# zhvng/open-musiclm

Hardware: AMD Instinct MI355X
Metric: train steps/sec + AR tokens/sec, coarse-stage musiclm_small (higher is better)
Workload: dtype fp16ff

## Files before the change

### include/omlm.h

```cpp
#ifndef OMLM_H
#define OMLM_H
#include <stdint.h>
#ifdef __cplusplus
extern "C" {
#endif

int         omlm_version(void);
const char* omlm_last_error(void);
void        omlm_set_error(const char* msg);

int omlm_gemm(const void* A, const void* B, void* C, const float* Cin,
              const int* a_map, const int* b_map, const int* c_map, long long a_rows, long long b_rows,
              int M, int N, int K, int lda, int ldb, int ldc, int ldcin,
              int a_kmajor, int b_kmajor, int in_dtype, int out_dtype, float alpha,
              void* workspace, long long workspace_bytes, void* stream);
long long omlm_gemm_tail_workspace_bytes(int M, int N);

int omlm_layernorm_fwd(const float* x, const float* gamma, void* y, void* xcast, float* mean, float* rstd,
                       int M, int D, int ldy, float eps, int out_dtype, void* stream);
int omlm_layernorm_fwd_planes(const float* x, const float* gamma, void* y, void* y_lo, float* mean, float* rstd,
                              int M, int D, int ldy, float eps, int out_dtype, void* stream);
long long omlm_layernorm_bwd_workspace_bytes(int D);
int omlm_layernorm_bwd(const void* dy, const float* x, const float* gamma, const float* mean, const float* rstd,
                       const float* dres, float* dx, void* dxcast, float* dgamma, float* workspace, int M, int D,
                       float dx_scale, int cast_dtype, int dy_dtype, void* stream);
int omlm_layernorm_bwd2(const void* dy, const float* x, const float* gamma, const float* mean, const float* rstd,
                        const float* dres, const void* dres2, float* dx, void* dxcast, float* dgamma, float* workspace, int M, int D,
                        float dx_scale, int cast_dtype, int dy_dtype, void* stream);

int omlm_qk_norm_fwd(const float* q_raw, const float* kv_raw, const float* q_scale, const float* k_scale,
                     void* q, void* k, void* v, int M, int H, int out_dtype, void* stream);
int omlm_qk_norm_bwd(const float* dq, const float* dk, const float* dv, const float* q_raw, const float* kv_raw,
                     const float* q_scale, const float* k_scale, void* dq_raw, void* dkv_raw,
                     float* dq_scale, float* dk_scale, int M, int H, int out_dtype, void* stream);

int omlm_gemm_qknorm(const void* A, const void* B, void* C, void* C2, int c2_col0, int ldc2, const float* scale, float* norm_out,
                     int ldnorm, int groups, long long a_rows, long long b_rows, int M, int N, int K, int lda, int ldb, int ldc,
                     int dtype, void* stream);
int omlm_qk_norm_bwd2(const float* dq, const float* dk, const float* dv, const void* q, const void* k, const float* qn, const float* kn,
                      const float* q_scale, const float* k_scale, void* dq_raw, void* dkv_raw, float* dq_scale, float* dk_scale,
                      int M, int H, int dtype, void* stream);

int omlm_mqa_attn_fwd(const void* q, const void* k, const void* v, const float* bias, const float* biasT,
                      const unsigned char* keymask, void* out, float* lse, int B, int N, int H, float scale, int bias_ld,
                      int dtype, void* stream);
long long omlm_attn_bias_table_floats(int N, int H);
int omlm_attn_bias_prepare(const float* bias, float* biasT, int N, int H, int bias_ld, const float* q_scale,
                           const float* k_scale, float qk_bound, float scale, int p_max_log2, void* stream);
int omlm_attn_bias_prepare_group(const float* bias, float* const* biasT, int layers, int N, int H, int bias_ld,
                                 const float* const* q_scale, const float* const* k_scale, float qk_bound, float scale,
                                 int p_max_log2, void* stream);
long long omlm_mqa_attn_bwd_workspace_bytes(int B, int N, int H);
int omlm_mqa_attn_bwd(const void* q, const void* k, const void* v, const float* bias, const float* biasT,
                      const unsigned char* keymask, const void* out, const void* dout, const float* lse, float* delta,
                      float* dq, float* dk, float* dv, float* dbias, float* dbias_ws,
                      int B, int N, int H, float scale, int bias_ld, int dtype, void* stream);

int omlm_mqa_attn_fwd_dropout(const void* q, const void* k, const void* v, const float* bias, const float* biasT,
                              const unsigned char* keymask, void* out, float* lse, int B, int N, int H, float scale, int bias_ld,
                              int dtype, float p, unsigned long long seed, const unsigned long long* seed_dev, void* stream);
int omlm_mqa_attn_bwd_dropout(const void* q, const void* k, const void* v, const float* bias, const float* biasT,
                              const unsigned char* keymask, const void* out, const void* dout, const float* lse, float* delta,
                              float* dq, float* dk, float* dv, float* dbias, float* dbias_ws,
                              int B, int N, int H, float scale, int bias_ld, int dtype, float p, unsigned long long seed,
                              const unsigned long long* seed_dev, void* stream);
int omlm_mqa_attn_fwd_prefix(const void* q, const void* k, const void* v, const float* bias, const float* biasT, const unsigned char* keymask,
                             void* out, float* lse, int B, int N, int H, float scale, int bias_ld, int dtype, int P, float p,
                             unsigned long long seed, const unsigned long long* seed_dev, void* stream);
int omlm_mqa_attn_bwd_prefix(const void* q, const void* k, const void* v, const float* bias, const float* biasT, const unsigned char* keymask,
                             const void* out, const void* dout, const float* lse, float* delta, float* dq, float* dk, float* dv, float* dbias,
                             float* dbias_ws, int B, int N, int H, float scale, int bias_ld, int dtype, int P, float p, unsigned long long seed,
                             const unsigned long long* seed_dev, void* stream);
long long omlm_attn_bias_table_floats_prefix(int N, int H, int P);
int omlm_attn_bias_prepare_group_prefix(const float* bias, float* const* biasT, int layers, int N, int H, int bias_ld,
                                        const float* const* q_scale, const float* const* k_scale, float qk_bound, float scale,
                                        int p_max_log2, int P, void* stream);
int omlm_attn_dropout_keep(unsigned char* keep, int B, int N, int H, float p, unsigned long long seed,
                           const unsigned long long* seed_dev, void* stream);
int omlm_dropout_residual_fwd(const float* x, const float* y, float* x1, long long M, int D, float p, unsigned long long seed,
                              const unsigned long long* seed_dev, void* stream);
int omlm_dropout_residual_bwd(const float* dx1, void* dy, long long M, int D, float p, unsigned long long seed,
                              const unsigned long long* seed_dev, int out_dtype, void* stream);

int omlm_ffmid_fwd(const void* h1, const void* convw, const void* gamma, void* h2, float* mean, float* rstd,
                   int M, int nseq, int F, int Fp, float eps, float p, unsigned long long seed,
                   const unsigned long long* seed_dev, unsigned char* drop_bits, void* gh, int dtype, void* stream);
int omlm_ffmid_fwd_planes(const void* h1, const void* h1_lo, const void* convw, const void* convw_lo, const void* gamma, const void* gamma_lo,
                          void* h2, void* h2_lo, float* mean, float* rstd, int M, int nseq, int F, int Fp, float eps, float p,
                          unsigned long long seed, const unsigned long long* seed_dev, unsigned char* drop_bits, void* gh, int dtype, void* stream);
long long omlm_ffmid_bwd_workspace_bytes(int F, int Fp);
int omlm_ffmid_bwd(const void* dh2, const void* h1, const void* convw, const void* gamma, const float* mean,
                   const float* rstd, void* du_tmp, void* dh1, float* dgamma, float* dconv, float* workspace,
                   int M, int nseq, int F, int Fp, float p, unsigned long long seed,
                   const unsigned long long* seed_dev, const unsigned char* drop_bits, const void* gh, int dtype, void* stream);
int omlm_colsum_accumulate(const float* part, float* out, int P, int C, int ldp, void* stream);
typedef struct omlm_colsum_desc { const float* part; float* out; int P, C, ldp; } omlm_colsum_desc;
int omlm_colsum_group(const omlm_colsum_desc* problems, int count, void* stream);
int omlm_ffmid_set_impl(int impl);

int omlm_embed_gather_fwd(const int* ids, const int* seg, const int* posidx,
                          const float* const* tables, const float* const* starts, const float* const* pos,
                          int nseq, float* out, int B, int N, int D,
                          const long long* table_rows, const long long* pos_rows, int* err_flag, void* stream);
int omlm_embed_gather_bwd(const int* ids, const int* seg, const int* posidx,
                          float* const* dtables, float* const* dstarts, float* const* dpos,
                          int nseq, const float* dx, int B, int N, int D, float alpha,
                          const long long* table_rows, const long long* pos_rows, int* err_flag, void* stream);

int omlm_prepare_train_batch(const long long* const* ids, int* const* labels, const int* len, const int* eos, const int* Q,
                             const int* codebook, int nseq, int B, int pad_id, const float* scores, int n_drop,
                             int* ids32, unsigned char* keymask, int N, void* stream);

int omlm_cross_entropy_fwd(const float* logits, const int* labels, float* row_lse, float* nll_sum,
                           int R, int V, int ld, int* err_flag, void* stream);
int omlm_cross_entropy_bwd(const float* logits, const int* labels, const float* row_lse, const float* gscale,
                           float coef, void* dlogits, int R, int V, int ld, int ldd, int out_dtype, void* stream);

int omlm_sumsq_accumulate(const float* g, long long n, float* out, float* partials, void* stream);
int omlm_adamw_clip_step(float* p, float* g, float* m, float* v, void* p16, long long n,
                         float lr, float beta1, float beta2, float eps, float wd, int step,
                         float gscale, const float* gnorm_sq, float max_norm, int decoupled, int zero_grad, int p16_dtype,
                         const float* ls_state, void* stream);
int omlm_loss_scale_update(float* ls_state, const float* gnorm_sq, float growth, float backoff, int interval,
                           float scale_min, float scale_max, void* stream);

int omlm_cast_pad(const float* src, void* dst, long long R, int C, int ld_src, int ld_dst, int out_dtype, void* stream);
int omlm_transpose_cast(const float* src, void* dst, int R, int C, int ld_src, int ld_dst, int out_dtype, void* stream);
typedef struct omlm_cast_pad_desc { const float* src; void* dst; int R, C, ld_src, ld_dst, transpose, lo; } omlm_cast_pad_desc;
int omlm_cast_pad_group(const omlm_cast_pad_desc* problems, int count, int out_dtype, void* stream);

int omlm_gemm_planes(const void* A, long long a_plane_bytes, const void* B, long long b_plane_bytes, void* C, const float* Cin,
                     const int* a_map, const int* b_map, const int* c_map, long long a_rows, long long b_rows,
                     int M, int N, int K, int lda, int ldb, int ldc, int ldcin,
                     int a_kmajor, int b_kmajor, int out_dtype, float alpha, void* workspace, long long workspace_bytes, void* stream);
int omlm_split_planes(const float* x, void* planes, long long n, long long plane_elems, void* stream);
int omlm_gemm_planes16(const void* A, const void* A_lo, const void* B, const void* B_lo, void* C, void* C_lo, const float* Cin,
                       const int* a_map, const int* c_map, long long a_rows, long long b_rows, int M, int N, int K,
                       int lda, int ldb, int ldc, int ldcin, int dtype, void* workspace, long long workspace_bytes, void* stream);
int omlm_gemm_mx16(const void* A, const void* A8, long long a8_stride, const unsigned char* a_scale,
                   const void* B, const void* B8, long long b8_stride, const unsigned char* b_scale,
                   void* C, void* C_lo, int c_lo_bf8, const float* Cin, long long a_rows, long long b_rows,
                   int M, int N, int K, int lda, int ldb, int ldc, int ldcin,
                   void* workspace, long long workspace_bytes, void* stream);
long long omlm_gemm_mx16_workspace_bytes(int M, int N, int K);
int omlm_layernorm_fwd_mx(const float* x, const float* gamma, void* y, void* y8, long long y8_stride, unsigned char* scale8,
                          float* mean, float* rstd, int M, int D, int ldy, float eps, void* stream);
int omlm_ffmid_fwd_mx(const void* h1, const void* h1_lo, const void* convw, const void* convw_lo, const void* gamma, const void* gamma_lo,
                      void* h2, void* h2_8, long long h2_8_stride, unsigned char* scale8, float* mean, float* rstd, int M, int nseq, int F, int Fp,
                      float eps, float p, unsigned long long seed, const unsigned long long* seed_dev, unsigned char* drop_bits, void* gh, void* stream);
typedef struct omlm_quant_rows_desc { const float* src; unsigned char* dst8; long long lo_stride; unsigned char* scale8; int R, C, ld_src, ld8; } omlm_quant_rows_desc;
int omlm_quant_rows_mx(const omlm_quant_rows_desc* problems, int count, void* stream);
typedef struct omlm_gemm_wgrad_desc {
    const void* A; const void* B; float* C; const int* c_map;
    int M, N, K, lda, ldb, ldc;
} omlm_gemm_wgrad_desc;
int omlm_gemm_wgrad_group(const omlm_gemm_wgrad_desc* problems, int count, int splits, int dtype, void* stream);

int omlm_relpos_first_fwd(const float* w0, const float* b0, float* pre, float* z, int n, int Hd, void* stream);
int omlm_relpos_first_bwd(const float* ds, float* dw0, int n, int Hd, void* stream);
int omlm_relpos_first_fwd_from(const float* w0, const float* b0, float* pre, float* z, int n, int Hd, int x0, void* stream);
int omlm_relpos_first_bwd_from(const float* ds, float* dw0, int n, int Hd, int x0, void* stream);
int omlm_bias_silu_fwd(const float* a, const float* b, float* pre, float* z, long long R, int C, void* stream);
int omlm_silu_bwd(const float* dz, const float* pre, float* ds, long long total, void* stream);
int omlm_bias_add(const float* a, const float* b, float* out, int R, int C, int ld, void* stream);
int omlm_relpos_mlp_fwd(const float* w0, const float* b0, const float* W1, const float* b1, const float* W2, const float* b2,
                        const float* W3, const float* b3, float* pre0, float* z0, float* pre1, float* z1, float* pre2, float* z2,
                        float* table, int n, int Hd, int H, int ldb, void* stream);
int omlm_relpos_mlp_bwd(const float* dtable, const float* W1, const float* W2, const float* W3, const float* pre0, const float* z0,
                        const float* pre1, const float* z1, const float* pre2, const float* z2, float* scratch, float* gw0, float* gb0,
                        float* gW1, float* gb1, float* gW2, float* gb2, float* gW3, float* gb3, int n, int Hd, int H, int ldb, void* stream);
int omlm_relpos_mlp_fwd_from(const float* w0, const float* b0, const float* W1, const float* b1, const float* W2, const float* b2,
                             const float* W3, const float* b3, float* pre0, float* z0, float* pre1, float* z1, float* pre2, float* z2,
                             float* table, int n, int Hd, int H, int ldb, int x0, void* stream);
int omlm_relpos_mlp_bwd_from(const float* dtable, const float* W1, const float* W2, const float* W3, const float* pre0, const float* z0,
                             const float* pre1, const float* z1, const float* pre2, const float* z2, float* scratch, float* gw0, float* gb0,
                             float* gW1, float* gb1, float* gW2, float* gb2, float* gW3, float* gb3, int n, int Hd, int H, int ldb, int x0,
                             void* stream);

int omlm_rvq_encode(const float* x, const float* codebooks_T, int* indices, float* residual_out,
                    int n, int D, int C, int nstage, void* stream);
int omlm_nearest_centroid(const float* x, const float* centroids_T, int* indices, int n, int D, int C, void* stream);
int omlm_rvq_encode_strided(const float* x, const float* codebook_T, int* indices, int idx_stride, float* residual_out,
                            int n, int D, int C, void* stream);
int omlm_vq_accumulate(const float* x, const int* indices, int idx_stride, float* counts, float* sums, int n, int D, int K, void* stream);
int omlm_vq_kmeans_update(float* means, float* means_T, const float* counts, const float* sums, int K, int D, void* stream);
int omlm_vq_ema_update(float* cluster_size, float* embed_avg, float* embed, float* embed_T, const float* counts, const float* sums,
                       float* total_scratch, int K, int D, float decay, float eps, void* stream);

int omlm_sample_topk_gumbel(const float* logits, const float* uniform, long long* out, int B, int V, int ld,
                            int k, float temperature, int forbid_last, void* stream);

int omlm_sample_topk_gumbel_at(const float* logits, const float* uniform_base, const int* step_dev, long long* out,
                               long long* hist, int B, int V, int ld, int k, float temperature, int forbid_last, void* stream);

int omlm_sample_embed_at(const float* logits, const float* uniform_base, const int* step_dev, long long* out, long long* hist,
                         int B, int V, int ld, int k, float temperature, int forbid_last,
                         const float* emb_table, long long emb_row_offset, long long emb_rows, float* x, int D, void* stream);

typedef struct omlm_decode_args {
    int B, D, H, L, F, Fp, Nmax, w_dtype, round_bf16, nsplit;
    float eps, scale;
    const int* pos_dev;
    const void* const* Wq; const void* const* Wkv; const void* const* Wo; const void* const* W1p; const void* const* W2p;
    const float* const* attn_gamma; const float* const* q_scale; const float* const* k_scale;
    const float* const* ffin_gamma; const float* const* convw; const float* const* mid_gamma;
    float* const* Kc; float* const* Vc; float* const* hist;
    const float* bias_table; int bias_ld;
    const float* final_gamma; const void* head_W; int V1; int ldV;
    const float* emb_table; long long emb_row_offset; long long emb_rows;
    float* x; float* x1; float* q; float* parts; float* u; float* logits;
    int* advance_pos; int* advance_step;
    float* ln_parts;
    const void* const* W1p_lo; const void* const* W2p_lo; const void* head_W_lo;
    float* splitk_ws; int* splitk_cnt;
} omlm_decode_args;
#define OMLM_DECODE_SPLITK_FLOATS(D) (4 * (((D) + 15) / 16) * 256)
#define OMLM_DECODE_LN_PARTS(D, Fp) ((((D) + 15) / 16 > ((Fp) + 7) / 8 ? ((D) + 15) / 16 : ((Fp) + 7) / 8) * 32)
int omlm_decode_step(const omlm_decode_args* args, const long long* ids, void* stream);
int omlm_decode_advance(int* pos_dev, int* step_dev, void* stream);

int omlm_probe_tr16(short* out, void* stream);

#ifdef __cplusplus
}
#endif
#endif
```

### open_musiclm_amd/csrc/gemm.hip

```cpp
#include "common.h"
#include "gemm_common.h"

namespace OMLM_NS {

template <int BM_, int BN_, int WM_, int WN_, bool A_KMAJ, bool B_KMAJ, typename TOUT, bool KMAP, bool SPLIT3 = false, bool FASTK = false, int EPI = 0>
__device__ __forceinline__ void gemm_tile_body(const GemmArgs& g, const int lg, const bool split, char* smem) {
    constexpr int NWN = BN_ / WN_, NWAVES = (BM_ / WM_) * NWN;
    constexpr int MI = WM_ / 32, NJ = WN_ / 32;
    constexpr int A_BYTES = BM_ * BK * 2, B_BYTES = BN_ * BK * 2, STAGE = A_BYTES + B_BYTES;
    constexpr int UA = (BM_ / 8) / NWAVES, UB = (BN_ / 8) / NWAVES;

    const int tiles_m = (g.M + BM_ - 1) / BM_, tiles_n = (g.N + BN_ - 1) / BN_;
    const int nwg = tiles_m * tiles_n;
    const int nk1 = (g.K + BK - 1) / BK;
    const int nk_all = SPLIT3 ? 3 * nk1 : nk1;
    constexpr int GROUP = OMLM_SUPER_ROWS / BM_;
    const int lane = threadIdx.x & 63;
    const int wave = __builtin_amdgcn_readfirstlane(threadIdx.x >> 6);
    const int wm = (wave / NWN) * WM_, wn = (wave % NWN) * WN_;
    const dma_rsrc rsA = make_dma_rsrc(g.A, (unsigned long long)g.a_rows * g.lda * 2);
    const dma_rsrc rsB = make_dma_rsrc(g.B, (unsigned long long)g.b_rows * g.ldb * 2);
    const dma_rsrc rsAl = make_dma_rsrc(SPLIT3 ? g.A_lo : g.A, (unsigned long long)g.a_rows * g.lda * 2);
    const dma_rsrc rsBl = make_dma_rsrc(SPLIT3 ? g.B_lo : g.B, (unsigned long long)g.b_rows * g.ldb * 2);

    {
        const int ksplit_id = lg / nwg;
        const int bid = lg - ksplit_id * nwg;
        const int kt0 = ksplit_id * g.kt_per_split;
        const int kt1 = min(nk_all, kt0 + g.kt_per_split);
        const int gsz = GROUP * tiles_n;
        const int grp = bid / gsz, first_m = grp * GROUP;
        const int rows_in = min(GROUP, tiles_m - first_m);
        const int tm = first_m + (bid - grp * gsz) % rows_in, tn = (bid - grp * gsz) / rows_in;
        const int m0 = tm * BM_, n0 = tn * BN_;

        DmaStagerT<A_KMAJ, BM_, NWAVES> sa;
        DmaStagerT<B_KMAJ, BN_, NWAVES> sb;
        sa.init(g.a_map, g.lda, g.M, m0, wave, lane);
        sb.init(g.b_map, g.ldb, g.N, n0, wave, lane);

        f32x16 acc[MI][NJ];
#pragma unroll
        for (int i = 0; i < MI; ++i)
#pragma unroll
            for (int j = 0; j < NJ; ++j)
#pragma unroll
                for (int e = 0; e < 16; ++e) acc[i][j][e] = 0.f;

        auto tile_at = [&](int t, bool& pa, bool& pb) -> int {
            if constexpr (SPLIT3) {
                const int which = t >= 2 * nk1 ? 2 : (t >= nk1 ? 1 : 0);
                pa = which == 2;
                pb = which == 1;
                return (t - which * nk1) * BK;
            } else {
                pa = false; pb = false;
                return t * BK;
            }
        };
        if (kt0 < kt1) {
            bool pa, pb;
            const int k00 = tile_at(kt0, pa, pb);
            sa.template issue<KMAP, FASTK>(SPLIT3 && pa ? rsAl : rsA, g.a_map, g.lda, k00, g.K, smem, wave);
            sb.template issue<KMAP, FASTK>(SPLIT3 && pb ? rsBl : rsB, g.b_map, g.ldb, k00, g.K, smem + A_BYTES, wave);
        }
        {
            h16x8 a[2][MI], b[2][NJ];
            bool pending = false;
            constexpr int MPS = MI * NJ, NLOAD = UA + UB;
            constexpr int SPREAD = 2;
            constexpr int STRIDE = (SPREAD * MPS) / NLOAD > 0 ? (SPREAD * MPS) / NLOAD : 1;
            for (int kt = kt0; kt < kt1; ++kt) {
                const int cur = (kt - kt0) & 1;
                asm volatile("s_waitcnt vmcnt(0)" ::: "memory");
                __syncthreads();
                const bool live = kt + 1 < kt1;
                char* nxt = smem + (cur ^ 1) * STAGE;
                bool pan, pbn;
                const int knext = tile_at(kt + 1, pan, pbn);
                const dma_rsrc rsAn = SPLIT3 && pan ? rsAl : rsA, rsBn = SPLIT3 && pbn ? rsBl : rsB;
                const char* As = smem + cur * STAGE;
                const char* Bs = As + A_BYTES;
                auto phase = [&](const int ph, const int fi, const bool mul) {
#pragma unroll
                    for (int i = 0; i < MI; ++i)
#pragma unroll
                        for (int j = 0; j < NJ; ++j) {
                            if (mul) acc[i][j] = OMLM_MFMA_32x32x16(a[fi][i], b[fi][j], acc[i][j]);
                            else if (mul) asm volatile("" :: "v"(a[fi][i]), "v"(b[fi][j]));
                            const int midx = ph * MPS + i * NJ + j;
                            if (midx % STRIDE == 0 && midx / STRIDE < NLOAD) {
                                const int l = midx / STRIDE;
                                __builtin_amdgcn_sched_barrier(0);
                                if (l < UA) sa.template issue_one<KMAP, FASTK>(l, rsAn, g.a_map, g.lda, knext, g.K, nxt, wave, live);
                                else        sb.template issue_one<KMAP, FASTK>(l - UA, rsBn, g.b_map, g.ldb, knext, g.K, nxt + A_BYTES, wave, live);
                                __builtin_amdgcn_sched_barrier(0);
                            }
                        }
                };
#pragma unroll
                for (int i = 0; i < MI; ++i) a[0][i] = read_frag<A_KMAJ>(As, wm + 32 * i, 0, lane);
#pragma unroll
                for (int j = 0; j < NJ; ++j) b[0][j] = read_frag<B_KMAJ>(Bs, wn + 32 * j, 0, lane);
                __builtin_amdgcn_sched_barrier(0);
                phase(0, 1, pending);
                __builtin_amdgcn_sched_barrier(0);
#pragma unroll
                for (int st = 0; st < 3; ++st) {
#pragma unroll
                    for (int i = 0; i < MI; ++i) a[(st + 1) & 1][i] = read_frag<A_KMAJ>(As, wm + 32 * i, st + 1, lane);
#pragma unroll
                    for (int j = 0; j < NJ; ++j) b[(st + 1) & 1][j] = read_frag<B_KMAJ>(Bs, wn + 32 * j, st + 1, lane);
                    __builtin_amdgcn_sched_barrier(0);
                    phase(st + 1, st & 1, true);
                    __builtin_amdgcn_sched_barrier(0);
                }
                pending = true;
            }
            if (pending) {
#pragma unroll
                for (int i = 0; i < MI; ++i)
#pragma unroll
                    for (int j = 0; j < NJ; ++j) acc[i][j] = OMLM_MFMA_32x32x16(a[1][i], b[1][j], acc[i][j]);
            }
        }
        asm volatile("s_waitcnt vmcnt(0)" ::: "memory");
        __syncthreads();
        constexpr bool SLICE = BM_ == 128 && BN_ == 128 && std::is_same<TOUT, float>::value && EPI == 0;
        tile_epilogue<MI, NJ, WN_, TOUT, EPI, (MI * NJ <= 4), SLICE>(g, acc, smem, m0, n0, wm, wn, wave, lane, split, nullptr,
                                                                     SLICE ? ksplit_id : 0);
    }
}

template <int BM_, int BN_, int WM_, int WN_, bool A_KMAJ, bool B_KMAJ, typename TOUT, bool KMAP, bool SPLIT3 = false, bool FASTK = false, int EPI = 0>
__global__ __launch_bounds__((BM_ / WM_) * (BN_ / WN_) * 64) void gemm_bf16_tile_kernel(GemmArgs g) {
    extern __shared__ __attribute__((aligned(16))) char smem[];
    const int nwg = gridDim.x;
    const int total = nwg * (int)gridDim.y;
    const int lg = xcd_logical_id(blockIdx.y * nwg + blockIdx.x, total);
    gemm_tile_body<BM_, BN_, WM_, WN_, A_KMAJ, B_KMAJ, TOUT, KMAP, SPLIT3, FASTK, EPI>(g, lg, gridDim.y > 1, smem);
}


template <int BM_, int BN_, int WM_, int WN_, bool A_KMAJ, bool B_KMAJ, typename TOUT, bool CIN, int EPI = 0>
__global__ __launch_bounds__((BM_ / WM_) * (BN_ / WN_) * 64) void gemm_bf16_tile_persist_kernel(GemmArgs g) {
    extern __shared__ __attribute__((aligned(16))) char smem[];
    constexpr int NWN = BN_ / WN_, NWAVES = (BM_ / WM_) * NWN;
    constexpr int MI = WM_ / 32, NJ = WN_ / 32;
    constexpr int A_BYTES = BM_ * BK * 2, B_BYTES = BN_ * BK * 2, STAGE = A_BYTES + B_BYTES;
    constexpr int UA = (BM_ / 8) / NWAVES, UB = (BN_ / 8) / NWAVES;
    constexpr int PATCH = 32 * (WN_ + 4) * 4;
    static_assert((NWAVES - 1) * PATCH <= STAGE, "all but the last wave's patch must fit inside one stage");
    constexpr int GROUP = OMLM_SUPER_ROWS / BM_;
    constexpr int VEC = sizeof(TOUT) == 2 ? 8 : 4, NSTORE = MI * (32 / (64 / (WN_ / VEC)));

    const int tiles_m = (g.M + BM_ - 1) / BM_, tiles_n = (g.N + BN_ - 1) / BN_;
    const int total = tiles_m * tiles_n;
    const int nk = g.K / BK;
    const int lane = threadIdx.x & 63;
    const int wave = __builtin_amdgcn_readfirstlane(threadIdx.x >> 6);
    const int wm = (wave / NWN) * WM_, wn = (wave % NWN) * WN_;
    const dma_rsrc rsA = make_dma_rsrc(g.A, (unsigned long long)g.a_rows * g.lda * 2);
    const dma_rsrc rsB = make_dma_rsrc(g.B, (unsigned long long)g.b_rows * g.ldb * 2);
    const unsigned smem_lds = (unsigned)(size_t)LDS_PTR(char, smem);

    auto origin = [&](int lin, int& m0, int& n0) {
        const int bid = xcd_logical_id(lin, total);
        const int gsz = GROUP * tiles_n;
        const int grp = bid / gsz, first_m = grp * GROUP;
        const int rows_in = min(GROUP, tiles_m - first_m);
        m0 = (first_m + (bid - grp * gsz) % rows_in) * BM_;
        n0 = ((bid - grp * gsz) / rows_in) * BN_;
    };
    auto piece = [&](int l, const unsigned (&va)[UA], const unsigned (&vb)[UB], int k0, unsigned stage_lds, bool live) {
        if (l < UA) {
            const int b = wave + NWAVES * l;
            dma_issue_s(rsA, stage_lds + (unsigned)(b * 1024), live ? va[l] : OOB_OFF,
                        A_KMAJ ? (unsigned)k0 * (unsigned)(g.lda * 2) : (unsigned)(k0 * 2));
        } else {
            const int b = wave + NWAVES * (l - UA);
            dma_issue_s(rsB, stage_lds + (unsigned)A_BYTES + (unsigned)(b * 1024), live ? vb[l - UA] : OOB_OFF,
                        B_KMAJ ? (unsigned)k0 * (unsigned)(g.ldb * 2) : (unsigned)(k0 * 2));
        }
    };

    int lin = blockIdx.x;
    const int G = gridDim.x;
    if (lin >= total) return;
    int m0, n0;
    origin(lin, m0, n0);
    unsigned va[UA], vb[UB];
    {
        DmaStagerT<A_KMAJ, BM_, NWAVES> sa;
        DmaStagerT<B_KMAJ, BN_, NWAVES> sb;
        sa.init(nullptr, g.lda, g.M, m0, wave, lane);
        sb.init(nullptr, g.ldb, g.N, n0, wave, lane);
#pragma unroll
        for (int i = 0; i < UA; ++i) va[i] = sa.vfast[i];
#pragma unroll
        for (int i = 0; i < UB; ++i) vb[i] = sb.vfast[i];
    }
    int par = 0;
#pragma unroll
    for (int l = 0; l < UA + UB; ++l) piece(l, va, vb, 0, smem_lds, true);
    bool counted = false;

    for (;;) {
        const int lin_n = lin + G;
        const bool has_next = lin_n < total;
        int m0n = m0, n0n = n0;
        if (has_next) origin(lin_n, m0n, n0n);
        unsigned van[UA], vbn[UB];
        {
            DmaStagerT<A_KMAJ, BM_, NWAVES> sa;
            DmaStagerT<B_KMAJ, BN_, NWAVES> sb;
            sa.init(nullptr, g.lda, g.M, m0n, wave, lane);
            sb.init(nullptr, g.ldb, g.N, n0n, wave, lane);
#pragma unroll
            for (int i = 0; i < UA; ++i) van[i] = sa.vfast[i];
#pragma unroll
            for (int i = 0; i < UB; ++i) vbn[i] = sb.vfast[i];
        }
        f32x16 acc[MI][NJ];
#pragma unroll
        for (int i = 0; i < MI; ++i)
#pragma unroll
            for (int j = 0; j < NJ; ++j)
#pragma unroll
                for (int e = 0; e < 16; ++e) acc[i][j][e] = 0.f;
        {
            h16x8 a[2][MI], b[2][NJ];
            bool pending = false;
            constexpr int MPS = MI * NJ, NLOAD = UA + UB;
            constexpr int SPREAD = 2;
            constexpr int STRIDE = (SPREAD * MPS) / NLOAD > 0 ? (SPREAD * MPS) / NLOAD : 1;
            for (int kt = 0; kt < nk; ++kt) {
                const int cur = (par + kt) & 1;
                if (kt == 0 && counted) asm volatile("s_waitcnt vmcnt(%0)" :: "n"(NSTORE) : "memory");
                else asm volatile("s_waitcnt vmcnt(0)" ::: "memory");
                __syncthreads();
                const bool last = kt + 1 == nk;
                const bool live = !last || has_next;
                const unsigned nxt = smem_lds + (unsigned)((cur ^ 1) * STAGE);
                const int knext = last ? 0 : (kt + 1) * BK;
                const char* As = smem + cur * STAGE;
                const char* Bs = As + A_BYTES;
                auto phase = [&](const int ph, const int fi, const bool mul) {
#pragma unroll
                    for (int i = 0; i < MI; ++i)
#pragma unroll
                        for (int j = 0; j < NJ; ++j) {
                            if (mul) acc[i][j] = OMLM_MFMA_32x32x16(a[fi][i], b[fi][j], acc[i][j]);
                            const int midx = ph * MPS + i * NJ + j;
                            if (midx % STRIDE == 0 && midx / STRIDE < NLOAD) {
                                const int l = midx / STRIDE;
                                __builtin_amdgcn_sched_barrier(0);
                                unsigned v;
                                if (l < UA) v = last ? van[l] : va[l]; else v = last ? vbn[l - UA] : vb[l - UA];
                                {
                                    unsigned one_a[UA], one_b[UB];
#pragma unroll
                                    for (int x = 0; x < UA; ++x) one_a[x] = v;
#pragma unroll
                                    for (int x = 0; x < UB; ++x) one_b[x] = v;
                                    piece(l, one_a, one_b, knext, nxt, live);
                                }
                                __builtin_amdgcn_sched_barrier(0);
                            }
                        }
                };
#pragma unroll
                for (int i = 0; i < MI; ++i) a[0][i] = read_frag<A_KMAJ>(As, wm + 32 * i, 0, lane);
#pragma unroll
                for (int j = 0; j < NJ; ++j) b[0][j] = read_frag<B_KMAJ>(Bs, wn + 32 * j, 0, lane);
                __builtin_amdgcn_sched_barrier(0);
                phase(0, 1, pending);
                __builtin_amdgcn_sched_barrier(0);
#pragma unroll
                for (int st = 0; st < 3; ++st) {
#pragma unroll
                    for (int i = 0; i < MI; ++i) a[(st + 1) & 1][i] = read_frag<A_KMAJ>(As, wm + 32 * i, st + 1, lane);
#pragma unroll
                    for (int j = 0; j < NJ; ++j) b[(st + 1) & 1][j] = read_frag<B_KMAJ>(Bs, wn + 32 * j, st + 1, lane);
                    __builtin_amdgcn_sched_barrier(0);
                    phase(st + 1, st & 1, true);
                    __builtin_amdgcn_sched_barrier(0);
                }
                pending = true;
            }
            if (pending) {
#pragma unroll
                for (int i = 0; i < MI; ++i)
#pragma unroll
                    for (int j = 0; j < NJ; ++j) acc[i][j] = OMLM_MFMA_32x32x16(a[1][i], b[1][j], acc[i][j]);
            }
        }
        const int cur_last = (par + nk - 1) & 1;
        if (!has_next) asm volatile("s_waitcnt vmcnt(0)" ::: "memory");
        __syncthreads();
        float* patch = wave < NWAVES - 1 ? (float*)(smem + cur_last * STAGE + wave * PATCH) : (float*)(smem + 2 * STAGE);
        GemmArgs ge = g;
        ge.c_map = nullptr;
        if constexpr (!CIN) ge.Cin = nullptr;
        tile_epilogue<MI, NJ, WN_, TOUT, EPI, false>(ge, acc, smem, m0, n0, wm, wn, wave, lane, false, patch);
        if (!has_next) break;
        counted = m0 + BM_ <= g.M && n0 + BN_ <= g.N;
        par = (par + nk) & 1;
        lin = lin_n; m0 = m0n; n0 = n0n;
#pragma unroll
        for (int i = 0; i < UA; ++i) va[i] = van[i];
#pragma unroll
        for (int i = 0; i < UB; ++i) vb[i] = vbn[i];
    }
}


template <bool A_KMAJ, bool B_KMAJ, typename TOUT, bool SPLIT3 = false>
__device__ __forceinline__ void gemm_tile8_body(const GemmArgs& g, const int m0, const int n0, const int kt0, const int kt1, const bool split, char* smem) {
    constexpr int A_BYTES = 256 * BK * 2, STAGE = 2 * A_BYTES;
    const int lane = threadIdx.x & 63;
    const int wave = __builtin_amdgcn_readfirstlane(threadIdx.x >> 6);
    const int wr = wave >> 2, wc = wave & 3;
    const dma_rsrc rsA = make_dma_rsrc(g.A, (unsigned long long)g.a_rows * g.lda * 2);
    const dma_rsrc rsB = make_dma_rsrc(g.B, (unsigned long long)g.b_rows * g.ldb * 2);
    const dma_rsrc rsAl = make_dma_rsrc(SPLIT3 ? g.A_lo : g.A, (unsigned long long)g.a_rows * g.lda * 2);
    const dma_rsrc rsBl = make_dma_rsrc(SPLIT3 ? g.B_lo : g.B, (unsigned long long)g.b_rows * g.ldb * 2);
    DmaStagerT<A_KMAJ, 256, 8> sa;
    DmaStagerT<B_KMAJ, 256, 8> sb;
    sa.init(nullptr, g.lda, g.M, m0, wave, lane);
    sb.init(nullptr, g.ldb, g.N, n0, wave, lane);
    const int nk = kt1 - kt0;
    const unsigned smem_lds = (unsigned)(size_t)LDS_PTR(char, smem);

    f32x16 acc[2][2][2];
#pragma unroll
    for (int x = 0; x < 8; ++x)
#pragma unroll
        for (int e = 0; e < 16; ++e) acc[x >> 2][(x >> 1) & 1][x & 1][e] = 0.f;

    auto stage = [&](auto JC, const int T) {
        constexpr int J = decltype(JC)::value;
        constexpr bool isA = (J & 1) != 0;
        constexpr int h = J >> 1;
        const bool live = T < nk;
        unsigned k0 = (unsigned)(kt0 + T) * BK;
        bool lo = false;
        if constexpr (SPLIT3) {
            const int t = kt0 + T, nk1 = g.K / BK;
            const int which = t >= 2 * nk1 ? 2 : (t >= nk1 ? 1 : 0);
            k0 = (unsigned)(t - which * nk1) * BK;
            lo = isA ? which == 2 : which == 1;
        }
        const dma_rsrc rs = isA ? (SPLIT3 && lo ? rsAl : rsA) : (SPLIT3 && lo ? rsBl : rsB);
        if constexpr (SPLIT3) k0 = (unsigned)__builtin_amdgcn_readfirstlane((int)k0);
        const unsigned base = smem_lds + (unsigned)((T & 1) * STAGE) + (isA ? 0u : (unsigned)A_BYTES);
#pragma unroll
        for (int u = 0; u < 2; ++u) {
            const int i = 2 * h + u;
            const int b = wave + 8 * i;
            if constexpr (isA) dma_issue_s(rs, base + (unsigned)(b * 1024), live ? sa.vfast[i] : OOB_OFF, A_KMAJ ? k0 * (unsigned)(g.lda * 2) : k0 * 2u);
            else               dma_issue_s(rs, base + (unsigned)(b * 1024), live ? sb.vfast[i] : OOB_OFF, B_KMAJ ? k0 * (unsigned)(g.ldb * 2) : k0 * 2u);
        }
    };
    using J0 = std::integral_constant<int, 0>; using J1 = std::integral_constant<int, 1>;
    using J2 = std::integral_constant<int, 2>; using J3 = std::integral_constant<int, 3>;

    h16x8 a[2][4], bX[4], bY[4], bZ[4];
    auto read_a = [&](const int T, const int ha) {
        const char* As = smem + (T & 1) * STAGE;
#pragma unroll
        for (int i = 0; i < 2; ++i)
#pragma unroll
            for (int st = 0; st < 4; ++st) a[i][st] = read_frag<A_KMAJ>(As, ha * 128 + wr * 64 + 32 * i, st, lane);
    };
    auto read_b = [&](h16x8 (&b)[4], const int T, const int hb) {
        const char* Bs = smem + (T & 1) * STAGE + A_BYTES;
#pragma unroll
        for (int st = 0; st < 4; ++st) b[st] = read_frag<B_KMAJ>(Bs, hb * 128 + wc * 32, st, lane);
    };
    auto mma = [&](f32x16 (&c)[2], const h16x8 (&b)[4]) {
        __builtin_amdgcn_s_setprio(1);
#pragma unroll
        for (int st = 0; st < 4; ++st)
#pragma unroll
            for (int i = 0; i < 2; ++i) c[i] = OMLM_MFMA_32x32x16(a[i][st], b[st], c[i]);
        __builtin_amdgcn_s_setprio(0);
    };
#define T8_SYNC_IN()                                                           \
    do {                                                                       \
        __builtin_amdgcn_sched_barrier(0);                                     \
        asm volatile("s_waitcnt vmcnt(10)" ::: "memory");                      \
        __builtin_amdgcn_s_barrier();                                          \
        asm volatile("s_waitcnt lgkmcnt(0)" ::: "memory");                     \
        __builtin_amdgcn_sched_barrier(0);                                     \
    } while (0)
#define T8_SYNC_OUT()                                                          \
    do {                                                                       \
        __builtin_amdgcn_sched_barrier(0);                                     \
        __builtin_amdgcn_s_barrier();                                          \
        __builtin_amdgcn_sched_barrier(0);                                     \
    } while (0)

    stage(J0{}, 0); stage(J1{}, 0); stage(J2{}, 0); stage(J3{}, 0);
    stage(J0{}, 1); stage(J1{}, 1); stage(J2{}, 1);
    asm volatile("s_waitcnt vmcnt(10)" ::: "memory");
    __builtin_amdgcn_s_barrier();
    read_b(bX, 0, 0);
    asm volatile("s_waitcnt lgkmcnt(0)" ::: "memory");
    __builtin_amdgcn_sched_barrier(0);
    if (wr == 1) __builtin_amdgcn_s_barrier();

    auto ktile = [&](h16x8 (&b0)[4], h16x8 (&bn)[4], const int T) {
        read_a(T, 0);             stage(J3{}, T + 1);  T8_SYNC_IN();  mma(acc[0][0], b0);  T8_SYNC_OUT();
        read_b(bY, T, 1);         stage(J0{}, T + 2);  T8_SYNC_IN();  mma(acc[0][1], bY);  T8_SYNC_OUT();
        read_a(T, 1);             stage(J1{}, T + 2);  T8_SYNC_IN();  mma(acc[1][1], bY);  T8_SYNC_OUT();
        read_b(bn, T + 1, 0);     stage(J2{}, T + 2);  T8_SYNC_IN();  mma(acc[1][0], b0);  T8_SYNC_OUT();
    };
    for (int T = 0; T < nk; T += 2) {
        ktile(bX, bZ, T);
        if (T + 1 < nk) ktile(bZ, bX, T + 1);
    }
    if (wr == 0) __builtin_amdgcn_s_barrier();
#undef T8_SYNC_IN
#undef T8_SYNC_OUT
    asm volatile("s_waitcnt vmcnt(0)" ::: "memory");
    __syncthreads();
#pragma unroll
    for (int ha = 0; ha < 2; ++ha)
#pragma unroll
        for (int hb = 0; hb < 2; ++hb)
            tile_epilogue<2, 1, 32, TOUT>(g, reinterpret_cast<f32x16 (&)[2][1]>(acc[ha][hb]), smem, m0, n0, ha * 128 + wr * 64, hb * 128 + wc * 32,
                                          wave, lane, split);
}

template <bool A_KMAJ, bool B_KMAJ, typename TOUT, bool SPLIT3 = false>
__global__ __launch_bounds__(512) void gemm_tile8_kernel(GemmArgs g) {
    extern __shared__ __attribute__((aligned(16))) char smem[];
    const int nwg = gridDim.x;
    const int lg = xcd_logical_id(blockIdx.y * nwg + blockIdx.x, nwg * (int)gridDim.y);
    const int tiles_m = (g.M + 255) / 256, tiles_n = (g.N + 255) / 256;
    const int ksplit = lg / nwg, bid = lg - ksplit * nwg;
    const int nk_all = (SPLIT3 ? 3 : 1) * (g.K / BK);
    const int kt0 = ksplit * g.kt_per_split, kt1 = min(nk_all, kt0 + g.kt_per_split);
    constexpr int GROUP = OMLM_SUPER_ROWS / 256;
    const int gsz = GROUP * tiles_n;
    const int grp = bid / gsz, first_m = grp * GROUP;
    const int rows_in = min(GROUP, tiles_m - first_m);
    const int tm = first_m + (bid - grp * gsz) % rows_in, tn = (bid - grp * gsz) / rows_in;
    if (kt0 >= kt1) return;
    gemm_tile8_body<A_KMAJ, B_KMAJ, TOUT, SPLIT3>(g, tm * 256, tn * 256, kt0, kt1, gridDim.y > 1, smem);
}


#define OMLM_GROUP_MAX 48
struct omlm_gemm_wgrad_desc { const void* A; const void* B; float* C; const int* c_map; int M, N, K, lda, ldb, ldc; };
struct GroupProb { const void* A; const void* B; float* C; const int* c_map; int M, N, K, lda, ldb, ldc, kt_per_split, start; };
struct GroupArgs { int n, total; GroupProb p[OMLM_GROUP_MAX]; };

template <bool FASTK, bool T8 = false>
__global__ __launch_bounds__(512) void gemm_wgrad_group_kernel(GroupArgs ga) {
    extern __shared__ __attribute__((aligned(16))) char smem[];
    const int lg = xcd_logical_id(blockIdx.x, ga.total);
    int pi = 0;
    for (int i = 1; i < ga.n; ++i) if (lg >= ga.p[i].start) pi = i;
    const GroupProb& q = ga.p[pi];
    GemmArgs g;
    g.A = q.A; g.B = q.B; g.C = q.C; g.Cin = q.C; g.a_map = nullptr; g.b_map = nullptr; g.c_map = q.c_map;
    g.a_rows = q.K; g.b_rows = q.K; g.M = q.M; g.N = q.N; g.K = q.K; g.lda = q.lda; g.ldb = q.ldb; g.ldc = q.ldc; g.ldcin = q.ldc;
    g.alpha = 1.f; g.kt_per_split = q.kt_per_split; g.bal_ck = 0; g.bal_chunks = 0; g.debug = 0; g.split3 = 0; g.A_lo = nullptr; g.B_lo = nullptr; g.C_lo = nullptr; g.c_lo8 = 0; g.c_split_stride = 0;
    g.epi_scale = nullptr; g.epi_norm = nullptr; g.epi_groups = 0; g.epi_ldnorm = 0; g.C2 = nullptr; g.c2_col0 = 0; g.ldc2 = 0;
    const int nk = (q.K + BK - 1) / BK;
    if constexpr (T8) {
        const int lq = lg - q.start;
        const int tiles_m = (q.M + 255) / 256, tiles_n = (q.N + 255) / 256, nwg = tiles_m * tiles_n;
        const int ksplit = lq / nwg, bid = lq - ksplit * nwg;
        const int kt0 = ksplit * q.kt_per_split, kt1 = min(nk, kt0 + q.kt_per_split);
        constexpr int GROUP = OMLM_SUPER_ROWS / 256;
        const int gsz = GROUP * tiles_n;
        const int grp = bid / gsz, first_m = grp * GROUP;
        const int rows_in = min(GROUP, tiles_m - first_m);
        const int tm = first_m + (bid - grp * gsz) % rows_in, tn = (bid - grp * gsz) / rows_in;
        if (kt0 < kt1) gemm_tile8_body<true, true, float>(g, tm * 256, tn * 256, kt0, kt1, q.kt_per_split < nk, smem);
    } else {
        gemm_tile_body<256, 256, 128, 64, true, true, float, false, false, FASTK>(g, lg - q.start, q.kt_per_split < nk, smem);
    }
}


#ifdef OMLM_ISA_ONLY
template __global__ void gemm_bf16_tile_persist_kernel<256, 256, 128, 64, false, false, h16_t, false>(GemmArgs);
template __global__ void gemm_bf16_tile_persist_kernel<256, 256, 128, 64, false, true, h16_t, false>(GemmArgs);
template __global__ void gemm_bf16_tile_persist_kernel<256, 256, 128, 64, false, false, float, true>(GemmArgs);
template __global__ void gemm_bf16_tile_persist_kernel<256, 256, 128, 64, false, true, float, true>(GemmArgs);
template __global__ void gemm_bf16_tile_persist_kernel<128, 128, 64, 64, false, false, h16_t, false>(GemmArgs);
template __global__ void gemm_bf16_tile_persist_kernel<128, 128, 64, 64, false, false, float, true>(GemmArgs);
template __global__ void gemm_bf16_tile_persist_kernel<128, 128, 64, 64, false, false, h16_t, false, 1>(GemmArgs);
template __global__ void gemm_tile8_kernel<false, false, h16_t>(GemmArgs);
template __global__ void gemm_tile8_kernel<false, true, h16_t>(GemmArgs);
template __global__ void gemm_tile8_kernel<false, false, float>(GemmArgs);
template __global__ void gemm_tile8_kernel<true, true, float>(GemmArgs);
template __global__ void gemm_tile8_kernel<false, false, h16pl_t, true>(GemmArgs);
template __global__ void gemm_tile8_kernel<false, false, float, true>(GemmArgs);
}
#else
static int gemm_persist_slots() {
    static int ncu8 = -1;
    if (ncu8 < 0) {
        int dev = 0, n = 0;
        ncu8 = (hipGetDevice(&dev) == hipSuccess && hipDeviceGetAttribute(&n, hipDeviceAttributeMultiprocessorCount, dev) == hipSuccess && n >= 8) ? n / 8 * 8 : 0;
    }
    const char* e = getenv("OMLM_GEMM_PERSIST");
    return (e && e[0] == '0') ? 0 : ncu8;
}

static int gemm_t8_mode() {
    const char* e = getenv("OMLM_GEMM_T8");
    return e ? atoi(e) : OMLM_GEMM_T8_DEFAULT;
}
static bool gemm_t8_wanted(int K, int tiles, int splits) {
    const int mode = gemm_t8_mode();
    if (mode <= 0) return false;
    if (mode == 1) return true;
    static int ncu = 0;
    if (ncu == 0) {
        int dev = 0, n = 0;
        ncu = (hipGetDevice(&dev) == hipSuccess && hipDeviceGetAttribute(&n, hipDeviceAttributeMultiprocessorCount, dev) == hipSuccess && n > 0) ? n : 256;
    }
    return splits == 1 && K >= 2048 && tiles > ncu;
}

template <int BM_, int BN_, int WM_, int WN_, typename TOUT>
static int launch_tile(const GemmArgs& g, int a_kmaj, int b_kmaj, int splits, hipStream_t st) {
    constexpr int NTH = (BM_ / WM_) * (BN_ / WN_) * 64;
    constexpr size_t LDS = 2 * (size_t)(BM_ + BN_) * BK * 2;
    const int tiles = ((g.M + BM_ - 1) / BM_) * ((g.N + BN_ - 1) / BN_);
    dim3 grid(tiles, splits), block(NTH);
    if constexpr (BM_ == 256 && BN_ == 256) {
        if (gemm_t8_wanted(g.split3 ? 3 * g.K : g.K, tiles, splits) && g.K % BK == 0 && !g.a_map && !g.b_map &&
            (!g.split3 || !OMLM_FP16)) {
#define OMLM_T8_LAUNCH(AK, BKM)                                                                                       \
            do {                                                                                                       \
                auto k8 = gemm_tile8_kernel<AK, BKM, TOUT>;                                                            \
                static bool attr8 = false;                                                                             \
                if (!attr8) { (void)hipFuncSetAttribute((const void*)k8, hipFuncAttributeMaxDynamicSharedMemorySize, (int)LDS); attr8 = true; } \
                if constexpr (!OMLM_FP16) {                                                                            \
                    auto k83 = gemm_tile8_kernel<AK, BKM, TOUT, true>;                                                 \
                    static bool attr83 = false;                                                                        \
                    if (!attr83) { (void)hipFuncSetAttribute((const void*)k83, hipFuncAttributeMaxDynamicSharedMemorySize, (int)LDS); attr83 = true; } \
                    if (g.split3) { hipLaunchKernelGGL(k83, grid, block, LDS, st, g); break; }                         \
                }                                                                                                      \
                hipLaunchKernelGGL(k8, grid, block, LDS, st, g);                                                       \
            } while (0)
            if (!a_kmaj && !b_kmaj)      OMLM_T8_LAUNCH(false, false);
            else if (!a_kmaj && b_kmaj)  OMLM_T8_LAUNCH(false, true);
            else if (a_kmaj && b_kmaj)   OMLM_T8_LAUNCH(true, true);
            else                         OMLM_T8_LAUNCH(true, false);
#undef OMLM_T8_LAUNCH
            return omlm_post_launch("omlm_gemm");
        }
    }
    const bool need_kmap = (a_kmaj && g.a_map) || (b_kmaj && g.b_map);
    if (need_kmap && BM_ != 128) { omlm_set_error("omlm_gemm: k-row maps are only built for the 128x128 tile"); return OMLM_ERR_UNSUPPORTED; }
#define OMLM_TILE_LAUNCH(AK, BKM)                                                                                          \
    do {                                                                                                                    \
        auto kfn = gemm_bf16_tile_kernel<BM_, BN_, WM_, WN_, AK, BKM, TOUT, false>;                                        \
        auto kmap = gemm_bf16_tile_kernel<BM_, BN_, WM_, WN_, AK, BKM, TOUT, (AK || BKM) && BM_ == 128>;                   \
        auto kfast = gemm_bf16_tile_kernel<BM_, BN_, WM_, WN_, AK, BKM, TOUT, false, false, true>;                         \
        static bool attr = false;                                                                                           \
        if (!attr) {                                                                                                        \
            (void)hipFuncSetAttribute((const void*)kfn, hipFuncAttributeMaxDynamicSharedMemorySize, (int)LDS);             \
            (void)hipFuncSetAttribute((const void*)kfast, hipFuncAttributeMaxDynamicSharedMemorySize, (int)LDS);           \
            (void)hipFuncSetAttribute((const void*)kmap, hipFuncAttributeMaxDynamicSharedMemorySize, (int)LDS);            \
        }                                                                                                                   \
        if constexpr (!OMLM_FP16) {                                                                                         \
            auto ks3 = gemm_bf16_tile_kernel<BM_, BN_, WM_, WN_, AK, BKM, TOUT, false, true>;                               \
            if (!attr) (void)hipFuncSetAttribute((const void*)ks3, hipFuncAttributeMaxDynamicSharedMemorySize, (int)LDS);  \
            attr = true;                                                                                                    \
            if (g.split3) { hipLaunchKernelGGL(ks3, grid, block, LDS, st, g); break; }                                     \
        }                                                                                                                   \
        attr = true;                                                                                                        \
        if (need_kmap) hipLaunchKernelGGL(kmap, grid, block, LDS, st, g);                                                  \
        else if (g.K % BK == 0) hipLaunchKernelGGL(kfast, grid, block, LDS, st, g);                                        \
        else           hipLaunchKernelGGL(kfn, grid, block, LDS, st, g);                                                   \
    } while (0)
    if constexpr ((BM_ == 256 && BN_ == 256) || (BM_ == 128 && BN_ == 128)) {
        const int slots = gemm_persist_slots() * (BM_ == 128 ? 2 : 1);
        if (slots > 0 && !a_kmaj && splits == 1 && !g.split3 && !g.a_map && !g.b_map && !g.c_map && g.K % BK == 0 && tiles > slots) {
            constexpr size_t LDSP = LDS + 32 * (WN_ + 4) * 4;
            static bool pattr = false;
            auto k0 = gemm_bf16_tile_persist_kernel<BM_, BN_, WM_, WN_, false, false, TOUT, false>;
            auto k1 = gemm_bf16_tile_persist_kernel<BM_, BN_, WM_, WN_, false, true, TOUT, false>;
            auto k0c = gemm_bf16_tile_persist_kernel<BM_, BN_, WM_, WN_, false, false, TOUT, true>;
            auto k1c = gemm_bf16_tile_persist_kernel<BM_, BN_, WM_, WN_, false, true, TOUT, true>;
            if (!pattr) {
                (void)hipFuncSetAttribute((const void*)k0, hipFuncAttributeMaxDynamicSharedMemorySize, (int)LDSP);
                (void)hipFuncSetAttribute((const void*)k1, hipFuncAttributeMaxDynamicSharedMemorySize, (int)LDSP);
                (void)hipFuncSetAttribute((const void*)k0c, hipFuncAttributeMaxDynamicSharedMemorySize, (int)LDSP);
                (void)hipFuncSetAttribute((const void*)k1c, hipFuncAttributeMaxDynamicSharedMemorySize, (int)LDSP);
                pattr = true;
            }
            hipLaunchKernelGGL(g.Cin ? (b_kmaj ? k1c : k0c) : (b_kmaj ? k1 : k0), dim3(slots), block, LDSP, st, g);
            return omlm_post_launch("omlm_gemm");
        }
    }
    if (!a_kmaj && !b_kmaj)      OMLM_TILE_LAUNCH(false, false);
    else if (!a_kmaj && b_kmaj)  OMLM_TILE_LAUNCH(false, true);
    else if (a_kmaj && b_kmaj)   OMLM_TILE_LAUNCH(true, true);
    else                         OMLM_TILE_LAUNCH(true, false);
#undef OMLM_TILE_LAUNCH
    return omlm_post_launch("omlm_gemm");
}

template <int BM_, int BN_, int WM_, int WN_, typename TOUT>
static int launch_tile_s3(const GemmArgs& g, hipStream_t st, int splits = 1) {
    constexpr int NTH = (BM_ / WM_) * (BN_ / WN_) * 64;
    constexpr size_t LDS = 2 * (size_t)(BM_ + BN_) * BK * 2;
    const int tiles = ((g.M + BM_ - 1) / BM_) * ((g.N + BN_ - 1) / BN_);
    dim3 grid(tiles, splits), block(NTH);
    if constexpr (BM_ == 256 && BN_ == 256) {
        if (gemm_t8_mode() > 0 && g.K % BK == 0 && !g.a_map && splits == 1) {
            auto k8 = gemm_tile8_kernel<false, false, TOUT, true>;
            static bool attr8 = false;
            if (!attr8) { (void)hipFuncSetAttribute((const void*)k8, hipFuncAttributeMaxDynamicSharedMemorySize, (int)LDS); attr8 = true; }
            hipLaunchKernelGGL(k8, grid, block, LDS, st, g);
            return omlm_post_launch("omlm_gemm_planes16");
        }
    }
    auto ks3 = gemm_bf16_tile_kernel<BM_, BN_, WM_, WN_, false, false, TOUT, false, true>;
    static bool attr = false;
    if (!attr) { (void)hipFuncSetAttribute((const void*)ks3, hipFuncAttributeMaxDynamicSharedMemorySize, (int)LDS); attr = true; }
    hipLaunchKernelGGL(ks3, grid, block, LDS, st, g);
    return omlm_post_launch("omlm_gemm_planes16");
}

template <typename T, typename TOUT>
static int launch_layout(const GemmArgs& g, int a_kmaj, int b_kmaj, int splits, hipStream_t st) {
    const int tiles = ((g.M + BM - 1) / BM) * ((g.N + BN - 1) / BN);
    const size_t lds = 4 * (size_t)(BM * BK * 2);
    dim3 grid(tiles, splits), block(NTHREADS);
    if constexpr (elt_traits<T>::precise) {
        if (!a_kmaj && !b_kmaj)      hipLaunchKernelGGL((gemm_kernel<T, false, false, TOUT>), grid, block, lds, st, g);
        else if (!a_kmaj && b_kmaj)  hipLaunchKernelGGL((gemm_kernel<T, false, true, TOUT>), grid, block, lds, st, g);
        else if (a_kmaj && b_kmaj)   hipLaunchKernelGGL((gemm_kernel<T, true, true, TOUT>), grid, block, lds, st, g);
        else                         hipLaunchKernelGGL((gemm_kernel<T, true, false, TOUT>), grid, block, lds, st, g);
    }
    return omlm_post_launch("omlm_gemm");
}


static bool gemm_tail_split_on() {
    const char* e = getenv("OMLM_GEMM_TAIL_SPLIT");
    return !(e && e[0] == '0');
}

static int gemm_impl(const void* A, const void* B, void* C, const float* Cin,
                     const int* a_map, const int* b_map, const int* c_map,
                     long long a_rows, long long b_rows,
                     int M, int N, int K, int lda, int ldb, int ldc, int ldcin,
                     int a_kmajor, int b_kmajor, int in_dtype, int out_dtype, float alpha, void* stream,
                     int split3, const void* A_lo, const void* B_lo, void* C_lo = nullptr, bool s3_route = false,
                     float* tail_ws = nullptr, long long tail_ws_bytes = 0) {
    if (M <= 0 || N <= 0) return OMLM_OK;
    OMLM_CHECK_ARG(A && B && C, "null operand");
    OMLM_CHECK_ARG(K > 0, "K must be positive");
    OMLM_CHECK_ARG((lda % 8) == 0 && (ldb % 8) == 0, "operand leading dimensions must be multiples of 8 elements");
    OMLM_CHECK_ARG(((uintptr_t)A % 16) == 0 && ((uintptr_t)B % 16) == 0, "operands must be 16-byte aligned");
    OMLM_CHECK_ARG(in_dtype == 0 || in_dtype == 1, "in_dtype: 0=fp32 (bf16x3) or 1=bf16");
    OMLM_CHECK_ARG(out_dtype == 0 || out_dtype == 1, "out_dtype: 0=fp32 or 1=bf16");
    const size_t esz = in_dtype == 0 ? 4 : 2;
    OMLM_CHECK_ARG((unsigned long long)a_rows * lda * esz < 0xFFFFFFF0ull, "A exceeds the 4 GiB buffer-descriptor window");
    OMLM_CHECK_ARG((unsigned long long)b_rows * ldb * esz < 0xFFFFFFF0ull, "B exceeds the 4 GiB buffer-descriptor window");
    if (a_kmajor) OMLM_CHECK_ARG(lda >= ((M + 7) / 8) * 8, "k-major A: row pitch shorter than M padded to 8");
    if (b_kmajor) OMLM_CHECK_ARG(ldb >= ((N + 7) / 8) * 8, "k-major B: row pitch shorter than N padded to 8");
    if (!a_kmajor || !b_kmajor) OMLM_CHECK_ARG(K % 8 == 0, "k-contiguous operands need K % 8 == 0 (zero-pad the contraction)");
    GemmArgs g;
    g.A = A; g.B = B; g.C = C; g.Cin = Cin; g.a_map = a_map; g.b_map = b_map; g.c_map = c_map;
    g.a_rows = a_rows; g.b_rows = b_rows; g.M = M; g.N = N; g.K = K;
    g.lda = lda; g.ldb = ldb; g.ldc = ldc; g.ldcin = ldcin; g.alpha = alpha;
    g.bal_ck = 0; g.bal_chunks = 0; g.debug = 0;
    g.split3 = split3; g.A_lo = A_lo; g.B_lo = B_lo; g.C_lo = C_lo; g.c_lo8 = 0; g.c_split_stride = 0;
    g.epi_scale = nullptr; g.epi_norm = nullptr; g.epi_groups = 0; g.epi_ldnorm = 0; g.C2 = nullptr; g.c2_col0 = 0; g.ldc2 = 0;
    hipStream_t st = as_stream(stream);
    int bm = BM, bn = BN;
    const char* force = getenv("OMLM_GEMM_TILE");
    const bool need_kmap = (a_kmajor && a_map) || (b_kmajor && b_map);
    if (in_dtype == 1 && !need_kmap) {
        if (force && force[0]) { if (!strcmp(force, "256x256")) { bm = 256; bn = 256; } else if (!strcmp(force, "256x128")) { bm = 256; bn = 128; } }
        else if (K <= 512 && N <= 1024 && K % BK == 0 && !a_kmajor && !a_map && !b_map && !c_map && !split3 && Cin != (const float*)C &&
                 ((M + 127) / 128) * ((N + 127) / 128) > 2 * gemm_persist_slots() && gemm_persist_slots() > 0) { bm = 128; bn = 128; }
        else if (M >= 1024 && N >= 1024) { bm = 256; bn = 256; }
        else if (M >= 2048 && N > 512) { bm = 256; bn = 128; }
        else if (N >= 2048 && M >= 256) { bm = 256; bn = 256; }
    }
    static int ncu = 0;
    if (ncu == 0) {
        int dev = 0, n = 0;
        if (hipGetDevice(&dev) == hipSuccess && hipDeviceGetAttribute(&n, hipDeviceAttributeMultiprocessorCount, dev) == hipSuccess && n > 0) ncu = n;
        else ncu = 256;
    }
    const int nk = ((K + BK - 1) / BK) * (split3 ? 3 : 1);
    const int tiles = ((M + bm - 1) / bm) * ((N + bn - 1) / bn);
    int splits = 1;
    const bool fine = in_dtype == 0 && !split3;
    if (Cin == (const float*)C && out_dtype == 0 && tiles < 512 && nk >= (fine ? 4 : 16)) {
        const int slots = (bm == 256 ? 1 : 2) * ncu;
        int smax = fine ? nk / 2 : nk / 8; if (smax > 32) smax = 32; if (smax < 1) smax = 1;
        int smin = (slots + tiles - 1) / tiles; if (smin > smax) smin = smax; if (smin < 1) smin = 1;
        float best = -1.f;
        for (int sp = smin; sp <= smax; ++sp) {
            const int total = tiles * sp, rounds = (total + slots - 1) / slots;
            const float util = (float)total / (float)(rounds * slots) - (bm == 256 ? 0.02f : 0.012f) * (float)sp;
            if (util > best) { best = util; splits = sp; }
        }
    }
    g.kt_per_split = (nk + splits - 1) / splits;
    splits = (nk + g.kt_per_split - 1) / g.kt_per_split;
    if (in_dtype == 0) {
#if OMLM_FP16
        omlm_set_error("omlm_gemm: fp32 operands are served by the bf16 copy of the library");
        return OMLM_ERR_UNSUPPORTED;
#else
        static bool attr_done = false;
        if (!attr_done) {
            (void)hipFuncSetAttribute((const void*)gemm_kernel<float, false, false, float>, hipFuncAttributeMaxDynamicSharedMemorySize, 65536);
            (void)hipFuncSetAttribute((const void*)gemm_kernel<float, false, true, float>, hipFuncAttributeMaxDynamicSharedMemorySize, 65536);
            (void)hipFuncSetAttribute((const void*)gemm_kernel<float, true, true, float>, hipFuncAttributeMaxDynamicSharedMemorySize, 65536);
            (void)hipFuncSetAttribute((const void*)gemm_kernel<float, true, false, float>, hipFuncAttributeMaxDynamicSharedMemorySize, 65536);
            attr_done = true;
        }
        OMLM_CHECK_ARG(out_dtype == 0, "fp32 operands produce fp32 output");
        return launch_layout<float, float>(g, a_kmajor, b_kmajor, splits, st);
#endif
    }
    auto launch = [&](const GemmArgs& ga, int tm_, int tn_, int sp) -> int {
        if (s3_route) {
            if (tm_ == 256 && tn_ == 256)
                return ga.C_lo ? launch_tile_s3<256, 256, 128, 64, h16pl_t>(ga, st) : launch_tile_s3<256, 256, 128, 64, float>(ga, st);
            if (tm_ == 256 && tn_ == 128)
                return ga.C_lo ? launch_tile_s3<256, 128, 64, 64, h16pl_t>(ga, st) : launch_tile_s3<256, 128, 64, 64, float>(ga, st);
            return ga.C_lo ? launch_tile_s3<128, 128, 64, 64, h16pl_t>(ga, st) : launch_tile_s3<128, 128, 64, 64, float>(ga, st);
        }
        if (tm_ == 256 && tn_ == 256)
            return out_dtype == 0 ? launch_tile<256, 256, 128, 64, float>(ga, a_kmajor, b_kmajor, sp, st)
                                  : launch_tile<256, 256, 128, 64, h16_t>(ga, a_kmajor, b_kmajor, sp, st);
        if (tm_ == 256 && tn_ == 128)
            return out_dtype == 0 ? launch_tile<256, 128, 64, 64, float>(ga, a_kmajor, b_kmajor, sp, st)
                                  : launch_tile<256, 128, 64, 64, h16_t>(ga, a_kmajor, b_kmajor, sp, st);
        return out_dtype == 0 ? launch_tile<128, 128, 64, 64, float>(ga, a_kmajor, b_kmajor, sp, st)
                              : launch_tile<128, 128, 64, 64, h16_t>(ga, a_kmajor, b_kmajor, sp, st);
    };
    if (bm == 256 && bn == 256 && splits == 1 && !a_kmajor && !a_map && !c_map && !(force && force[0]) && tiles > ncu) {
        const int tiles_n = (N + 255) / 256, tiles_m = (M + 255) / 256;
        const int rem = tiles % ncu;
        const int m_full = ((tiles / ncu) * ncu) / tiles_n;
        if (rem > 0 && rem < ncu / 2 && m_full >= 1 && m_full < tiles_m) {
            const size_t osz = out_dtype == 0 ? 4 : 2;
            const long long M1 = (long long)m_full * 256;
            GemmArgs g1 = g, g2 = g;
            g1.M = (int)M1;
            g2.M = M - (int)M1;
            g2.A = (const char*)A + (size_t)M1 * lda * 2;
            g2.a_rows = a_rows - M1;
            g2.C = (char*)C + (size_t)M1 * ldc * osz;
            if (g.A_lo && !a_kmajor) g2.A_lo = (const char*)g.A_lo + (size_t)M1 * lda * 2;
            if (g.C_lo) g2.C_lo = (char*)g.C_lo + (size_t)M1 * ldc * osz;
            if (Cin) g2.Cin = Cin + (size_t)M1 * ldcin;
            const int rc = launch(g1, 256, 256, 1);
            if (rc != OMLM_OK) return rc;
            if (tail_ws && gemm_tail_split_on() && alpha == 1.0f) {
                const int Mt = g2.M, Nw = (N + 3) / 4 * 4;
                const int tiles_t = ((Mt + 127) / 128) * ((N + 127) / 128);
                int S = (2 * ncu) / tiles_t;
                if (S > nk / 8) S = nk / 8;
                if (S > 8) S = 8;
                if (S >= 2) {
                    const int ktps = (nk + S - 1) / S;
                    S = (nk + ktps - 1) / ktps;
                    const long long slice = (long long)Mt * Nw;
                    if (S >= 2 && (long long)S * slice * 4 <= tail_ws_bytes) {
                        GemmArgs gw = g2;
                        gw.C = tail_ws; gw.C_lo = nullptr; gw.Cin = nullptr; gw.ldc = Nw; gw.ldcin = 0;
                        gw.c_split_stride = slice; gw.kt_per_split = ktps;
                        const int rc2 = s3_route ? launch_tile_s3<128, 128, 64, 64, float>(gw, st, S)
                                                 : launch_tile<128, 128, 64, 64, float>(gw, a_kmajor, b_kmajor, S, st);
                        if (rc2 != OMLM_OK) return rc2;
                        const long long quads = (long long)Mt * (Nw / 4);
                        const int blocks = (int)((quads + 255) / 256 > 4096 ? 4096 : (quads + 255) / 256);
                        if (out_dtype == 0)
                            hipLaunchKernelGGL(gemm_tail_reduce_kernel<0>, dim3(blocks), dim3(256), 0, st, tail_ws, S, slice, Mt, N, Nw, g2.C, nullptr, ldc, g2.Cin, ldcin);
                        else if (g2.C_lo)
                            hipLaunchKernelGGL(gemm_tail_reduce_kernel<2>, dim3(blocks), dim3(256), 0, st, tail_ws, S, slice, Mt, N, Nw, g2.C, g2.C_lo, ldc, g2.Cin, ldcin);
                        else
                            hipLaunchKernelGGL(gemm_tail_reduce_kernel<1>, dim3(blocks), dim3(256), 0, st, tail_ws, S, slice, Mt, N, Nw, g2.C, nullptr, ldc, g2.Cin, ldcin);
                        return omlm_post_launch("omlm_gemm (tail reduce)");
                    }
                }
            }
            return launch(g2, 128, 128, 1);
        }
    }
    return launch(g, bm, bn, splits);
}

#if !OMLM_FP16
extern "C" long long omlm_gemm_tail_workspace_bytes(int M, int N) {
    if (M <= 0 || N <= 0) return 0;
    int dev = 0, ncu = 256;
    if (hipGetDevice(&dev) == hipSuccess) (void)hipDeviceGetAttribute(&ncu, hipDeviceAttributeMultiprocessorCount, dev);
    const long long tiles_n = (N + 255) / 256, tiles_m = (M + 255) / 256;
    if (tiles_m * tiles_n <= ncu) return 0;
    long long tail_rows = ((long long)(ncu / 2) / tiles_n + 1) * 256;
    if (tail_rows > M) tail_rows = M;
    return 8ll * tail_rows * ((N + 3) / 4 * 4) * 4;
}
#endif

#if !OMLM_FP16
extern "C" int omlm_gemm_h(const void* A, const void* B, void* C, const float* Cin, const int* a_map, const int* b_map, const int* c_map,
                           long long a_rows, long long b_rows, int M, int N, int K, int lda, int ldb, int ldc, int ldcin,
                           int a_kmajor, int b_kmajor, int in_dtype, int out_dtype, float alpha, void* workspace, long long workspace_bytes, void* stream);
#endif
extern "C" int OMLM_API(omlm_gemm)(const void* A, const void* B, void* C, const float* Cin,
                         const int* a_map, const int* b_map, const int* c_map,
                         long long a_rows, long long b_rows,
                         int M, int N, int K, int lda, int ldb, int ldc, int ldcin,
                         int a_kmajor, int b_kmajor, int in_dtype, int out_dtype, float alpha, void* workspace, long long workspace_bytes, void* stream) {
#if !OMLM_FP16
    if (in_dtype == OMLM_DT_F16) {
        OMLM_CHECK_ARG(out_dtype == OMLM_DT_F32 || out_dtype == OMLM_DT_F16, "fp16 operands produce fp32 or fp16 output");
        return omlm_gemm_h(A, B, C, Cin, a_map, b_map, c_map, a_rows, b_rows, M, N, K, lda, ldb, ldc, ldcin, a_kmajor, b_kmajor,
                           1, OMLM_H_CODE(out_dtype), alpha, workspace, workspace_bytes, stream);
    }
#endif
    OMLM_CHECK_ARG((workspace == nullptr) == (workspace_bytes == 0) && workspace_bytes >= 0 && ((uintptr_t)workspace % 16) == 0,
                   "tail workspace: 16-byte aligned buffer and its size, or NULL / 0");
    return gemm_impl(A, B, C, Cin, a_map, b_map, c_map, a_rows, b_rows, M, N, K, lda, ldb, ldc, ldcin, a_kmajor, b_kmajor,
                     in_dtype, out_dtype, alpha, stream, 0, nullptr, nullptr, nullptr, false, (float*)workspace, workspace_bytes);
}

#if !OMLM_FP16
extern "C" int omlm_gemm_qknorm_h(const void* A, const void* B, void* C, void* C2, int c2_col0, int ldc2, const float* scale, float* norm_out,
                                  int ldnorm, int groups, long long a_rows, long long b_rows, int M, int N, int K, int lda, int ldb, int ldc,
                                  int dtype, void* stream);
#endif
extern "C" int OMLM_API(omlm_gemm_qknorm)(const void* A, const void* B, void* C, void* C2, int c2_col0, int ldc2, const float* scale,
                                          float* norm_out, int ldnorm, int groups, long long a_rows, long long b_rows, int M, int N, int K,
                                          int lda, int ldb, int ldc, int dtype, void* stream) {
#if !OMLM_FP16
    if (dtype == OMLM_DT_F16) return omlm_gemm_qknorm_h(A, B, C, C2, c2_col0, ldc2, scale, norm_out, ldnorm, groups, a_rows, b_rows, M, N, K, lda, ldb, ldc, 1, stream);
#endif
    if (M <= 0 || N <= 0) return OMLM_OK;
    OMLM_CHECK_ARG(dtype == 1, "gemm_qknorm: operand dtype 1 (bf16) or 2 (fp16)");
    OMLM_CHECK_ARG(A && B && C && scale && norm_out && K > 0 && (K % 8) == 0, "gemm_qknorm: null operand / K");
    OMLM_CHECK_ARG((N % 64) == 0 && groups >= 0 && groups * 64 <= N && ldnorm >= groups, "gemm_qknorm: N must be whole 64-wide heads");
    OMLM_CHECK_ARG((lda % 8) == 0 && (ldb % 8) == 0 && (ldc % 8) == 0 && ((uintptr_t)A % 16) == 0 && ((uintptr_t)B % 16) == 0 && ((uintptr_t)C % 16) == 0,
                   "gemm_qknorm: 16-byte aligned operands, pitches multiples of 8");
    OMLM_CHECK_ARG(!C2 || ((c2_col0 % 64) == 0 && (ldc2 % 8) == 0 && ((uintptr_t)C2 % 16) == 0), "gemm_qknorm: second output");
    OMLM_CHECK_ARG((unsigned long long)a_rows * lda * 2 < 0xFFFFFFF0ull && (unsigned long long)b_rows * ldb * 2 < 0xFFFFFFF0ull, "operand exceeds the 4 GiB window");
    GemmArgs g;
    memset(&g, 0, sizeof(g));
    g.A = A; g.B = B; g.C = C; g.a_rows = a_rows; g.b_rows = b_rows; g.M = M; g.N = N; g.K = K; g.lda = lda; g.ldb = ldb; g.ldc = ldc;
    g.alpha = 1.f; g.epi_scale = scale; g.epi_norm = norm_out; g.epi_groups = groups; g.epi_ldnorm = ldnorm; g.C2 = C2; g.c2_col0 = c2_col0; g.ldc2 = ldc2;
    const int nk = (K + BK - 1) / BK;
    g.kt_per_split = nk;
    constexpr size_t LDS = 2 * (size_t)(128 + 128) * BK * 2;
    const int tiles = ((M + 127) / 128) * ((N + 127) / 128);
    auto kfast = gemm_bf16_tile_kernel<128, 128, 64, 64, false, false, h16_t, false, false, true, 1>;
    auto kgen = gemm_bf16_tile_kernel<128, 128, 64, 64, false, false, h16_t, false, false, false, 1>;
    static bool attr = false;
    if (!attr) {
        (void)hipFuncSetAttribute((const void*)kfast, hipFuncAttributeMaxDynamicSharedMemorySize, (int)LDS);
        (void)hipFuncSetAttribute((const void*)kgen, hipFuncAttributeMaxDynamicSharedMemorySize, (int)LDS);
        attr = true;
    }
    const int slots = 2 * gemm_persist_slots();
    if (slots > 0 && tiles > slots && K % BK == 0) {
        constexpr size_t LDSP = LDS + 32 * (64 + 4) * 4;
        auto kp = gemm_bf16_tile_persist_kernel<128, 128, 64, 64, false, false, h16_t, false, 1>;
        static bool pattr = false;
        if (!pattr) { (void)hipFuncSetAttribute((const void*)kp, hipFuncAttributeMaxDynamicSharedMemorySize, (int)LDSP); pattr = true; }
        hipLaunchKernelGGL(kp, dim3(slots), dim3(256), LDSP, as_stream(stream), g);
    }
    else if (K % BK == 0) hipLaunchKernelGGL(kfast, dim3(tiles, 1), dim3(256), LDS, as_stream(stream), g);
    else                                        hipLaunchKernelGGL(kgen, dim3(tiles, 1), dim3(256), LDS, as_stream(stream), g);
    return omlm_post_launch("omlm_gemm_qknorm");
}

#if !OMLM_FP16
extern "C" int omlm_gemm_planes16_h(const void* A, const void* A_lo, const void* B, const void* B_lo, void* C, void* C_lo, const float* Cin,
                                    const int* a_map, const int* c_map, long long a_rows, long long b_rows, int M, int N, int K,
                                    int lda, int ldb, int ldc, int ldcin, int dtype, void* workspace, long long workspace_bytes, void* stream);
#endif
extern "C" int OMLM_API(omlm_gemm_planes16)(const void* A, const void* A_lo, const void* B, const void* B_lo, void* C, void* C_lo, const float* Cin,
                                            const int* a_map, const int* c_map, long long a_rows, long long b_rows, int M, int N, int K,
                                            int lda, int ldb, int ldc, int ldcin, int dtype, void* workspace, long long workspace_bytes, void* stream) {
#if !OMLM_FP16
    if (dtype == OMLM_DT_F16) return omlm_gemm_planes16_h(A, A_lo, B, B_lo, C, C_lo, Cin, a_map, c_map, a_rows, b_rows, M, N, K, lda, ldb, ldc, ldcin, 1,
                                                          workspace, workspace_bytes, stream);
#endif
    OMLM_CHECK_ARG((workspace == nullptr) == (workspace_bytes == 0) && workspace_bytes >= 0 && ((uintptr_t)workspace % 16) == 0,
                   "tail workspace: 16-byte aligned buffer and its size, or NULL / 0");
    OMLM_CHECK_ARG(dtype == 1, "gemm_planes16: operand dtype 1 (bf16) or 2 (fp16)");
    OMLM_CHECK_ARG(A_lo && B_lo, "gemm_planes16: null lo plane");
    OMLM_CHECK_ARG(((uintptr_t)A_lo % 16) == 0 && ((uintptr_t)B_lo % 16) == 0 && ((uintptr_t)C_lo % 16) == 0, "gemm_planes16: 16-byte aligned planes");
    OMLM_CHECK_ARG(!(C_lo && Cin), "gemm_planes16: plane output takes no residual");
    return gemm_impl(A, B, C, Cin, a_map, nullptr, c_map, a_rows, b_rows, M, N, K, lda, ldb, ldc, ldcin, 0, 0,
                     1, C_lo ? 1 : 0, 1.0f, stream, 1, A_lo, B_lo, C_lo, true, (float*)workspace, workspace_bytes);
}

#if !OMLM_FP16
extern "C" int omlm_gemm_planes(const void* A, long long a_plane_bytes, const void* B, long long b_plane_bytes, void* C, const float* Cin,
                                const int* a_map, const int* b_map, const int* c_map, long long a_rows, long long b_rows,
                                int M, int N, int K, int lda, int ldb, int ldc, int ldcin,
                                int a_kmajor, int b_kmajor, int out_dtype, float alpha, void* workspace, long long workspace_bytes, void* stream) {
    OMLM_CHECK_ARG((workspace == nullptr) == (workspace_bytes == 0) && workspace_bytes >= 0 && ((uintptr_t)workspace % 16) == 0,
                   "tail workspace: 16-byte aligned buffer and its size, or NULL / 0");
    OMLM_CHECK_ARG(a_plane_bytes > 0 && b_plane_bytes > 0 && (a_plane_bytes % 16) == 0 && (b_plane_bytes % 16) == 0, "plane strides");
    OMLM_CHECK_ARG(!(a_kmajor && a_map) && !(b_kmajor && b_map), "k-row maps are not supported on operand planes");
    return gemm_impl(A, B, C, Cin, a_map, b_map, c_map, a_rows, b_rows, M, N, K, lda, ldb, ldc, ldcin, a_kmajor, b_kmajor,
                     1, out_dtype, alpha, stream, 1, (const char*)A + a_plane_bytes, (const char*)B + b_plane_bytes, nullptr, false,
                     (float*)workspace, workspace_bytes);
}

__global__ __launch_bounds__(256) void split_planes_kernel(const float* __restrict__ x, unsigned short* __restrict__ planes,
                                                           long long n, long long plane_elems) {
    const long long i0 = ((long long)blockIdx.x * 256 + threadIdx.x) * 8;
    const long long stride = (long long)gridDim.x * 256 * 8;
    for (long long i = i0; i < n; i += stride) {
        if (i + 8 <= n) {
            const float4 a = *(const float4*)(x + i), b = *(const float4*)(x + i + 4);
            unsigned h0, h1, h2, h3, l0, l1, l2, l3;
            split_pair(a.x, a.y, h0, l0); split_pair(a.z, a.w, h1, l1);
            split_pair(b.x, b.y, h2, l2); split_pair(b.z, b.w, h3, l3);
            u32x4 hi, lo;
            hi[0] = h0; hi[1] = h1; hi[2] = h2; hi[3] = h3; lo[0] = l0; lo[1] = l1; lo[2] = l2; lo[3] = l3;
            *(u32x4*)(planes + i) = hi;
            *(u32x4*)(planes + plane_elems + i) = lo;
        } else {
            for (long long j = i; j < n; ++j) {
                const unsigned u = f2u(x[j]) & 0xFFFF0000u;
                planes[j] = (unsigned short)(u >> 16);
                planes[plane_elems + j] = (unsigned short)bf16_bits_rne(x[j] - u2f(u));
            }
        }
    }
}
extern "C" int omlm_split_planes(const float* x, void* planes, long long n, long long plane_elems, void* stream) {
    if (n <= 0) return OMLM_OK;
    OMLM_CHECK_ARG(x && planes && plane_elems >= n && (plane_elems % 8) == 0, "split_planes arguments");
    OMLM_CHECK_ARG(((uintptr_t)x % 16) == 0 && ((uintptr_t)planes % 16) == 0, "split_planes: 16-byte aligned buffers");
    long long blocks = (n / 8 + 255) / 256;
    if (blocks > 16384) blocks = 16384;
    if (blocks < 1) blocks = 1;
    hipLaunchKernelGGL(split_planes_kernel, dim3((unsigned)blocks), dim3(256), 0, as_stream(stream), x, (unsigned short*)planes, n, plane_elems);
    return omlm_post_launch("omlm_split_planes");
}

#endif

#if !OMLM_FP16
extern "C" int omlm_gemm_wgrad_group_h(const omlm_gemm_wgrad_desc* d, int count, int splits, int dtype, void* stream);
#endif
extern "C" int OMLM_API(omlm_gemm_wgrad_group)(const omlm_gemm_wgrad_desc* d, int count, int splits, int dtype, void* stream) {
    if (count <= 0) return OMLM_OK;
    OMLM_CHECK_ARG(d, "null descriptor array");
#if !OMLM_FP16
    if (dtype == OMLM_DT_F16) return omlm_gemm_wgrad_group_h(d, count, splits, 1, stream);
#endif
    OMLM_CHECK_ARG(dtype == 1, "wgrad group: operand dtype must be 1 (bf16) or 2 (fp16)");
    static int ncu = 0;
    if (ncu == 0) {
        int dev = 0, n = 0;
        if (hipGetDevice(&dev) == hipSuccess && hipDeviceGetAttribute(&n, hipDeviceAttributeMultiprocessorCount, dev) == hipSuccess && n > 0) ncu = n;
        else ncu = 256;
    }
    static bool attr = false;
    if (!attr) {
        (void)hipFuncSetAttribute((const void*)gemm_wgrad_group_kernel<false>, hipFuncAttributeMaxDynamicSharedMemorySize, 131072);
        (void)hipFuncSetAttribute((const void*)gemm_wgrad_group_kernel<true>, hipFuncAttributeMaxDynamicSharedMemorySize, 131072);
        (void)hipFuncSetAttribute((const void*)gemm_wgrad_group_kernel<true, true>, hipFuncAttributeMaxDynamicSharedMemorySize, 131072);
        attr = true;
    }
    for (int base = 0; base < count; base += OMLM_GROUP_MAX) {
        const int n = count - base < OMLM_GROUP_MAX ? count - base : OMLM_GROUP_MAX;
        long long units = 0;
        int nk_min = 1 << 30;
        bool fastk = true;
        for (int i = 0; i < n; ++i) {
            const omlm_gemm_wgrad_desc& q = d[base + i];
            if (q.K % BK != 0) fastk = false;
            OMLM_CHECK_ARG(q.A && q.B && q.C && q.M > 0 && q.N > 0 && q.K > 0, "wgrad group: bad problem");
            OMLM_CHECK_ARG((q.lda % 8) == 0 && (q.ldb % 8) == 0 && q.lda >= ((q.M + 7) / 8) * 8 && q.ldb >= ((q.N + 7) / 8) * 8,
                           "wgrad group: k-major operand pitches must be multiples of 8 covering the padded extent");
            OMLM_CHECK_ARG(((uintptr_t)q.A % 16) == 0 && ((uintptr_t)q.B % 16) == 0, "wgrad group: operands must be 16-byte aligned");
            OMLM_CHECK_ARG((unsigned long long)q.K * q.lda * 2 < 0xFFFFFFF0ull && (unsigned long long)q.K * q.ldb * 2 < 0xFFFFFFF0ull,
                           "wgrad group: operand exceeds the 4 GiB buffer-descriptor window");
            units += (long long)((q.M + 255) / 256) * ((q.N + 255) / 256);
            const int nk = (q.K + BK - 1) / BK;
            if (nk < nk_min) nk_min = nk;
        }
        int sp = splits;
        if (sp <= 0) {
            float best = -1.f;
            sp = 1;
            for (int s = 1; s <= 4; ++s) {
                const long long wgs = units * s, rounds = (wgs + ncu - 1) / ncu;
                const float util = (float)wgs / (float)(rounds * ncu) - 0.02f * (float)(s - 1);
                if (util > best) { best = util; sp = s; }
            }
        }
        if (sp > nk_min / 8) sp = nk_min / 8 > 0 ? nk_min / 8 : 1;
        GroupArgs ga;
        memset(&ga, 0, sizeof(ga));
        ga.n = n;
        int start = 0;
        for (int i = 0; i < n; ++i) {
            const omlm_gemm_wgrad_desc& q = d[base + i];
            GroupProb& p = ga.p[i];
            p.A = q.A; p.B = q.B; p.C = q.C; p.c_map = q.c_map; p.M = q.M; p.N = q.N; p.K = q.K; p.lda = q.lda; p.ldb = q.ldb; p.ldc = q.ldc;
            const int nk = (q.K + BK - 1) / BK;
            p.kt_per_split = (nk + sp - 1) / sp;
            const int s_eff = (nk + p.kt_per_split - 1) / p.kt_per_split;
            p.start = start;
            start += ((q.M + 255) / 256) * ((q.N + 255) / 256) * s_eff;
        }
        ga.total = start;
        if (fastk && gemm_t8_mode() > 0) hipLaunchKernelGGL((gemm_wgrad_group_kernel<true, true>), dim3(start), dim3(512), 131072, as_stream(stream), ga);
        else if (fastk) hipLaunchKernelGGL(gemm_wgrad_group_kernel<true>, dim3(start), dim3(512), 131072, as_stream(stream), ga);
        else       hipLaunchKernelGGL(gemm_wgrad_group_kernel<false>, dim3(start), dim3(512), 131072, as_stream(stream), ga);
    }
    return omlm_post_launch("omlm_gemm_wgrad_group");
}

}
#endif
```

### open_musiclm_amd/engine.py

```python
from __future__ import annotations

import math
import os
from dataclasses import dataclass, field
from typing import Dict, List, Optional, Sequence, Tuple

import torch

from . import ops
from .hip import require_gpu

ATTN_SCALE = 8.0
DIM_HEAD = 64

_PRECISIONS = {"bf16": torch.bfloat16, "bf16x3": torch.float32, "fp16": torch.float16, "fp16ff": torch.float16}


def is_half(precision: str) -> bool:
    return precision in ("fp16", "fp16ff")
_H16 = (torch.bfloat16, torch.float16)



FF_PLANES_MAX_FP = 4096


def ff_planes_ok(Fp: int) -> bool:
    return Fp <= FF_PLANES_MAX_FP


def ff_mx_ok(D: int, Fp: int) -> bool:
    return D % 64 == 0 and D <= 4096 and Fp % 64 == 0 and ff_planes_ok(Fp)


def default_precision() -> str:
    p = os.environ.get("OMLM_PRECISION", "bf16")
    if p not in _PRECISIONS:
        raise ValueError(f"OMLM_PRECISION must be one of {list(_PRECISIONS)}, got {p}")
    return p


def loss_scale_initial() -> float:
    return float(os.environ.get("OMLM_FP16_LOSS_SCALE", "4096"))


def loss_scale_state(model) -> torch.Tensor:
    dev = model.start_tokens[0].device
    st = model.__dict__.get("_omlm_ls_state")
    if st is None or st.device != dev:
        st = torch.tensor([loss_scale_initial(), 0.0, 0.0, 0.0, loss_scale_initial()], device=dev, dtype=torch.float32)
        model.__dict__["_omlm_ls_state"] = st
    return st


def loss_scale(precision: str, model=None) -> float:
    if not is_half(precision):
        return 1.0
    if model is None or "_omlm_ls_state" not in model.__dict__:
        return loss_scale_initial()
    return float(model.__dict__["_omlm_ls_state"][0].item())


_MODEL_OF: Dict[int, tuple] = {}


def tag_parameters(model, precision: Optional[str]):
    import weakref
    ref = weakref.ref(model)
    for p in model.parameters():
        p._omlm_precision = precision
        key = id(p)
        _MODEL_OF[key] = (weakref.ref(p, lambda _r, k=key: _MODEL_OF.pop(k, None)), ref)


def model_of(p) -> Optional[torch.nn.Module]:
    ent = _MODEL_OF.get(id(p))
    if ent is None or ent[0]() is not p:
        return None
    return ent[1]()


@torch.no_grad()
def unscale_grads_(model, precision: Optional[str] = None):
    s = loss_scale(precision or getattr(model, "precision", None) or default_precision(), model)
    if s != 1.0:
        for p in model.parameters():
            if p.grad is not None:
                p.grad.mul_(1.0 / s)


def ceil_to(x: int, m: int) -> int:
    return (x + m - 1) // m * m


def grad_of(p: torch.Tensor) -> torch.Tensor:
    if p.grad is None:
        p.grad = torch.zeros_like(p, memory_format=torch.contiguous_format)
    return p.grad


@dataclass
class SeqLayout:
    B: int
    N: int
    lens: Tuple[int, ...]
    starts: Tuple[int, ...]
    n_out: Tuple[int, ...]
    seg: torch.Tensor
    posidx: torch.Tensor
    start_col: torch.Tensor
    final_only: bool = False
    head_maps: Dict[Tuple[int, int], Tuple[torch.Tensor, torch.Tensor, int]] = field(default_factory=dict)


def build_layout(B: int, lens: Sequence[int], quantizers: Sequence[int], device, final_rows_only: bool = False) -> SeqLayout:
    starts, pos = [], 0
    for l in lens:
        starts.append(pos)
        pos += l + 1
    N = pos
    seg = torch.empty(N, dtype=torch.int32)
    posidx = torch.zeros(N, dtype=torch.int32)
    start_col = torch.zeros(N, dtype=torch.bool)
    for s, (st, l) in enumerate(zip(starts, lens)):
        seg[st: st + l + 1] = s
        start_col[st] = True
        posidx[st + 1: st + l + 1] = torch.arange(l, dtype=torch.int32)
    n_out = [l for l in lens[:-1]] + [lens[-1] + 1]
    lay = SeqLayout(B, N, tuple(lens), tuple(starts), tuple(n_out), seg.to(device), posidx.to(device),
                    start_col.to(device), final_rows_only)
    if final_rows_only:
        s, st, n_s, Q = len(lens) - 1, starts[-1], n_out[-1], quantizers[-1]
        b = torch.arange(B)
        a_map = (b * N + st + n_s - 1).to(torch.int32)
        lay.head_maps[(s, (n_s - 1) % Q)] = (a_map.to(device), b.to(torch.int32).to(device), B)
        return lay
    for s, (st, n_s, Q) in enumerate(zip(starts, n_out, quantizers)):
        for qq in range(Q):
            js = torch.arange(qq, n_s, Q)
            if js.numel() == 0:
                continue
            b = torch.arange(B)[:, None]
            a_map = (b * N + st + js[None, :]).reshape(-1).to(torch.int32)
            c_map = (b * n_s + js[None, :]).reshape(-1).to(torch.int32)
            lay.head_maps[(s, qq)] = (a_map.to(device), c_map.to(device), int(a_map.numel()))
    return lay


def h16_operand(w: torch.Tensor, T: torch.dtype) -> torch.Tensor:
    sh = getattr(w, "_omlm_bf16", None)
    if (sh is not None and sh.dtype == T and getattr(w, "_omlm_bf16_version", -1) == w._version and sh.device == w.device):
        return sh
    c = torch.empty(w.shape, dtype=T, device=w.device)
    ops.cast_pad(w.detach(), c, w.numel() // w.shape[-1], w.shape[-1], w.shape[-1], w.shape[-1])
    return c


class PreparedWeights:
    def __init__(self, model, precision: str, persistent: bool = True):
        tr = model.transformer
        self.precision = precision
        self.T = _PRECISIONS[precision]
        self.ff3 = precision == "fp16ff"
        T = self.T
        dev = model.start_tokens[0].device
        D = tr.dim
        Fp_all = {ceil_to(ff.inner_dim, 64) for _, _, ff in tr.layers}
        self.ff_planes = self.ff3 and all(ff_planes_ok(f) for f in Fp_all)
        self.mx = self.ff_planes and all(ff_mx_ok(D, f) for f in Fp_all)
        quants = ops.QuantRowsGroup()
        self.layers = []
        wbuf = model.__dict__.setdefault("_omlm_wbuf", {})
        packs = ops.CastPadGroup()
        for li, (attn, _, ff) in enumerate(tr.layers):
            F = ff.inner_dim
            Fp = ceil_to(F, 64)
            w1 = ff.w_in.weight
            w2 = ff.w_out.weight
            ent = {}
            if T == torch.float32:
                ent["Wq"], ent["Wkv"], ent["Wo"] = attn.to_q.weight, attn.to_kv.weight, attn.to_out[0].weight
            else:
                for name, w in (("Wq", attn.to_q.weight), ("Wkv", attn.to_kv.weight), ("Wo", attn.to_out[0].weight)):
                    ent[name] = h16_operand(w, T)
            bkey = (li, T, str(dev), F, D)
            if not persistent:
                W1p, W2p, convp, gammap = (torch.zeros(2 * Fp, D, dtype=T, device=dev), torch.zeros(D, Fp, dtype=T, device=dev),
                                           torch.zeros(3, 2 * Fp, dtype=T, device=dev), torch.zeros(Fp, dtype=T, device=dev))
            else:
                if bkey not in wbuf:
                    wbuf[bkey] = (torch.zeros(2 * Fp, D, dtype=T, device=dev), torch.zeros(D, Fp, dtype=T, device=dev),
                                  torch.zeros(3, 2 * Fp, dtype=T, device=dev), torch.zeros(Fp, dtype=T, device=dev))
                W1p, W2p, convp, gammap = wbuf[bkey]
            packs.add(w1.detach(), W1p, F, D, D, D)
            packs.add(w1.detach()[F:], W1p[Fp:], F, D, D, D)
            packs.add(w2.detach(), W2p, D, F, F, Fp)
            ent["W1p"], ent["W2p"], ent["F"], ent["Fp"] = W1p, W2p, F, Fp
            if self.ff_planes:
                lkey = bkey + ("lo",)
                if not persistent or lkey not in wbuf:
                    lo = (torch.zeros(2 * Fp, D, dtype=T, device=dev), torch.zeros(D, Fp, dtype=T, device=dev),
                          torch.zeros(3, 2 * Fp, dtype=T, device=dev), torch.zeros(Fp, dtype=T, device=dev))
                    if persistent:
                        wbuf[lkey] = lo
                else:
                    lo = wbuf[lkey]
                W1l, W2l, convl, gammal = lo
                if not (self.mx and persistent):
                    packs.add(w1.detach(), W1l, F, D, D, D, lo=True)
                    packs.add(w1.detach()[F:], W1l[Fp:], F, D, D, D, lo=True)
                    packs.add(w2.detach(), W2l, D, F, F, Fp, lo=True)
                ent["W1p_lo"], ent["W2p_lo"], ent["convw_lo"], ent["gamma_mid_lo"] = W1l, W2l, convl, gammal
            if self.mx:
                mkey = bkey + ("mx",)
                if not persistent or mkey not in wbuf:
                    m8 = (ops.Fp8Planes(2 * Fp, D, dev), ops.Fp8Planes(D, Fp, dev))
                    if persistent:
                        wbuf[mkey] = m8
                else:
                    m8 = wbuf[mkey]
                quants.add(w1.detach(), m8[0], 0, F, D, D)
                quants.add(w1.detach()[F:], m8[0], Fp, F, D, D)
                quants.add(w2.detach(), m8[1], 0, D, F, F)
                ent["W1p8"], ent["W2p8"] = m8
            cw = ff.conv_weight().detach().reshape(2 * F, 3)
            packs.add(cw, convp, F, 3, 3, 2 * Fp, transpose=True)
            packs.add(cw[F:], convp[:, Fp:], F, 3, 3, 2 * Fp, transpose=True)
            packs.add(ff.norm_mid.gamma.detach(), gammap, 1, F, F, Fp)
            ent["convw"], ent["gamma_mid"] = convp, gammap
            if self.ff_planes:
                packs.add(cw, ent["convw_lo"], F, 3, 3, 2 * Fp, transpose=True, lo=True)
                packs.add(cw[F:], ent["convw_lo"][:, Fp:], F, 3, 3, 2 * Fp, transpose=True, lo=True)
                packs.add(ff.norm_mid.gamma.detach(), ent["gamma_mid_lo"], 1, F, F, Fp, lo=True)
            cache = ff.__dict__.setdefault("_omlm_cmap", {})
            if (F, Fp, str(dev)) not in cache:
                cm = torch.full((2 * Fp,), -1, dtype=torch.int32)
                cm[:F] = torch.arange(F, dtype=torch.int32)
                cm[Fp:Fp + F] = torch.arange(F, 2 * F, dtype=torch.int32)
                cache[(F, Fp, str(dev))] = cm.to(dev)
            ent["dW1_cmap"] = cache[(F, Fp, str(dev))]
            self.layers.append(ent)
        self.heads_lo = []
        if self.ff3:
            for w in model.logit_weights:
                lo = torch.empty(w.shape, dtype=T, device=dev)
                packs.add(w.detach().reshape(-1, D), lo.view(-1, D), w.numel() // D, D, D, D, lo=True)
                self.heads_lo.append(lo)
        packs.flush()
        quants.flush()
        self.heads = [w if T == torch.float32 else h16_operand(w, T) for w in model.logit_weights]


def prepared_weights(model, precision: str) -> PreparedWeights:
    key = (precision, sum(p._version for p in model.parameters()), tuple(p.data_ptr() for p in model.parameters()))
    cache = getattr(model, "_omlm_prepared", None)
    if cache is not None and cache[0] == key:
        return cache[1]
    pw = PreparedWeights(model, precision, persistent=False)
    object.__setattr__(model, "_omlm_prepared", (key, pw))
    return pw


class RelposStepCache:

    def __init__(self, tr):
        self.tr, self.enabled, self.valid = tr, False, False
        self.n, self.table, self.dtable, self.saved = None, None, None, None

    def __getstate__(self):
        return dict(tr=self.tr, enabled=False, valid=False, n=None, table=None, dtable=None, saved=None)

    def usable(self, n: int) -> bool:
        return self.enabled and self.valid and self.n == n

    def adopt(self, n: int, table: torch.Tensor, saved):
        self.n, self.table, self.saved = n, table, saved
        self.dtable = torch.zeros_like(table)
        self.valid = True

    def reset_accum(self):
        if self.dtable is not None:
            self.dtable.zero_()

    def refresh(self):
        if not self.enabled or self.n is None:
            return
        table, saved = relpos_forward(self.tr, self.n, True, prefix_rows(self.tr))
        self.table.copy_(table)
        self.saved = saved
        self.dtable.zero_()
        self.valid = True

    def flush(self):
        if self.enabled and self.valid and self.n is not None:
            relpos_backward(self.tr, self.n, self.saved, self.dtable)
        self.valid = False


def relpos_step_cache(tr) -> "RelposStepCache":
    c = tr.__dict__.get("_omlm_relpos_cache")
    if c is None:
        c = tr.__dict__["_omlm_relpos_cache"] = RelposStepCache(tr)
    return c


def prefix_rows(tr) -> int:
    return int(getattr(tr, "non_causal_prefix_size", 0) or 0)


def relpos_rows(n: int, P: int = 0) -> Tuple[int, int]:
    x0 = -(min(P, n) - 1) if P > 0 else 0
    return n - x0, x0


def relpos_forward(tr, n: int, save: bool, P: int = 0):
    rp = tr.rel_pos_bias
    if rp is None:
        return None, None
    H = tr.heads
    ldb = ceil_to(H, 8)
    dev = tr.norm.gamma.device
    rows, x0 = relpos_rows(n, P)
    if tr.relative_position_bias_type == "t5":
        from .transformer import t5_bucket_of_distance
        bucket = t5_bucket_of_distance(torch.arange(x0, n, device=dev), rp.num_buckets, rp.max_distance)
        table = torch.zeros(rows, ldb, device=dev, dtype=torch.float32)
        table[:, :H] = rp.relative_attention_bias.weight.detach()[bucket]
        return table, ("t5", bucket)
    lin = [rp.net[0][0], rp.net[1][0], rp.net[2][0], rp.net[3]]
    Hd = lin[0].weight.shape[0]
    if Hd in (256, 512) and H <= 16 and len(rp.net) == 4:
        saves = [torch.empty(rows, Hd, device=dev) for _ in range(6)] if save else None
        table = torch.empty(rows, ldb, device=dev)
        ops.relpos_mlp_fwd(lin[0].weight.detach().reshape(-1), lin[0].bias.detach(), lin[1].weight.detach(), lin[1].bias.detach(),
                           lin[2].weight.detach(), lin[2].bias.detach(), lin[3].weight.detach(), lin[3].bias.detach(), saves, table, rows, Hd, H, ldb,
                           x0=x0)
        return table, (("mlp_fused", saves) if save else None)
    n = rows
    pres, zs = [], []
    pre = torch.empty(n, Hd, device=dev)
    z = torch.empty(n, Hd, device=dev)
    ops.relpos_first_fwd(lin[0].weight.detach().reshape(-1), lin[0].bias.detach(), pre, z, n, Hd, x0=x0)
    pres.append(pre); zs.append(z)
    for k in (1, 2):
        a = torch.empty(n, Hd, device=dev)
        ops.gemm(zs[-1], lin[k].weight.detach(), a, M=n, N=Hd, K=Hd, planes=False)
        pre = torch.empty(n, Hd, device=dev)
        z = torch.empty(n, Hd, device=dev)
        ops.bias_silu_fwd(a, lin[k].bias.detach(), pre, z, n, Hd)
        pres.append(pre); zs.append(z)
    a = torch.zeros(n, ldb, device=dev)
    ops.gemm(zs[-1], lin[3].weight.detach(), a, M=n, N=H, K=Hd, ldc=ldb)
    table = torch.empty(n, ldb, device=dev)
    ops.bias_add(a, lin[3].bias.detach(), table, n, H, ldb)
    return table, (("mlp", pres, zs) if save else None)


def relpos_backward(tr, n: int, saved, dtable: torch.Tensor):
    rp = tr.rel_pos_bias
    H = tr.heads
    ldb = dtable.shape[-1]
    dev = dtable.device
    x0 = n - dtable.shape[0]
    n = dtable.shape[0]
    if saved[0] == "t5":
        g = grad_of(rp.relative_attention_bias.weight)
        g.index_add_(0, saved[1], dtable[:, :H])
        return
    lin = [rp.net[0][0], rp.net[1][0], rp.net[2][0], rp.net[3]]
    Hd = lin[0].weight.shape[0]
    if saved[0] == "mlp_fused":
        scratch = torch.empty(3 * n * Hd, device=dev)
        grads = [grad_of(lin[0].weight).view(-1), grad_of(lin[0].bias), grad_of(lin[1].weight), grad_of(lin[1].bias),
                 grad_of(lin[2].weight), grad_of(lin[2].bias), grad_of(lin[3].weight), grad_of(lin[3].bias)]
        ops.relpos_mlp_bwd(dtable, lin[1].weight.detach(), lin[2].weight.detach(), lin[3].weight.detach(), saved[1], scratch, grads, n, Hd, H, ldb,
                           x0=x0)
        return
    _, pres, zs = saved
    ops.colsum_accumulate(dtable, grad_of(lin[3].bias), n, H, ldb)
    gw = grad_of(lin[3].weight)
    ops.gemm(dtable, zs[2], gw, M=H, N=Hd, K=n, a_kmajor=True, b_kmajor=True, Cin=gw, lda=ldb)
    dz = torch.empty(n, Hd, device=dev)
    ops.gemm(dtable, lin[3].weight.detach(), dz, M=n, N=Hd, K=ldb, b_kmajor=True, lda=ldb, b_rows=H)
    for k in (2, 1):
        ds = torch.empty(n, Hd, device=dev)
        ops.silu_bwd(dz, pres[k], ds, n * Hd)
        ops.colsum_accumulate(ds, grad_of(lin[k].bias), n, Hd, Hd)
        gw = grad_of(lin[k].weight)
        ops.gemm(ds, zs[k - 1], gw, M=Hd, N=Hd, K=n, a_kmajor=True, b_kmajor=True, Cin=gw, planes=False)
        dz = torch.zeros(n, Hd, device=dev)
        ops.gemm(ds, lin[k].weight.detach(), dz, M=n, N=Hd, K=Hd, b_kmajor=True, Cin=dz, planes=False)
    ds = torch.empty(n, Hd, device=dev)
    ops.silu_bwd(dz, pres[0], ds, n * Hd)
    ops.colsum_accumulate(ds, grad_of(lin[0].bias), n, Hd, Hd)
    ops.relpos_first_bwd(ds, grad_of(lin[0].weight).view(-1), n, Hd, x0=x0)


class LayerSaved:
    __slots__ = ("x", "m1", "r1", "xn", "xc", "q_raw", "kv_raw", "q", "k", "v", "o", "lse", "abias",
                 "x1", "m2", "r2", "xn2", "h1", "h2", "m3", "r3", "seed", "p", "drop_bits", "gh", "h1_lo_tail",
                 "pa", "sa", "po", "so")


def _dropout_state(tr, dev):
    st = tr.__dict__.get("_omlm_dropout")
    if st is None or st["counter"].device != dev:
        rank = int(os.environ.get("RANK", "0"))
        g = torch.Generator().manual_seed((int(torch.initial_seed()) + 0x9E3779B1 * rank) & 0x7FFFFFFF)
        L = len(tr.layers)
        st = dict(counter=torch.zeros(1, dtype=torch.int64, device=dev),
                  seeds=[int(v) for v in torch.randint(1, 2 ** 62, (L,), generator=g)])
        a = [int(v) for v in torch.randint(1, 2 ** 62, (2 * L,), generator=g)]
        st["attn_seeds"], st["out_seeds"] = a[:L], a[L:]
        st["last"] = None
        tr.__dict__["_omlm_dropout"] = st
    return st


def dropout_salt(tr, dev) -> torch.Tensor:
    st = _dropout_state(tr, dev)
    st["counter"].add_(1)
    st["last"] = st["counter"].clone()
    return st["last"], st["seeds"]


def dropout_state(tr, dev=None) -> dict:
    st = tr.__dict__.get("_omlm_dropout")
    if st is None:
        st = _dropout_state(tr, dev if dev is not None else torch.device("cpu"))
    last = st["last"]
    return dict(ff=list(st["seeds"]), attn=list(st["attn_seeds"]), out=list(st["out_seeds"]),
                salt=int(last.item()) if last is not None else None)


def trunk_forward(tr, pw: PreparedWeights, x: torch.Tensor, keymask: Optional[torch.Tensor], B: int, N: int,
                  save: bool, training: bool, keep_h1_lo_tail: bool = False):
    T = pw.T
    dev = x.device
    M, D = x.shape
    H = tr.heads
    P = prefix_rows(tr)
    rc = tr.__dict__.get("_omlm_relpos_cache")
    if rc is not None and save and training and rc.usable(N):
        table, rp_saved = rc.table, ("cached", rc)
    else:
        table, rp_saved = relpos_forward(tr, N, save, P)
        if (rc is not None and rc.enabled and rc.n is None and save and training and rp_saved is not None and rp_saved[0] != "t5"
                and not torch.cuda.is_current_stream_capturing()):
            rc.adopt(N, table, rp_saved)
            rp_saved = ("cached", rc)
    saved_layers: List[LayerSaved] = []
    abiases = None
    salt, seeds, aseeds, oseeds = (None, None, None, None)
    aps = [(float(a_.attn_dropout.p), float(a_.to_out[1].p)) if training else (0.0, 0.0) for a_, _, _ in tr.layers]
    if training and (any(float(ff.dropout_p) > 0 for _, _, ff in tr.layers) or any(pa > 0 or po > 0 for pa, po in aps)):
        salt, seeds = dropout_salt(tr, dev)
        st_ = tr.__dict__["_omlm_dropout"]
        aseeds, oseeds = st_["attn_seeds"], st_["out_seeds"]
    for li, ((attn, _, ff), w) in enumerate(zip(tr.layers, pw.layers)):
        sv = LayerSaved()
        F, Fp = w["F"], w["Fp"]
        m1 = torch.empty(M, device=dev); r1 = torch.empty(M, device=dev)
        xn = torch.empty(M, D, dtype=T, device=dev)
        xc = x if T == torch.float32 else torch.empty(M, D, dtype=T, device=dev)
        ops.layernorm_fwd(x, attn.norm.gamma.detach(), xn, None if T == torch.float32 else xc, m1, r1)
        q = torch.empty(M, H * DIM_HEAD, dtype=T, device=dev)
        k = torch.empty(M, DIM_HEAD, dtype=T, device=dev)
        v = torch.empty(M, DIM_HEAD, dtype=T, device=dev)
        fused_qk = T in _H16
        if fused_qk:
            qn = torch.empty(M, H, device=dev)
            kn = torch.empty(M, device=dev)
            q_raw, kv_raw = qn, kn
            ops.gemm_qknorm(xn, w["Wq"], q, attn.q_scale.detach(), qn, H, M=M, N=H * DIM_HEAD, K=D)
            ops.gemm_qknorm(xc, w["Wkv"], k, attn.k_scale.detach(), kn, 1, M=M, N=2 * DIM_HEAD, K=D, C2=v, c2_col0=DIM_HEAD)
        else:
            q_raw = torch.empty(M, H * DIM_HEAD, device=dev)
            kv_raw = torch.empty(M, 2 * DIM_HEAD, device=dev)
            ops.gemm(xn, w["Wq"], q_raw, M=M, N=H * DIM_HEAD, K=D)
            ops.gemm(xc, w["Wkv"], kv_raw, M=M, N=2 * DIM_HEAD, K=D)
            ops.qk_norm_fwd(q_raw, kv_raw, attn.q_scale.detach(), attn.k_scale.detach(), q, k, v, H)
        o = torch.empty(M, H * DIM_HEAD, dtype=T, device=dev)
        lse = torch.empty(B, H, N, device=dev)
        if abiases is None:
            abiases = ops.AttnBias.group(table, N, H, dev, [a_.q_scale.detach() for a_, _, _ in tr.layers],
                                         [a_.k_scale.detach() for a_, _, _ in tr.layers], scale=ATTN_SCALE, half=T == torch.float16, P=P)
        abias = abiases[li]
        pa, po = aps[li]
        sa = aseeds[li] if pa > 0 else 0
        so = oseeds[li] if po > 0 else 0
        if P > 0:
            ops.attn_fwd_prefix(q, k, v, abias, keymask, o, lse, B, N, H, ATTN_SCALE, P, p=pa, seed=sa, seed_dev=salt if pa > 0 else None)
        else:
            ops.attn_fwd(q, k, v, abias, keymask, o, lse, B, N, H, ATTN_SCALE, p=pa, seed=sa, seed_dev=salt if pa > 0 else None)
        x1 = torch.empty(M, D, device=dev)
        if po > 0:
            yo = torch.empty(M, D, device=dev)
            ops.gemm(o, w["Wo"], yo, M=M, N=D, K=H * DIM_HEAD)
            ops.dropout_residual_fwd(x, yo, x1, po, so, seed_dev=salt)
            del yo
        else:
            ops.gemm(o, w["Wo"], x1, M=M, N=D, K=H * DIM_HEAD, Cin=x)
        m2 = torch.empty(M, device=dev); r2 = torch.empty(M, device=dev)
        xn2 = torch.empty(M, D, dtype=T, device=dev)
        h1 = torch.empty(M, 2 * Fp, dtype=T, device=dev)
        if pw.mx:
            P1 = ops.Fp8Planes(M, D, dev, zero=False)
            ops.layernorm_fwd_mx(x1, ff.norm_in.gamma.detach(), xn2, P1, m2, r2)
            h1_lo = torch.empty(M, 2 * Fp, dtype=torch.uint8, device=dev)
            ops.gemm_mx16(xn2, P1, w["W1p"], w["W1p8"], h1, h1_lo, M=M, N=2 * Fp, K=D)
        elif pw.ff_planes:
            xn2_lo = torch.empty(M, D, dtype=T, device=dev)
            ops.layernorm_fwd_planes(x1, ff.norm_in.gamma.detach(), xn2, xn2_lo, m2, r2)
            h1_lo = torch.empty(M, 2 * Fp, dtype=T, device=dev)
            ops.gemm_planes16(xn2, xn2_lo, w["W1p"], w["W1p_lo"], h1, h1_lo, M=M, N=2 * Fp, K=D)
        else:
            ops.layernorm_fwd(x1, ff.norm_in.gamma.detach(), xn2, None, m2, r2)
            ops.gemm(xn2, w["W1p"], h1, M=M, N=2 * Fp, K=D)
        h2 = torch.empty(M, Fp, dtype=T, device=dev)
        m3 = torch.empty(M, device=dev); r3 = torch.empty(M, device=dev)
        p = float(ff.dropout_p) if training else 0.0
        seed = seeds[li] if (p > 0 and seeds is not None) else 0
        drop_bits = torch.empty(M, Fp // 8, dtype=torch.uint8, device=dev) if (p > 0 and (save or pw.ff_planes)) else None
        gh = torch.empty(M, Fp, dtype=T, device=dev) if save else None
        x2 = torch.empty(M, D, device=dev)
        if pw.ff_planes:
            if pw.mx:
                P2 = ops.Fp8Planes(M, Fp, dev, zero=False)
                ops.ffmid_fwd_mx(h1, h1_lo, w["convw"], w["convw_lo"], w["gamma_mid"], w["gamma_mid_lo"], h2, P2, m3, r3, N, F, Fp, p, seed,
                                 seed_dev=salt if p > 0 else None, drop_bits=drop_bits, gh=gh)
                ops.gemm_mx16(h2, P2, w["W2p"], w["W2p8"], x2, M=M, N=D, K=Fp, Cin=x1)
            else:
                h2_lo = torch.empty(M, Fp, dtype=T, device=dev)
                ops.ffmid_fwd_planes(h1, h1_lo, w["convw"], w["convw_lo"], w["gamma_mid"], w["gamma_mid_lo"], h2, h2_lo, m3, r3, N, F, Fp, p, seed,
                                     seed_dev=salt if p > 0 else None, drop_bits=drop_bits, gh=gh)
                ops.gemm_planes16(h2, h2_lo, w["W2p"], w["W2p_lo"], x2, M=M, N=D, K=Fp, Cin=x1)
                del xn2_lo, h2_lo
            if keep_h1_lo_tail and save:
                take = min(2, N)
                sv.h1_lo_tail = torch.zeros(B, 2, 2 * Fp, device=dev)
                tail = h1_lo.view(B, N, -1)[:, N - take:]
                if tail.dtype == torch.uint8:
                    tail = (tail.contiguous().to(torch.int16) << 8).view(torch.float16)
                sv.h1_lo_tail[:, 2 - take:].copy_(tail)
            del h1_lo
        else:
            ops.ffmid_fwd(h1, w["convw"], w["gamma_mid"], h2, m3, r3, N, F, Fp, p, seed, seed_dev=salt if p > 0 else None,
                          drop_bits=drop_bits, gh=gh)
            ops.gemm(h2, w["W2p"], x2, M=M, N=D, K=Fp, Cin=x1)
        if save:
            sv.x, sv.m1, sv.r1, sv.xn, sv.xc = x, m1, r1, xn, xc
            sv.q_raw, sv.kv_raw, sv.q, sv.k, sv.v, sv.o, sv.lse, sv.abias = q_raw, kv_raw, q, k, v, o, lse, abias
            sv.x1, sv.m2, sv.r2, sv.xn2, sv.h1, sv.h2, sv.m3, sv.r3, sv.seed, sv.p = x1, m2, r2, xn2, h1, h2, m3, r3, seed, p
            sv.drop_bits = drop_bits
            sv.gh = gh
            sv.pa, sv.sa, sv.po, sv.so = pa, sa, po, so
            saved_layers.append(sv)
        x = x2
    mf = torch.empty(M, device=dev); rf = torch.empty(M, device=dev)
    y = torch.empty(M, D, dtype=T, device=dev)
    if pw.ff3:
        y_lo = torch.empty(M, D, dtype=T, device=dev)
        ops.layernorm_fwd_planes(x, tr.norm.gamma.detach(), y, y_lo, mf, rf)
        y._omlm_lo = y_lo
    else:
        ops.layernorm_fwd(x, tr.norm.gamma.detach(), y, None, mf, rf)
    saved = dict(layers=saved_layers, xL=x, mf=mf, rf=rf, table=table, rp=rp_saved, keymask=keymask, salt=salt) if save else None
    return y, saved


def trunk_backward(tr, pw: PreparedWeights, saved, dy: torch.Tensor, B: int, N: int, out_scale: float, head_wgrads=None):
    T = pw.T
    dev = dy.device
    M, D = dy.shape
    H = tr.heads
    table, keymask = saved["table"], saved["keymask"]
    rp_cached = saved["rp"] is not None and saved["rp"][0] == "cached"
    dtable = (saved["rp"][1].dtable if rp_cached else torch.zeros_like(table)) if table is not None else None
    nl = len(saved["layers"])
    dres = torch.empty(M, D, device=dev)
    dres_c = dres if T == torch.float32 else torch.empty(M, D, dtype=T, device=dev)
    cg = ops.ColsumGroup()
    ops.layernorm_bwd(dy, saved["xL"], tr.norm.gamma.detach(), saved["mf"], saved["rf"], None, dres,
                      None if T == torch.float32 else dres_c, grad_of(tr.norm.gamma),
                      dx_scale=out_scale if nl == 0 else 1.0, defer=cg)
    ws = None
    wg = ops.WgradGroup() if T in _H16 else None
    for dYh, Xh, dWh, Mo, No in (head_wgrads or []):
        if wg is not None:
            wg.add(dYh, Xh, dWh, M=Mo, N=No, K=dYh.shape[0])
        else:
            ops.gemm(dYh, Xh, dWh, M=Mo, N=No, K=dYh.shape[0], a_kmajor=True, b_kmajor=True, Cin=dWh)

    def wgrad(dY, X, dW, Mo, No, c_map=None):
        if wg is not None:
            wg.add(dY, X, dW, M=Mo, N=No, K=M, c_map=c_map)
            if len(wg.items) >= 40:
                wg.flush()
        else:
            ops.gemm(dY, X, dW, M=Mo, N=No, K=M, a_kmajor=True, b_kmajor=True, Cin=dW, c_map=c_map)

    for li in range(nl - 1, -1, -1):
        attn, _, ff = tr.layers[li]
        w, sv = pw.layers[li], saved["layers"][li]
        F, Fp = w["F"], w["Fp"]
        dh2 = torch.empty(M, Fp, dtype=T, device=dev)
        ops.gemm(dres_c, w["W2p"], dh2, M=M, N=Fp, K=D, b_kmajor=True)
        gW2 = grad_of(ff.w_out.weight)
        wgrad(dres_c, sv.h2, gW2, D, F)
        if ws is None or ws.numel() < ops.ffmid_bwd_workspace_floats(F, Fp):
            ws = torch.empty(ops.ffmid_bwd_workspace_floats(F, Fp), device=dev)
        du = torch.empty(M, 2 * Fp, dtype=T, device=dev)
        dh1 = torch.empty(M, 2 * Fp, dtype=T, device=dev)
        gconv = grad_of(ff.conv_param()).view(-1) if ff.conv_param() is not None else None
        ops.ffmid_bwd(dh2, sv.h1, w["convw"], w["gamma_mid"], sv.m3, sv.r3, du, dh1,
                      grad_of(ff.norm_mid.gamma), gconv, ws, N, F, Fp, sv.p, sv.seed,
                      seed_dev=saved["salt"] if sv.p > 0 else None, drop_bits=sv.drop_bits, gh=sv.gh)
        del du, dh2
        dxn2 = torch.empty(M, D, dtype=T, device=dev)
        ops.gemm(dh1, w["W1p"], dxn2, M=M, N=D, K=2 * Fp, b_kmajor=True)
        gW1 = grad_of(ff.w_in.weight)
        wgrad(dh1, sv.xn2, gW1, 2 * Fp, D, c_map=w["dW1_cmap"])
        del dh1
        dx1 = torch.empty(M, D, device=dev)
        dx1_c = dx1 if T == torch.float32 else torch.empty(M, D, dtype=T, device=dev)
        ops.layernorm_bwd(dxn2, sv.x1, ff.norm_in.gamma.detach(), sv.m2, sv.r2, dres, dx1,
                          None if T == torch.float32 else dx1_c, grad_of(ff.norm_in.gamma), defer=cg)
        dyo = dx1_c
        if sv.po > 0:
            dyo = torch.empty(M, D, dtype=T, device=dev)
            ops.dropout_residual_bwd(dx1, dyo, sv.po, sv.so, seed_dev=saved["salt"])
        do = torch.empty(M, H * DIM_HEAD, dtype=T, device=dev)
        ops.gemm(dyo, w["Wo"], do, M=M, N=H * DIM_HEAD, K=D, b_kmajor=True)
        gWo = grad_of(attn.to_out[0].weight)
        wgrad(dyo, sv.o, gWo, D, H * DIM_HEAD)
        dq = torch.empty(M, H * DIM_HEAD, device=dev)
        dkv = torch.empty(2, M, DIM_HEAD, device=dev)
        dk, dv = dkv[0], dkv[1]
        delta = torch.empty(B, H, N, device=dev)
        P = prefix_rows(tr)
        if P > 0:
            ops.attn_bwd_prefix(sv.q, sv.k, sv.v, sv.abias, keymask, sv.o, do, sv.lse, delta, dq, dk, dv, dtable, B, N, H, ATTN_SCALE, P,
                                p=sv.pa, seed=sv.sa, seed_dev=saved["salt"] if sv.pa > 0 else None)
        else:
            ops.attn_bwd(sv.q, sv.k, sv.v, sv.abias, keymask, sv.o, do, sv.lse, delta, dq, dk, dv, dtable, B, N, H, ATTN_SCALE,
                         p=sv.pa, seed=sv.sa, seed_dev=saved["salt"] if sv.pa > 0 else None)
        dq_raw = torch.empty(M, H * DIM_HEAD, dtype=T, device=dev)
        dkv_raw = torch.empty(M, 2 * DIM_HEAD, dtype=T, device=dev)
        if T in _H16:
            ops.qk_norm_bwd2(dq, dk, dv, sv.q, sv.k, sv.q_raw, sv.kv_raw, attn.q_scale.detach(), attn.k_scale.detach(),
                             dq_raw, dkv_raw, grad_of(attn.q_scale), grad_of(attn.k_scale), H)
        else:
            ops.qk_norm_bwd(dq, dk, dv, sv.q_raw, sv.kv_raw, attn.q_scale.detach(), attn.k_scale.detach(),
                            dq_raw, dkv_raw, grad_of(attn.q_scale), grad_of(attn.k_scale), H)
        dxn = torch.empty(M, D, dtype=T, device=dev)
        kv16 = T in _H16
        tmp = torch.empty(M, D, dtype=T if kv16 else torch.float32, device=dev)
        ops.gemm(dq_raw, w["Wq"], dxn, M=M, N=D, K=H * DIM_HEAD, b_kmajor=True)
        ops.gemm(dkv_raw, w["Wkv"], tmp, M=M, N=D, K=2 * DIM_HEAD, b_kmajor=True, Cin=None if kv16 else dx1)
        gWq = grad_of(attn.to_q.weight)
        wgrad(dq_raw, sv.xn, gWq, H * DIM_HEAD, D)
        gWkv = grad_of(attn.to_kv.weight)
        wgrad(dkv_raw, sv.xc, gWkv, 2 * DIM_HEAD, D)
        dres = torch.empty(M, D, device=dev)
        dres_c = dres if T == torch.float32 else torch.empty(M, D, dtype=T, device=dev)
        last = li == 0
        ops.layernorm_bwd(dxn, sv.x, attn.norm.gamma.detach(), sv.m1, sv.r1, dx1 if kv16 else tmp, dres,
                          None if (T == torch.float32 or last) else dres_c, grad_of(attn.norm.gamma),
                          dx_scale=out_scale if last else 1.0, dres2=tmp if kv16 else None, defer=cg)
    cg.flush()
    if wg is not None:
        wg.flush()
    if dtable is not None and saved["rp"] is not None and not rp_cached:
        relpos_backward(tr, N, saved["rp"], dtable)
    return dres


def build_ids(model, all_token_ids: Sequence[torch.Tensor]) -> Tuple[torch.Tensor, List[int]]:
    parts, lens = [], []
    for seq, ids in zip(model.token_sequences, all_token_ids):
        ids = ids.reshape(ids.shape[0], -1)
        if seq.num_quantizers > 1:
            off = seq.codebook_size * (torch.arange(ids.shape[-1], device=ids.device) % seq.num_quantizers)
            ids = ids + off
        lens.append(ids.shape[-1])
        parts += [torch.full((ids.shape[0], 1), -2, device=ids.device, dtype=torch.int32), ids.to(torch.int32)]
    return torch.cat(parts, dim=1).contiguous(), lens


class PreparedIds:
    __slots__ = ("ids32", "lens")

    def __init__(self, ids32: torch.Tensor, lens: Sequence[int]):
        self.ids32, self.lens = ids32, list(lens)


def get_layout(model, B: int, lens: Sequence[int], device, final_rows_only: bool) -> SeqLayout:
    cache = model.__dict__.setdefault("_omlm_layouts", {})
    key = (B, tuple(lens), str(device), final_rows_only)
    if key not in cache:
        if len(cache) > 64:
            cache.clear()
        cache[key] = build_layout(B, lens, [s.num_quantizers for s in model.token_sequences], device, final_rows_only)
    return cache[key]


def embed_forward(model, ids32: torch.Tensor, lay: SeqLayout) -> torch.Tensor:
    B, N = ids32.shape
    D = model.dim
    x = torch.empty(B * N, D, device=ids32.device)
    pos = [e.weight.detach() for e in model.absolute_position_embeddings] if model.use_absolute_position_embeddings else None
    ops.embed_fwd(ids32, lay.seg, lay.posidx, [e.weight.detach() for e in model.embeddings],
                  [s.detach() for s in model.start_tokens], pos, x.view(B, N, D))
    return x


def embed_backward(model, ids32: torch.Tensor, lay: SeqLayout, dx: torch.Tensor, alpha: float):
    B, N = ids32.shape
    dpos = [grad_of(e.weight) for e in model.absolute_position_embeddings] if model.use_absolute_position_embeddings else None
    ops.embed_bwd(ids32, lay.seg, lay.posidx, [grad_of(e.weight) for e in model.embeddings],
                  [grad_of(s) for s in model.start_tokens], dpos, dx.view(B, N, -1), alpha)


def heads_forward(model, pw: PreparedWeights, y: torch.Tensor, lay: SeqLayout, want: Sequence[bool]):
    D = model.dim
    out = []
    y_lo = y.__dict__.pop("_omlm_lo", None) if pw.ff3 else None
    for s, seq in enumerate(model.token_sequences):
        if not want[s]:
            out.append(None)
            continue
        V1 = seq.codebook_size + 1
        ldV = ceil_to(V1, 8)
        n_s = lay.n_out[s]
        buf = torch.empty(lay.B if lay.final_only else lay.B * n_s, ldV, device=y.device)
        for qq in range(seq.num_quantizers):
            ent = lay.head_maps.get((s, qq))
            if ent is None:
                continue
            a_map, c_map, rows = ent
            if y_lo is not None:
                ops.gemm_planes16(y, y_lo, pw.heads[s][qq], pw.heads_lo[s][qq], buf, M=rows, N=V1, K=D, a_map=a_map, c_map=c_map, ldc=ldV,
                                  a_rows=y.shape[0], b_rows=V1)
                continue
            ops.gemm(y, pw.heads[s][qq], buf, M=rows, N=V1, K=D, a_map=a_map, c_map=c_map, ldc=ldV,
                     a_rows=y.shape[0], b_rows=V1)
        out.append(buf)
    return out


def heads_backward(model, pw: PreparedWeights, y: torch.Tensor, lay: SeqLayout, dlogits: Sequence[Optional[torch.Tensor]],
                   deferred: Optional[list] = None):
    D = model.dim
    dy = torch.zeros(y.shape[0], D, device=y.device)
    for s, seq in enumerate(model.token_sequences):
        dl = dlogits[s]
        if dl is None:
            continue
        V1 = seq.codebook_size + 1
        ldV = dl.shape[-1]
        gW = grad_of(model.logit_weights[s])
        for qq in range(seq.num_quantizers):
            ent = lay.head_maps.get((s, qq))
            if ent is None:
                continue
            a_map, c_map, rows = ent
            ops.gemm(dl, pw.heads[s][qq], dy, M=rows, N=D, K=ldV, b_kmajor=True, a_map=c_map, c_map=a_map,
                     a_rows=dl.shape[0], b_rows=V1)
            if deferred is not None and rows >= 1024:
                rp = ceil_to(rows, 64)
                gd = torch.empty(rp, dl.shape[-1], dtype=dl.dtype, device=dl.device)
                gy = torch.empty(rp, y.shape[-1], dtype=y.dtype, device=y.device)
                torch.index_select(dl, 0, c_map, out=gd[:rows])
                torch.index_select(y, 0, a_map, out=gy[:rows])
                if rp > rows:
                    gd[rows:].zero_(); gy[rows:].zero_()
                deferred.append((gd, gy, gW[qq], V1, D))
                continue
            ops.gemm(dl, y, gW[qq], M=V1, N=D, K=rows, a_kmajor=True, b_kmajor=True, a_map=c_map, b_map=a_map,
                     Cin=gW[qq], lda=ldV, a_rows=dl.shape[0], b_rows=y.shape[0])
    return dy


class ForwardState:
    __slots__ = ("model", "pw", "ids32", "lay", "trunk", "y", "B", "N", "logits", "labels", "lse_rows", "coefs")


def run_forward(model, all_token_ids, self_attn_mask, only_final: bool, save: bool, precision: str,
                want: Optional[Sequence[bool]] = None, final_rows_only: bool = False):
    tr = model.transformer
    require_gpu(model.start_tokens[0], "model parameters")
    ops.planes_begin()
    if isinstance(all_token_ids, PreparedIds):
        ids32, lens = all_token_ids.ids32, all_token_ids.lens
    else:
        ids32, lens = build_ids(model, all_token_ids)
    require_gpu(ids32, "token ids")
    B, N = ids32.shape
    lay = get_layout(model, B, lens, ids32.device, final_rows_only)
    pw = prepared_weights(model, precision) if not save else PreparedWeights(model, precision)
    keymask = None
    if self_attn_mask is not None:
        assert self_attn_mask.shape == (B, N), f"self_attn_mask must be [{B}, {N}]"
        keymask = self_attn_mask.to(torch.uint8).contiguous()
    x = embed_forward(model, ids32, lay)
    y, tsaved = trunk_forward(tr, pw, x, keymask, B, N, save, model.training)
    nseq = len(model.token_sequences)
    if want is None:
        want = [(not only_final) or s == nseq - 1 for s in range(nseq)]
    logits = heads_forward(model, pw, y, lay, want)
    st = None
    if save:
        st = ForwardState()
        st.model, st.pw, st.ids32, st.lay, st.trunk, st.y, st.B, st.N, st.logits = model, pw, ids32, lay, tsaved, y, B, N, logits
    else:
        ops.planes_end()
    return logits, lay, st


def run_backward(st: ForwardState, dlogits: Sequence[Optional[torch.Tensor]]):
    model = st.model
    deferred = [] if st.pw.T in _H16 else None
    dy = heads_backward(model, st.pw, st.y, st.lay, dlogits, deferred)
    alpha = float(model.transformer.grad_shrink_alpha)
    dx = trunk_backward(model.transformer, st.pw, st.trunk, dy, st.B, st.N, out_scale=alpha, head_wgrads=deferred)
    embed_backward(model, st.ids32, st.lay, dx, 1.0)
    ops.planes_end()


def logits_views(model, lay: SeqLayout, bufs):
    out = []
    for s, (seq, buf) in enumerate(zip(model.token_sequences, bufs)):
        if buf is None:
            out.append(None)
        else:
            out.append(buf.view(lay.B, -1, buf.shape[-1])[:, :, : seq.codebook_size + 1])
    return out


class LogitsFunction(torch.autograd.Function):

    @staticmethod
    def forward(ctx, model, all_token_ids, self_attn_mask, only_final, precision, *params):
        bufs, lay, st = run_forward(model, all_token_ids, self_attn_mask, only_final, True, precision)
        ctx.set_materialize_grads(False)
        ctx.st = st
        ctx.nparams = len(params)
        ctx.ls = loss_scale_state(model) if is_half(precision) else None
        views = logits_views(model, lay, bufs)
        ctx.present = [v is not None for v in views]
        return tuple(v for v in views if v is not None)

    @staticmethod
    def backward(ctx, *grads):
        st = ctx.st
        T = st.pw.T
        gi = iter(grads)
        dl = []
        for s, (seq, present) in enumerate(zip(st.model.token_sequences, ctx.present)):
            g = next(gi) if present else None
            if g is None:
                dl.append(None)
                continue
            V1 = seq.codebook_size + 1
            ldV = ceil_to(V1, 8)
            g2 = g.reshape(-1, V1).to(torch.float32).contiguous()
            if ctx.ls is not None:
                g2 = g2 * ctx.ls[0:1]
            d = torch.empty(g2.shape[0], ldV, dtype=T, device=g2.device)
            ops.cast_pad(g2, d, g2.shape[0], V1, V1, ldV)
            dl.append(d)
        run_backward(st, dl)
        ctx.st = None
        return (None,) * (5 + ctx.nparams)


class LossFunction(torch.autograd.Function):

    @staticmethod
    def forward(ctx, model, all_token_ids, labels, self_attn_mask, loss_weights, ignore_negative, precision, all_logits, *params):
        nseq = len(model.token_sequences)
        bufs, lay, st = run_forward(model, all_token_ids, self_attn_mask, False, True, precision,
                                    want=[bool(all_logits) or w > 0 for w in loss_weights])
        dev = next(b for b in bufs if b is not None).device
        total = 0
        total_dev = None
        nll = torch.zeros(nseq, device=dev)
        st.labels, st.lse_rows, st.coefs = [], [], []
        for s, (seq, buf, lb, w) in enumerate(zip(model.token_sequences, bufs, labels, loss_weights)):
            if w > 0:
                lb32 = lb.reshape(-1).to(torch.int32).contiguous()
                assert lb32.numel() == buf.shape[0], (lb32.numel(), buf.shape)
                lse_rows = torch.empty(buf.shape[0], device=dev)
                ops.ce_fwd(buf, lb32, lse_rows, nll[s:s + 1], seq.codebook_size + 1)
                if ignore_negative[s]:
                    cnt = (lb32 >= 0).sum().to(torch.float32)
                    total_dev = cnt if total_dev is None else total_dev + cnt
                else:
                    total += lb32.numel()
                st.labels.append(lb32); st.lse_rows.append(lse_rows)
            else:
                st.labels.append(None); st.lse_rows.append(None)
        loss = None
        if total_dev is None:
            for s, w in enumerate(loss_weights):
                if w > 0:
                    term = nll[s] * (float(w) / float(total))
                    loss = term if loss is None else loss + term
            st.coefs = [float(w) / float(total) if w > 0 else 0.0 for w in loss_weights]
            ctx.inv_total = None
        else:
            inv_total = 1.0 / (total_dev + float(total))
            for s, w in enumerate(loss_weights):
                if w > 0:
                    term = nll[s] * float(w)
                    loss = term if loss is None else loss + term
            loss = loss * inv_total
            st.coefs = [float(w) if w > 0 else 0.0 for w in loss_weights]
            ctx.inv_total = inv_total
        ctx.st = st
        ctx.nparams = len(params)
        ctx.ls = loss_scale_state(model) if is_half(precision) else None
        views = logits_views(model, lay, bufs)
        ctx.mark_non_differentiable(*[v for v in views if v is not None])
        return (loss, *views)

    @staticmethod
    def backward(ctx, gloss, *unused):
        st = ctx.st
        T = st.pw.T
        g = gloss.reshape(1).to(torch.float32).contiguous()
        if ctx.inv_total is not None:
            g = (g * ctx.inv_total).reshape(1).contiguous()
        if ctx.ls is not None:
            g = (g * ctx.ls[0:1]).contiguous()
        dl = []
        for s, seq in enumerate(st.model.token_sequences):
            if st.labels[s] is None:
                dl.append(None)
                continue
            buf = st.logits[s]
            d = torch.empty(buf.shape[0], buf.shape[1], dtype=T, device=buf.device)
            ops.ce_bwd(buf, st.labels[s], st.lse_rows[s], g, st.coefs[s], d, seq.codebook_size + 1)
            dl.append(d)
        run_backward(st, dl)
        ctx.st = None
        return (None,) * (8 + ctx.nparams)
```

### open_musiclm_amd/hip.py

```python
from __future__ import annotations

import ctypes as C
import os
from typing import Optional

import torch

_HERE = os.path.dirname(os.path.abspath(__file__))
LIB_PATH = os.environ.get("OMLM_LIB_PATH") or os.path.join(_HERE, "libomlm_hip.so")

_lib: Optional[C.CDLL] = None

vp, i32, i64, f32, u64 = C.c_void_p, C.c_int, C.c_longlong, C.c_float, C.c_ulonglong

SIGNATURES = {
    "omlm_version": [],
    "omlm_last_error": [],
    "omlm_set_error": [C.c_char_p],
    "omlm_gemm": [vp, vp, vp, vp, vp, vp, vp, i64, i64, i32, i32, i32, i32, i32, i32, i32, i32, i32, i32, i32, f32, vp, i64, vp],
    "omlm_gemm_tail_workspace_bytes": [i32, i32],
    "omlm_gemm_wgrad_group": [vp, i32, i32, i32, vp],
    "omlm_gemm_planes": [vp, i64, vp, i64, vp, vp, vp, vp, vp, i64, i64, i32, i32, i32, i32, i32, i32, i32, i32, i32, i32, f32, vp, i64, vp],
    "omlm_split_planes": [vp, vp, i64, i64, vp],
    "omlm_gemm_planes16": [vp, vp, vp, vp, vp, vp, vp, vp, vp, i64, i64, i32, i32, i32, i32, i32, i32, i32, i32, vp, i64, vp],
    "omlm_gemm_mx16": [vp, vp, i64, vp, vp, vp, i64, vp, vp, vp, i32, vp, i64, i64, i32, i32, i32, i32, i32, i32, i32, vp, i64, vp],
    "omlm_gemm_mx16_workspace_bytes": [i32, i32, i32],
    "omlm_layernorm_fwd_mx": [vp, vp, vp, vp, i64, vp, vp, vp, i32, i32, i32, f32, vp],
    "omlm_ffmid_fwd_mx": [vp, vp, vp, vp, vp, vp, vp, vp, i64, vp, vp, vp, i32, i32, i32, i32, f32, f32, u64, vp, vp, vp, vp],
    "omlm_quant_rows_mx": [vp, i32, vp],
    "omlm_layernorm_fwd_planes": [vp, vp, vp, vp, vp, vp, i32, i32, i32, f32, i32, vp],
    "omlm_ffmid_fwd_planes": [vp, vp, vp, vp, vp, vp, vp, vp, vp, vp, i32, i32, i32, i32, f32, f32, u64, vp, vp, vp, i32, vp],
    "omlm_layernorm_fwd": [vp, vp, vp, vp, vp, vp, i32, i32, i32, f32, i32, vp],
    "omlm_layernorm_bwd_workspace_bytes": [i32],
    "omlm_layernorm_bwd": [vp, vp, vp, vp, vp, vp, vp, vp, vp, vp, i32, i32, f32, i32, i32, vp],
    "omlm_layernorm_bwd2": [vp, vp, vp, vp, vp, vp, vp, vp, vp, vp, vp, i32, i32, f32, i32, i32, vp],
    "omlm_qk_norm_fwd": [vp, vp, vp, vp, vp, vp, vp, i32, i32, i32, vp],
    "omlm_qk_norm_bwd": [vp, vp, vp, vp, vp, vp, vp, vp, vp, vp, vp, i32, i32, i32, vp],
    "omlm_gemm_qknorm": [vp, vp, vp, vp, i32, i32, vp, vp, i32, i32, i64, i64, i32, i32, i32, i32, i32, i32, i32, vp],
    "omlm_qk_norm_bwd2": [vp, vp, vp, vp, vp, vp, vp, vp, vp, vp, vp, vp, vp, i32, i32, i32, vp],
    "omlm_attn_bias_table_floats": [i32, i32],
    "omlm_attn_bias_prepare": [vp, vp, i32, i32, i32, vp, vp, f32, f32, i32, vp],
    "omlm_attn_bias_prepare_group": [vp, vp, i32, i32, i32, i32, vp, vp, f32, f32, i32, vp],
    "omlm_mqa_attn_fwd": [vp, vp, vp, vp, vp, vp, vp, vp, i32, i32, i32, f32, i32, i32, vp],
    "omlm_mqa_attn_bwd": [vp, vp, vp, vp, vp, vp, vp, vp, vp, vp, vp, vp, vp, vp, vp, i32, i32, i32, f32, i32, i32, vp],
    "omlm_mqa_attn_bwd_workspace_bytes": [i32, i32, i32],
    "omlm_mqa_attn_fwd_dropout": [vp, vp, vp, vp, vp, vp, vp, vp, i32, i32, i32, f32, i32, i32, f32, u64, vp, vp],
    "omlm_mqa_attn_bwd_dropout": [vp, vp, vp, vp, vp, vp, vp, vp, vp, vp, vp, vp, vp, vp, vp, i32, i32, i32, f32, i32, i32, f32, u64, vp, vp],
    "omlm_mqa_attn_fwd_prefix": [vp] * 8 + [i32, i32, i32, f32, i32, i32, i32, f32, u64, vp, vp],
    "omlm_mqa_attn_bwd_prefix": [vp] * 15 + [i32, i32, i32, f32, i32, i32, i32, f32, u64, vp, vp],
    "omlm_attn_bias_table_floats_prefix": [i32, i32, i32],
    "omlm_attn_bias_prepare_group_prefix": [vp, vp, i32, i32, i32, i32, vp, vp, f32, f32, i32, i32, vp],
    "omlm_attn_dropout_keep": [vp, i32, i32, i32, f32, u64, vp, vp],
    "omlm_dropout_residual_fwd": [vp, vp, vp, i64, i32, f32, u64, vp, vp],
    "omlm_dropout_residual_bwd": [vp, vp, i64, i32, f32, u64, vp, i32, vp],
    "omlm_ffmid_fwd": [vp, vp, vp, vp, vp, vp, i32, i32, i32, i32, f32, f32, u64, vp, vp, vp, i32, vp],
    "omlm_ffmid_bwd_workspace_bytes": [i32, i32],
    "omlm_ffmid_bwd": [vp, vp, vp, vp, vp, vp, vp, vp, vp, vp, vp, i32, i32, i32, i32, f32, u64, vp, vp, vp, i32, vp],
    "omlm_colsum_accumulate": [vp, vp, i32, i32, i32, vp],
    "omlm_colsum_group": [vp, i32, vp],
    "omlm_ffmid_set_impl": [i32],
    "omlm_embed_gather_fwd": [vp, vp, vp, vp, vp, vp, i32, vp, i32, i32, i32, vp, vp, vp, vp],
    "omlm_embed_gather_bwd": [vp, vp, vp, vp, vp, vp, i32, vp, i32, i32, i32, f32, vp, vp, vp, vp],
    "omlm_prepare_train_batch": [vp, vp, vp, vp, vp, vp, i32, i32, i32, vp, i32, vp, vp, i32, vp],
    "omlm_cross_entropy_fwd": [vp, vp, vp, vp, i32, i32, i32, vp, vp],
    "omlm_cross_entropy_bwd": [vp, vp, vp, vp, f32, vp, i32, i32, i32, i32, i32, vp],
    "omlm_sumsq_accumulate": [vp, i64, vp, vp, vp],
    "omlm_adamw_clip_step": [vp, vp, vp, vp, vp, i64, f32, f32, f32, f32, f32, i32, f32, vp, f32, i32, i32, i32, vp, vp],
    "omlm_loss_scale_update": [vp, vp, f32, f32, i32, f32, f32, vp],
    "omlm_cast_pad": [vp, vp, i64, i32, i32, i32, i32, vp],
    "omlm_transpose_cast": [vp, vp, i32, i32, i32, i32, i32, vp],
    "omlm_cast_pad_group": [vp, i32, i32, vp],
    "omlm_sample_topk_gumbel_at": [vp, vp, vp, vp, vp, i32, i32, i32, i32, f32, i32, vp],
    "omlm_sample_embed_at": [vp, vp, vp, vp, vp, i32, i32, i32, i32, f32, i32, vp, i64, i64, vp, i32, vp],
    "omlm_decode_step": [vp, vp, vp],
    "omlm_decode_advance": [vp, vp, vp],
    "omlm_relpos_first_fwd": [vp, vp, vp, vp, i32, i32, vp],
    "omlm_relpos_first_bwd": [vp, vp, i32, i32, vp],
    "omlm_bias_silu_fwd": [vp, vp, vp, vp, i64, i32, vp],
    "omlm_silu_bwd": [vp, vp, vp, i64, vp],
    "omlm_bias_add": [vp, vp, vp, i32, i32, i32, vp],
    "omlm_relpos_mlp_fwd": [vp] * 15 + [i32, i32, i32, i32, vp],
    "omlm_relpos_mlp_bwd": [vp] * 19 + [i32, i32, i32, i32, vp],
    "omlm_relpos_first_fwd_from": [vp, vp, vp, vp, i32, i32, i32, vp],
    "omlm_relpos_first_bwd_from": [vp, vp, i32, i32, i32, vp],
    "omlm_relpos_mlp_fwd_from": [vp] * 15 + [i32, i32, i32, i32, i32, vp],
    "omlm_relpos_mlp_bwd_from": [vp] * 19 + [i32, i32, i32, i32, i32, vp],
    "omlm_rvq_encode": [vp, vp, vp, vp, i32, i32, i32, i32, vp],
    "omlm_nearest_centroid": [vp, vp, vp, i32, i32, i32, vp],
    "omlm_rvq_encode_strided": [vp, vp, vp, i32, vp, i32, i32, i32, vp],
    "omlm_vq_accumulate": [vp, vp, i32, vp, vp, i32, i32, i32, vp],
    "omlm_vq_kmeans_update": [vp, vp, vp, vp, i32, i32, vp],
    "omlm_vq_ema_update": [vp, vp, vp, vp, vp, vp, vp, i32, i32, f32, f32, vp],
    "omlm_sample_topk_gumbel": [vp, vp, vp, i32, i32, i32, i32, f32, i32, vp],
    "omlm_probe_tr16": [vp, vp],
}
_RESTYPES = {"omlm_last_error": C.c_char_p, "omlm_gemm_tail_workspace_bytes": C.c_longlong, "omlm_gemm_mx16_workspace_bytes": C.c_longlong, "omlm_ffmid_bwd_workspace_bytes": C.c_longlong,
             "omlm_attn_bias_table_floats": C.c_longlong, "omlm_attn_bias_table_floats_prefix": C.c_longlong, "omlm_mqa_attn_bwd_workspace_bytes": C.c_longlong,
             "omlm_layernorm_bwd_workspace_bytes": C.c_longlong, "omlm_set_error": None}


class HipLibraryMissing(RuntimeError):
    pass


def lib() -> C.CDLL:
    global _lib
    if _lib is None:
        if not os.path.exists(LIB_PATH):
            raise HipLibraryMissing(
                f"{LIB_PATH} not found: build it with `python -c 'import __graft_entry__ as g; g.build()'` "
                "(or `make -C open_musiclm_amd/csrc`). There is no CPU fallback for the MI355X hot path.")
        l = C.CDLL(LIB_PATH)
        for name, args in SIGNATURES.items():
            fn = getattr(l, name)
            fn.argtypes = args
            fn.restype = _RESTYPES.get(name, C.c_int)
        _lib = l
    return _lib


def stream_ptr() -> int:
    return torch.cuda.current_stream().cuda_stream


def ptr(t: Optional[torch.Tensor]):
    if t is None:
        return None
    return t.data_ptr()


def call(name: str, *args):
    rc = getattr(lib(), name)(*args)
    if rc != 0:
        msg = lib().omlm_last_error()
        raise RuntimeError(f"{name} failed (rc={rc}): {msg.decode() if msg else '?'}")


def require_gpu(t: torch.Tensor, what: str = "tensor"):
    if not t.is_cuda:
        raise RuntimeError(
            f"open_musiclm_amd: {what} is on {t.device}; the TokenConditionedTransformer path only runs on an "
            "MI355X through libomlm_hip.so (no CPU fallback). Move the model and inputs to 'cuda'.")
    cur = torch.cuda.current_device()
    if t.device.index != cur:
        raise RuntimeError(f"open_musiclm_amd: {what} lives on cuda:{t.device.index} but the current device is cuda:{cur}; "
                           "call torch.cuda.set_device(LOCAL_RANK) and keep the model and its inputs on that device")
```

### open_musiclm_amd/ops.py

```python
from __future__ import annotations

import ctypes as C
import os
import weakref
from typing import Optional, Sequence

import torch

from . import hip
from .hip import call, ptr, stream_ptr

F32, BF16, F16 = 0, 1, 2
_CODES = {torch.float32: F32, torch.bfloat16: BF16, torch.float16: F16}
H16 = (torch.bfloat16, torch.float16)


def dcode(dtype: torch.dtype) -> int:
    try:
        return _CODES[dtype]
    except KeyError:
        raise TypeError(f"unsupported operand dtype {dtype}") from None


def tdtype(code: int) -> torch.dtype:
    return {F32: torch.float32, BF16: torch.bfloat16, F16: torch.float16}[code]


def _chk(t: torch.Tensor, name: str):
    hip.require_gpu(t, name)
    if not t.is_contiguous():
        raise ValueError(f"{name} must be contiguous")


_X3_PLANES = os.environ.get("OMLM_X3_PLANES", "1") == "1"
_X3_MIN_MACS = 1 << 26
_PLANES = {}
_PLANE_SCOPE = [0]


def planes_begin():
    _PLANES.clear()
    _PLANE_SCOPE[0] = 1


def planes_end():
    _PLANES.clear()
    _PLANE_SCOPE[0] = 0


def operand_planes(t: torch.Tensor, rows: int, ld: int):
    n = int(rows) * int(ld)
    key = id(t)
    scoped = _PLANE_SCOPE[0] > 0
    if scoped:
        ent = _PLANES.get(key)
        if ent is not None and ent[0]() is t and ent[1] == t._version and ent[2] == (t.data_ptr(), n):
            return ent[3], ent[4]
    pe = (n + 7) // 8 * 8
    buf = torch.empty(2 * pe, dtype=torch.bfloat16, device=t.device)
    call("omlm_split_planes", ptr(t), ptr(buf), n, pe, stream_ptr())
    if scoped:
        try:
            ref = weakref.ref(t, lambda _r, k=key: _PLANES.pop(k, None))
            _PLANES[key] = (ref, t._version, (t.data_ptr(), n), buf, pe * 2)
        except TypeError:
            pass
    return buf, pe * 2


_TAIL_WS = {}
_TAIL_WS_BYTES = int(os.environ.get("OMLM_GEMM_TAIL_WS_MB", "64")) << 20


def tail_workspace(device: torch.device):
    if _TAIL_WS_BYTES <= 0:
        return None, 0
    idx = device.index if device.index is not None else torch.cuda.current_device()
    key = (idx, torch.cuda.current_stream(device).cuda_stream)
    buf = _TAIL_WS.get(key)
    if buf is None:
        buf = _TAIL_WS[key] = torch.empty(_TAIL_WS_BYTES // 4, device=device)
    return ptr(buf), _TAIL_WS_BYTES


def gemm(A: torch.Tensor, B: torch.Tensor, C_: torch.Tensor, *, M: int, N: int, K: int,
         lda: Optional[int] = None, ldb: Optional[int] = None, ldc: Optional[int] = None,
         a_kmajor: bool = False, b_kmajor: bool = False, Cin: Optional[torch.Tensor] = None,
         ldcin: Optional[int] = None, a_map=None, b_map=None, c_map=None, alpha: float = 1.0,
         a_rows: Optional[int] = None, b_rows: Optional[int] = None, planes: bool = True):
    hip.require_gpu(A, "A")
    assert A.dtype == B.dtype, (A.dtype, B.dtype)
    lda = lda if lda is not None else A.shape[-1]
    ldb = ldb if ldb is not None else B.shape[-1]
    ldc = ldc if ldc is not None else C_.shape[-1]
    if Cin is not None:
        assert Cin.dtype == torch.float32
        ldcin = ldcin if ldcin is not None else Cin.shape[-1]
    a_rows = a_rows if a_rows is not None else A.numel() // lda
    b_rows = b_rows if b_rows is not None else B.numel() // ldb
    ws, wsb = tail_workspace(A.device) if (A.dtype in H16 or A.dtype == torch.float32) else (None, 0)
    if (A.dtype == torch.float32 and planes and _X3_PLANES and M * N * K >= _X3_MIN_MACS and not (a_kmajor and a_map is not None)
            and not (b_kmajor and b_map is not None) and (a_kmajor and b_kmajor or K % 8 == 0)):
        pa, sa = operand_planes(A, a_rows, lda)
        pb, sb = operand_planes(B, b_rows, ldb)
        call("omlm_gemm_planes", ptr(pa), sa, ptr(pb), sb, ptr(C_), ptr(Cin), ptr(a_map), ptr(b_map), ptr(c_map),
             a_rows, b_rows, M, N, K, lda, ldb, ldc, ldcin or 0, int(a_kmajor), int(b_kmajor), dcode(C_.dtype), float(alpha),
             ws, wsb, stream_ptr())
        return
    call("omlm_gemm", ptr(A), ptr(B), ptr(C_), ptr(Cin), ptr(a_map), ptr(b_map), ptr(c_map),
         a_rows, b_rows, M, N, K, lda, ldb, ldc, ldcin or 0, int(a_kmajor), int(b_kmajor),
         dcode(A.dtype), dcode(C_.dtype), float(alpha), ws, wsb, stream_ptr())


def gemm_planes16(A, A_lo, B, B_lo, C_, C_lo=None, *, M: int, N: int, K: int, Cin: Optional[torch.Tensor] = None, a_map=None, c_map=None,
                  ldc: Optional[int] = None, a_rows: Optional[int] = None, b_rows: Optional[int] = None):
    hip.require_gpu(A, "A")
    assert A.dtype in H16 and A_lo.dtype == A.dtype and B.dtype == A.dtype and B_lo.dtype == A.dtype
    assert A_lo.shape == A.shape and B_lo.shape == B.shape
    if C_lo is None:
        assert C_.dtype == torch.float32 and (Cin is None or Cin.dtype == torch.float32)
    else:
        assert C_.dtype == A.dtype and C_lo.dtype == A.dtype and C_lo.shape == C_.shape and Cin is None
    lda, ldb = A.shape[-1], B.shape[-1]
    ldc = ldc if ldc is not None else C_.shape[-1]
    ws, wsb = tail_workspace(A.device)
    call("omlm_gemm_planes16", ptr(A), ptr(A_lo), ptr(B), ptr(B_lo), ptr(C_), ptr(C_lo), ptr(Cin), ptr(a_map), ptr(c_map),
         a_rows if a_rows is not None else A.numel() // lda, b_rows if b_rows is not None else B.numel() // ldb,
         M, N, K, lda, ldb, ldc, Cin.shape[-1] if Cin is not None else 0, dcode(A.dtype), ws, wsb, stream_ptr())


class Fp8Planes:
    __slots__ = ("planes", "scale", "rows", "ld")

    def __init__(self, rows: int, ld: int, device, zero: bool = True):
        self.rows, self.ld = int(rows), int(ld)
        rp = (self.rows + 255) // 256 * 256
        self.planes = (torch.zeros if zero else torch.empty)(2, rp, 2 * self.ld, dtype=torch.uint8, device=device)
        self.scale = (torch.full((rp,), 127, dtype=torch.uint8, device=device) if zero else torch.empty(rp, dtype=torch.uint8, device=device))

    @property
    def stride(self) -> int:
        return self.planes.shape[1] * self.planes.shape[2]


def gemm_mx16(A, A8: Fp8Planes, B, B8: Fp8Planes, C_, C_lo=None, *, M: int, N: int, K: int, Cin: Optional[torch.Tensor] = None):
    hip.require_gpu(A, "A")
    assert A.dtype == torch.float16 and B.dtype == torch.float16
    lda, ldb = A.shape[-1], B.shape[-1]
    assert A8.ld == lda and B8.ld == ldb and A8.rows >= M and B8.rows >= N
    if C_lo is None:
        assert C_.dtype == torch.float32 and (Cin is None or Cin.dtype == torch.float32)
    else:
        assert C_.dtype == A.dtype and C_lo.dtype in (A.dtype, torch.uint8) and C_lo.shape == C_.shape and Cin is None
    ws, wsb = tail_workspace(A.device)
    call("omlm_gemm_mx16", ptr(A), ptr(A8.planes), A8.stride, ptr(A8.scale), ptr(B), ptr(B8.planes), B8.stride, ptr(B8.scale),
         ptr(C_), ptr(C_lo), int(C_lo is not None and C_lo.dtype == torch.uint8), ptr(Cin), A.numel() // lda, B.numel() // ldb, M, N, K, lda, ldb, C_.shape[-1],
         Cin.shape[-1] if Cin is not None else 0, ws, wsb, stream_ptr())


class _WgradDesc(C.Structure):
    _fields_ = [("A", C.c_void_p), ("B", C.c_void_p), ("C", C.c_void_p), ("c_map", C.c_void_p),
                ("M", C.c_int), ("N", C.c_int), ("K", C.c_int), ("lda", C.c_int), ("ldb", C.c_int), ("ldc", C.c_int)]


class WgradGroup:

    def __init__(self):
        self.items = []
        self.dtype = None

    def add(self, dY: torch.Tensor, X: torch.Tensor, dW: torch.Tensor, *, M: int, N: int, K: int, c_map=None):
        hip.require_gpu(dY, "dY")
        assert dY.dtype in H16 and X.dtype == dY.dtype and dW.dtype == torch.float32
        assert self.dtype in (None, dY.dtype), "one operand type per group"
        self.dtype = dY.dtype
        self.items.append((dY, X, dW, c_map, M, N, K, dY.shape[-1], X.shape[-1], dW.shape[-1]))

    def flush(self, splits: int = 0):
        n = len(self.items)
        if n == 0:
            return
        arr = (_WgradDesc * n)()
        for d, (dY, X, dW, c_map, M, N, K, lda, ldb, ldc) in zip(arr, self.items):
            d.A, d.B, d.C, d.c_map = ptr(dY), ptr(X), ptr(dW), ptr(c_map)
            d.M, d.N, d.K, d.lda, d.ldb, d.ldc = M, N, K, lda, ldb, ldc
        call("omlm_gemm_wgrad_group", C.cast(arr, C.c_void_p), n, int(splits), dcode(self.dtype), stream_ptr())
        self.items = []


class _CastDesc(C.Structure):
    _fields_ = [("src", C.c_void_p), ("dst", C.c_void_p), ("R", C.c_int), ("C", C.c_int), ("ld_src", C.c_int), ("ld_dst", C.c_int),
                ("transpose", C.c_int), ("lo", C.c_int)]


class CastPadGroup:

    def __init__(self):
        self.items, self.dtype = [], None

    def add(self, src, dst, R, C_, ld_src, ld_dst, transpose=False, lo=False):
        hip.require_gpu(src, "src")
        assert src.dtype == torch.float32 and self.dtype in (None, dst.dtype), "fp32 sources, one output type per group"
        self.dtype = dst.dtype
        self.items.append((src, dst, int(R), int(C_), int(ld_src), int(ld_dst), int(bool(transpose)), int(bool(lo))))

    def flush(self):
        n = len(self.items)
        if n == 0:
            return
        arr = (_CastDesc * n)()
        for d, (src, dst, R, C_, ld_src, ld_dst, tr, lo) in zip(arr, self.items):
            d.src, d.dst, d.R, d.C, d.ld_src, d.ld_dst, d.transpose, d.lo = ptr(src), ptr(dst), R, C_, ld_src, ld_dst, tr, lo
        call("omlm_cast_pad_group", C.cast(arr, C.c_void_p), n, dcode(self.dtype), stream_ptr())
        self.items = []


def layernorm_fwd(x, gamma, y, xcast, mean, rstd, eps=1e-5):
    M, D = x.shape
    call("omlm_layernorm_fwd", ptr(x), ptr(gamma), ptr(y), ptr(xcast), ptr(mean), ptr(rstd),
         M, D, y.shape[-1], float(eps), dcode(y.dtype), stream_ptr())


def layernorm_fwd_planes(x, gamma, y, y_lo, mean, rstd, eps=1e-5):
    M, D = x.shape
    assert y.dtype in H16 and y_lo.dtype == y.dtype and y_lo.shape == y.shape
    call("omlm_layernorm_fwd_planes", ptr(x), ptr(gamma), ptr(y), ptr(y_lo), ptr(mean), ptr(rstd),
         M, D, y.shape[-1], float(eps), dcode(y.dtype), stream_ptr())


def layernorm_fwd_mx(x, gamma, y, P: "Fp8Planes", mean, rstd, eps=1e-5):
    M, D = x.shape
    assert y.dtype == torch.float16 and P.ld == y.shape[-1] and P.rows >= M
    call("omlm_layernorm_fwd_mx", ptr(x), ptr(gamma), ptr(y), ptr(P.planes), P.stride, ptr(P.scale), ptr(mean), ptr(rstd),
         M, D, y.shape[-1], float(eps), stream_ptr())


class _QuantDesc(C.Structure):
    _fields_ = [("src", C.c_void_p), ("dst8", C.c_void_p), ("lo_stride", C.c_longlong), ("scale8", C.c_void_p),
                ("R", C.c_int), ("C", C.c_int), ("ld_src", C.c_int), ("ld8", C.c_int)]


class QuantRowsGroup:

    def __init__(self):
        self.items = []

    def add(self, src, P: "Fp8Planes", row0: int, R: int, C_: int, ld_src: int):
        hip.require_gpu(src, "src")
        assert src.dtype == torch.float32 and row0 + R <= P.rows and C_ <= 2 * P.ld
        self.items.append((src, P, int(row0), int(R), int(C_), int(ld_src)))

    def flush(self):
        n = len(self.items)
        if n == 0:
            return
        arr = (_QuantDesc * n)()
        for d, (src, P, row0, R, C_, ld_src) in zip(arr, self.items):
            pitch = 2 * P.ld
            d.src, d.dst8, d.lo_stride, d.scale8 = ptr(src), P.planes.data_ptr() + row0 * pitch, P.stride, P.scale.data_ptr() + row0
            d.R, d.C, d.ld_src, d.ld8 = R, C_, ld_src, pitch
        call("omlm_quant_rows_mx", C.cast(arr, C.c_void_p), n, stream_ptr())
        self.items = []


_LN_WS = {}


def _ln_workspace(D: int, device) -> torch.Tensor:
    key = (D, str(device))
    if key not in _LN_WS:
        _LN_WS[key] = torch.empty(int(hip.lib().omlm_layernorm_bwd_workspace_bytes(D)) // 4, device=device)
    return _LN_WS[key]


class _ColsumDesc(C.Structure):
    _fields_ = [("part", C.c_void_p), ("out", C.c_void_p), ("P", C.c_int), ("C", C.c_int), ("ldp", C.c_int)]


class ColsumGroup:

    def __init__(self):
        self.items = []

    def add(self, part: torch.Tensor, out: torch.Tensor, P: int, C_: int, ldp: int):
        self.items.append((part, out, int(P), int(C_), int(ldp)))

    def flush(self):
        n = len(self.items)
        if n == 0:
            return
        arr = (_ColsumDesc * n)()
        for d, (part, out, P, C_, ldp) in zip(arr, self.items):
            d.part, d.out, d.P, d.C, d.ldp = ptr(part), ptr(out), P, C_, ldp
        call("omlm_colsum_group", C.cast(arr, C.c_void_p), n, stream_ptr())
        self.items = []


def layernorm_bwd(dy, x, gamma, mean, rstd, dres, dx, dxcast, dgamma, dx_scale=1.0, dres2=None, defer: Optional["ColsumGroup"] = None):
    M, D = x.shape
    code = dcode(dxcast.dtype) if dxcast is not None else (dcode(dres2.dtype) if dres2 is not None else F32)
    assert dres2 is None or dcode(dres2.dtype) == code, "dres2 must have the cast type"
    if dgamma is not None and defer is not None:
        rows = min(M, 2048)
        ws = torch.empty(rows * D, device=x.device)
        call("omlm_layernorm_bwd2", ptr(dy), ptr(x), ptr(gamma), ptr(mean), ptr(rstd), ptr(dres), ptr(dres2), ptr(dx),
             ptr(dxcast), None, ptr(ws), M, D, float(dx_scale), code, dcode(dy.dtype), stream_ptr())
        defer.add(ws, dgamma, rows, D, D)
        return
    ws = _ln_workspace(D, x.device) if dgamma is not None else None
    call("omlm_layernorm_bwd2", ptr(dy), ptr(x), ptr(gamma), ptr(mean), ptr(rstd), ptr(dres), ptr(dres2), ptr(dx),
         ptr(dxcast), ptr(dgamma), ptr(ws), M, D, float(dx_scale), code, dcode(dy.dtype), stream_ptr())


def qk_norm_fwd(q_raw, kv_raw, q_scale, k_scale, q, k, v, H):
    call("omlm_qk_norm_fwd", ptr(q_raw), ptr(kv_raw), ptr(q_scale), ptr(k_scale), ptr(q), ptr(k), ptr(v),
         q_raw.shape[0], H, dcode(q.dtype), stream_ptr())


def qk_norm_bwd(dq, dk, dv, q_raw, kv_raw, q_scale, k_scale, dq_raw, dkv_raw, dq_scale, dk_scale, H):
    call("omlm_qk_norm_bwd", ptr(dq), ptr(dk), ptr(dv), ptr(q_raw), ptr(kv_raw), ptr(q_scale), ptr(k_scale),
         ptr(dq_raw), ptr(dkv_raw), ptr(dq_scale), ptr(dk_scale), q_raw.shape[0], H, dcode(dq_raw.dtype), stream_ptr())


_DBIAS_WS = {}
_DBIAS_RETIRED = []


def gemm_qknorm(A, B, C_, scale, norm_out, groups, *, M, N, K, C2=None, c2_col0=0):
    hip.require_gpu(A, "A")
    assert A.dtype in H16 and B.dtype == A.dtype and C_.dtype == A.dtype and norm_out.dtype == torch.float32 and scale.dtype == torch.float32
    assert C2 is None or C2.dtype == A.dtype
    call("omlm_gemm_qknorm", ptr(A), ptr(B), ptr(C_), ptr(C2), int(c2_col0), C2.shape[-1] if C2 is not None else 0, ptr(scale), ptr(norm_out),
         norm_out.shape[-1] if norm_out.dim() > 1 else 1, int(groups), A.numel() // A.shape[-1], B.numel() // B.shape[-1], M, N, K,
         A.shape[-1], B.shape[-1], C_.shape[-1], dcode(A.dtype), stream_ptr())


def qk_norm_bwd2(dq, dk, dv, q, k, qn, kn, q_scale, k_scale, dq_raw, dkv_raw, dq_scale, dk_scale, H):
    call("omlm_qk_norm_bwd2", ptr(dq), ptr(dk), ptr(dv), ptr(q), ptr(k), ptr(qn), ptr(kn), ptr(q_scale), ptr(k_scale),
         ptr(dq_raw), ptr(dkv_raw), ptr(dq_scale), ptr(dk_scale), q.shape[0], H, dcode(dq_raw.dtype), stream_ptr())


class AttnBias:

    def __init__(self, table: Optional[torch.Tensor], N: int, H: int, device=None, q_scale=None, k_scale=None,
                 qk_bound: float = 0.0, scale: float = 8.0, half: bool = False, _tableT: Optional[torch.Tensor] = None):
        self.table, self.N, self.H = table, N, H
        dev = table.device if table is not None else device
        if _tableT is not None:
            self.tableT = _tableT
            return
        self.tableT = torch.empty(int(hip.lib().omlm_attn_bias_table_floats(N, H)), device=dev)
        call("omlm_attn_bias_prepare", ptr(table), ptr(self.tableT), N, H, table.shape[-1] if table is not None else 0,
             ptr(q_scale), ptr(k_scale), float(qk_bound), float(scale), 15 if half else 0, stream_ptr())

    @staticmethod
    def group(table: Optional[torch.Tensor], N: int, H: int, device, q_scales, k_scales, scale: float = 8.0, half: bool = False, P: int = 0):
        L = len(q_scales)
        dev = table.device if table is not None else device
        nfl = int(hip.lib().omlm_attn_bias_table_floats_prefix(N, H, P) if P > 0 else hip.lib().omlm_attn_bias_table_floats(N, H))
        buf = torch.empty(L, nfl, device=dev)
        outs = (C.c_void_p * L)(*[buf[l].data_ptr() for l in range(L)])
        qs = (C.c_void_p * L)(*[t.data_ptr() for t in q_scales])
        ks = (C.c_void_p * L)(*[t.data_ptr() for t in k_scales])
        for t in list(q_scales) + list(k_scales):
            hip.require_gpu(t, "scale")
        if P > 0:
            call("omlm_attn_bias_prepare_group_prefix", ptr(table), C.cast(outs, C.c_void_p), L, N, H, table.shape[-1] if table is not None else 0,
                 C.cast(qs, C.c_void_p), C.cast(ks, C.c_void_p), 0.0, float(scale), 15 if half else 0, int(P), stream_ptr())
        else:
            call("omlm_attn_bias_prepare_group", ptr(table), C.cast(outs, C.c_void_p), L, N, H, table.shape[-1] if table is not None else 0,
                 C.cast(qs, C.c_void_p), C.cast(ks, C.c_void_p), 0.0, float(scale), 15 if half else 0, stream_ptr())
        return [AttnBias(table, N, H, dev, _tableT=buf[l]) for l in range(L)]

    def dbias_workspace(self, B: int, N: int, H: int) -> torch.Tensor:
        n = int(hip.lib().omlm_mqa_attn_bwd_workspace_bytes(B, N, H)) // 4
        key = str(self.tableT.device)
        ws = _DBIAS_WS.get(key)
        if ws is None or ws.numel() < n:
            if ws is not None:
                _DBIAS_RETIRED.append(ws)
            ws = _DBIAS_WS[key] = torch.empty(n, device=self.tableT.device, dtype=torch.float32)
        return ws


def _attn_bias(bias, N, H, device) -> "AttnBias":
    return bias if isinstance(bias, AttnBias) else AttnBias(bias, N, H, device)


def attn_fwd(q, k, v, bias, keymask, out, lse, B, N, H, scale, p=0.0, seed=0, seed_dev=None):
    ab = _attn_bias(bias, N, H, q.device)
    if p > 0:
        call("omlm_mqa_attn_fwd_dropout", ptr(q), ptr(k), ptr(v), ptr(ab.table), ptr(ab.tableT), ptr(keymask), ptr(out), ptr(lse),
             B, N, H, float(scale), ab.table.shape[-1] if ab.table is not None else 0, dcode(q.dtype), float(p), int(seed),
             ptr(seed_dev), stream_ptr())
        return
    call("omlm_mqa_attn_fwd", ptr(q), ptr(k), ptr(v), ptr(ab.table), ptr(ab.tableT), ptr(keymask), ptr(out), ptr(lse),
         B, N, H, float(scale), ab.table.shape[-1] if ab.table is not None else 0, dcode(q.dtype), stream_ptr())


def attn_bwd(q, k, v, bias, keymask, out, dout, lse, delta, dq, dk, dv, dbias, B, N, H, scale, workspace=True, p=0.0, seed=0,
             seed_dev=None):
    ab = _attn_bias(bias, N, H, q.device)
    bias = ab.table
    ws = ab.dbias_workspace(B, N, H) if dbias is not None and workspace else None
    if p > 0:
        call("omlm_mqa_attn_bwd_dropout", ptr(q), ptr(k), ptr(v), ptr(bias), ptr(ab.tableT), ptr(keymask), ptr(out), ptr(dout), ptr(lse),
             ptr(delta), ptr(dq), ptr(dk), ptr(dv), ptr(dbias), ptr(ws), B, N, H, float(scale),
             bias.shape[-1] if bias is not None else 0, dcode(q.dtype), float(p), int(seed), ptr(seed_dev), stream_ptr())
        return
    call("omlm_mqa_attn_bwd", ptr(q), ptr(k), ptr(v), ptr(bias), ptr(ab.tableT), ptr(keymask), ptr(out), ptr(dout), ptr(lse),
         ptr(delta), ptr(dq), ptr(dk), ptr(dv), ptr(dbias), ptr(ws), B, N, H, float(scale),
         bias.shape[-1] if bias is not None else 0, dcode(q.dtype), stream_ptr())


def attn_fwd_prefix(q, k, v, bias, keymask, out, lse, B, N, H, scale, P, p=0.0, seed=0, seed_dev=None):
    table, tableT = (bias.table, bias.tableT) if isinstance(bias, AttnBias) else (bias, None)
    call("omlm_mqa_attn_fwd_prefix", ptr(q), ptr(k), ptr(v), ptr(table), ptr(tableT), ptr(keymask), ptr(out), ptr(lse), B, N, H, float(scale),
         table.shape[-1] if table is not None else 0, dcode(q.dtype), int(P), float(p), int(seed), ptr(seed_dev), stream_ptr())


def attn_bwd_prefix(q, k, v, bias, keymask, out, dout, lse, delta, dq, dk, dv, dtable, B, N, H, scale, P, workspace=True, p=0.0, seed=0,
                    seed_dev=None):
    table, tableT = (bias.table, bias.tableT) if isinstance(bias, AttnBias) else (bias, None)
    ws = None
    if dtable is not None and workspace:
        n = int(hip.lib().omlm_mqa_attn_bwd_workspace_bytes(B, N, H)) // 4
        key = str(q.device)
        ws = _DBIAS_WS.get(key)
        if ws is None or ws.numel() < n:
            if ws is not None:
                _DBIAS_RETIRED.append(ws)
            ws = _DBIAS_WS[key] = torch.empty(n, device=q.device, dtype=torch.float32)
    ld = table.shape[-1] if table is not None else (dtable.shape[-1] if dtable is not None else 0)
    call("omlm_mqa_attn_bwd_prefix", ptr(q), ptr(k), ptr(v), ptr(table), ptr(tableT), ptr(keymask), ptr(out), ptr(dout), ptr(lse), ptr(delta), ptr(dq),
         ptr(dk), ptr(dv), ptr(dtable), ptr(ws), B, N, H, float(scale), ld, dcode(q.dtype), int(P), float(p), int(seed), ptr(seed_dev),
         stream_ptr())


def attn_dropout_keep(B, N, H, p, seed, seed_dev=None, device=None) -> torch.Tensor:
    keep = torch.empty(B, H, N, N, dtype=torch.uint8, device=device if device is not None else seed_dev.device)
    call("omlm_attn_dropout_keep", ptr(keep), B, N, H, float(p), int(seed), ptr(seed_dev), stream_ptr())
    return keep


def dropout_residual_fwd(x, y, x1, p, seed, seed_dev=None):
    call("omlm_dropout_residual_fwd", ptr(x), ptr(y), ptr(x1), x.shape[0], x.shape[1], float(p), int(seed), ptr(seed_dev), stream_ptr())


def dropout_residual_bwd(dx1, dy, p, seed, seed_dev=None):
    call("omlm_dropout_residual_bwd", ptr(dx1), ptr(dy), dx1.shape[0], dx1.shape[1], float(p), int(seed), ptr(seed_dev), dcode(dy.dtype),
         stream_ptr())


def pack_conv_taps(convw: torch.Tensor, F: int, Fp: int) -> torch.Tensor:
    out = torch.zeros(3, 2 * Fp, device=convw.device, dtype=torch.float32)
    out[:, :F] = convw[:F].t()
    out[:, Fp:Fp + F] = convw[F:].t()
    return out


def pad_vector(v: torch.Tensor, n: int) -> torch.Tensor:
    out = torch.zeros(n, device=v.device, dtype=torch.float32)
    out[: v.numel()] = v
    return out


def ffmid_fwd(h1, convw, gamma, h2, mean, rstd, nseq, F, Fp, p, seed, eps=1e-5, seed_dev=None, drop_bits=None, gh=None):
    assert convw.shape == (3, 2 * Fp) and gamma.numel() == Fp
    assert convw.dtype == h1.dtype and gamma.dtype == h1.dtype, "taps / gamma travel in the operand dtype of h1"
    call("omlm_ffmid_fwd", ptr(h1), ptr(convw), ptr(gamma), ptr(h2), ptr(mean), ptr(rstd),
         h1.shape[0], nseq, F, Fp, float(eps), float(p), int(seed), ptr(seed_dev), ptr(drop_bits), ptr(gh), dcode(h1.dtype),
         stream_ptr())


def ffmid_fwd_planes(h1, h1_lo, convw, convw_lo, gamma, gamma_lo, h2, h2_lo, mean, rstd, nseq, F, Fp, p, seed, eps=1e-5, seed_dev=None,
                     drop_bits=None, gh=None):
    assert convw.shape == (3, 2 * Fp) and gamma.numel() == Fp and h1.dtype in H16
    for t in (h1_lo, convw, convw_lo, gamma, gamma_lo, h2, h2_lo):
        assert t.dtype == h1.dtype, "every plane travels in the operand dtype of h1"
    assert h1_lo.shape == h1.shape and h2_lo.shape == h2.shape and convw_lo.shape == convw.shape
    call("omlm_ffmid_fwd_planes", ptr(h1), ptr(h1_lo), ptr(convw), ptr(convw_lo), ptr(gamma), ptr(gamma_lo), ptr(h2), ptr(h2_lo), ptr(mean),
         ptr(rstd), h1.shape[0], nseq, F, Fp, float(eps), float(p), int(seed), ptr(seed_dev), ptr(drop_bits), ptr(gh), dcode(h1.dtype),
         stream_ptr())


def ffmid_fwd_mx(h1, h1_lo, convw, convw_lo, gamma, gamma_lo, h2, P: "Fp8Planes", mean, rstd, nseq, F, Fp, p, seed, eps=1e-5, seed_dev=None,
                 drop_bits=None, gh=None):
    assert convw.shape == (3, 2 * Fp) and gamma.numel() == Fp and h1.dtype == torch.float16 and h1_lo.dtype == torch.uint8
    for t in (convw, convw_lo, gamma, gamma_lo, h2):
        assert t.dtype == h1.dtype, "every plane travels in the operand dtype of h1"
    assert h1_lo.shape == h1.shape and convw_lo.shape == convw.shape and P.ld == Fp and P.rows >= h1.shape[0]
    call("omlm_ffmid_fwd_mx", ptr(h1), ptr(h1_lo), ptr(convw), ptr(convw_lo), ptr(gamma), ptr(gamma_lo), ptr(h2), ptr(P.planes), P.stride,
         ptr(P.scale), ptr(mean), ptr(rstd), h1.shape[0], nseq, F, Fp, float(eps), float(p), int(seed), ptr(seed_dev), ptr(drop_bits), ptr(gh),
         stream_ptr())


def ffmid_set_impl(impl: int):
    call("omlm_ffmid_set_impl", int(impl))


def ffmid_bwd_workspace_floats(F, Fp) -> int:
    return int(hip.lib().omlm_ffmid_bwd_workspace_bytes(F, Fp)) // 4


def ffmid_bwd(dh2, h1, convw, gamma, mean, rstd, du_tmp, dh1, dgamma, dconv, workspace, nseq, F, Fp, p, seed, seed_dev=None,
              drop_bits=None, gh=None):
    assert convw.shape == (3, 2 * Fp) and gamma.numel() == Fp
    assert convw.dtype == h1.dtype and gamma.dtype == h1.dtype, "taps / gamma travel in the operand dtype of h1"
    call("omlm_ffmid_bwd", ptr(dh2), ptr(h1), ptr(convw), ptr(gamma), ptr(mean), ptr(rstd), ptr(du_tmp), ptr(dh1),
         ptr(dgamma), ptr(dconv), ptr(workspace), h1.shape[0], nseq, F, Fp, float(p), int(seed), ptr(seed_dev), ptr(drop_bits),
         ptr(gh), dcode(h1.dtype), stream_ptr())


def _ptr_array(tensors: Sequence[Optional[torch.Tensor]]):
    arr = (C.c_void_p * len(tensors))()
    for i, t in enumerate(tensors):
        arr[i] = ptr(t) if t is not None else None
    return arr


_INDEX_ERR = {}


def index_error_flag(device) -> torch.Tensor:
    key = str(device)
    if key not in _INDEX_ERR:
        _INDEX_ERR[key] = torch.zeros(1, dtype=torch.int32, device=device)
    return _INDEX_ERR[key]


def raise_on_index_error(device):
    flag = _INDEX_ERR.get(str(device))
    if flag is None:
        return
    v = int(flag.item())
    if v:
        flag.zero_()
        what = [n for b, n in ((1, "token id >= embedding rows"), (2, "position >= absolute position rows"), (4, "label >= vocabulary")) if v & b]
        raise IndexError("open_musiclm_amd: " + ", ".join(what) + " (rows were skipped; check codebook sizes / the token store)")


def _rows_array(tensors):
    if tensors is None:
        return None
    return (C.c_longlong * len(tensors))(*[int(t.shape[0]) if t is not None else 0 for t in tensors])


def embed_fwd(ids, seg, posidx, tables, starts, pos_tables, out):
    B, N = ids.shape
    D = out.shape[-1]
    pos_arr = _ptr_array(pos_tables) if pos_tables is not None else None
    call("omlm_embed_gather_fwd", ptr(ids), ptr(seg), ptr(posidx), _ptr_array(tables), _ptr_array(starts),
         pos_arr, len(tables), ptr(out), B, N, D, _rows_array(tables), _rows_array(pos_tables), ptr(index_error_flag(out.device)),
         stream_ptr())


def embed_bwd(ids, seg, posidx, dtables, dstarts, dpos_tables, dx, alpha):
    B, N = ids.shape
    D = dx.shape[-1]
    pos_arr = _ptr_array(dpos_tables) if dpos_tables is not None else None
    call("omlm_embed_gather_bwd", ptr(ids), ptr(seg), ptr(posidx), _ptr_array(dtables), _ptr_array(dstarts),
         pos_arr, len(dtables), ptr(dx), B, N, D, float(alpha), _rows_array(dtables), _rows_array(dpos_tables),
         ptr(index_error_flag(dx.device)), stream_ptr())


def prepare_train_batch(raw_ids, eos_ids, quantizers, codebooks, pad_id, scores, n_drop, want_labels):
    n = len(raw_ids)
    B, dev = raw_ids[0].shape[0], raw_ids[0].device
    for t in raw_ids:
        hip.require_gpu(t, "token ids")
        assert t.dtype == torch.int64 and t.dim() == 2 and t.is_contiguous() and t.shape[0] == B
    lens = [int(t.shape[1]) for t in raw_ids]
    N = sum(l + 1 for l in lens) + (n - 1)
    ids32 = torch.empty(B, N, dtype=torch.int32, device=dev)
    keymask = torch.empty(B, N, dtype=torch.uint8, device=dev)
    labels = [torch.empty(B, l + 1, dtype=torch.int32, device=dev) if w else None for l, w in zip(lens, want_labels)]
    arr_i = lambda v: (C.c_int * n)(*[int(x) for x in v])
    call("omlm_prepare_train_batch", _ptr_array(raw_ids), _ptr_array(labels), arr_i(lens), arr_i(eos_ids), arr_i(quantizers), arr_i(codebooks),
         n, B, int(pad_id), ptr(scores), int(n_drop), ptr(ids32), ptr(keymask), N, stream_ptr())
    return ids32, keymask, labels, [l + 1 for l in lens[:-1]] + [lens[-1]]


def ce_fwd(logits, labels, row_lse, nll_sum, V):
    R, ld = logits.shape
    call("omlm_cross_entropy_fwd", ptr(logits), ptr(labels), ptr(row_lse), ptr(nll_sum), R, V, ld,
         ptr(index_error_flag(logits.device)), stream_ptr())


def ce_bwd(logits, labels, row_lse, gscale, coef, dlogits, V):
    R, ld = logits.shape
    call("omlm_cross_entropy_bwd", ptr(logits), ptr(labels), ptr(row_lse), ptr(gscale), float(coef), ptr(dlogits),
         R, V, ld, dlogits.shape[-1], dcode(dlogits.dtype), stream_ptr())


def sumsq_accumulate(g, out, partials=None):
    call("omlm_sumsq_accumulate", ptr(g), g.numel(), ptr(out), ptr(partials), stream_ptr())


def adamw_clip_step(p, g, m, v, p16, *, lr, beta1, beta2, eps, wd, step, gscale, gnorm_sq, max_norm,
                    decoupled, zero_grad, ls_state=None):
    call("omlm_adamw_clip_step", ptr(p), ptr(g), ptr(m), ptr(v), ptr(p16), p.numel(), float(lr), float(beta1),
         float(beta2), float(eps), float(wd), int(step), float(gscale), ptr(gnorm_sq), float(max_norm or 0.0),
         int(decoupled), int(zero_grad), dcode(p16.dtype) if p16 is not None else BF16, ptr(ls_state), stream_ptr())


def loss_scale_update(ls_state, gnorm_sq, *, growth=2.0, backoff=0.5, interval=2000, scale_min=1.0, scale_max=65536.0):
    call("omlm_loss_scale_update", ptr(ls_state), ptr(gnorm_sq), float(growth), float(backoff), int(interval), float(scale_min),
         float(scale_max), stream_ptr())


def cast_pad(src, dst, R, C_, ld_src, ld_dst):
    call("omlm_cast_pad", ptr(src), ptr(dst), R, C_, ld_src, ld_dst, dcode(dst.dtype), stream_ptr())


def transpose_cast(src, dst, R, C_, ld_src, ld_dst):
    call("omlm_transpose_cast", ptr(src), ptr(dst), R, C_, ld_src, ld_dst, dcode(dst.dtype), stream_ptr())


def colsum_accumulate(part, out, P, C_, ldp):
    call("omlm_colsum_accumulate", ptr(part), ptr(out), P, C_, ldp, stream_ptr())


def relpos_first_fwd(w0, b0, pre, z, n, Hd, x0=0):
    if x0:
        call("omlm_relpos_first_fwd_from", ptr(w0), ptr(b0), ptr(pre), ptr(z), n, Hd, int(x0), stream_ptr())
        return
    call("omlm_relpos_first_fwd", ptr(w0), ptr(b0), ptr(pre), ptr(z), n, Hd, stream_ptr())


def relpos_first_bwd(ds, dw0, n, Hd, x0=0):
    if x0:
        call("omlm_relpos_first_bwd_from", ptr(ds), ptr(dw0), n, Hd, int(x0), stream_ptr())
        return
    call("omlm_relpos_first_bwd", ptr(ds), ptr(dw0), n, Hd, stream_ptr())


def bias_silu_fwd(a, b, pre, z, R, C_):
    call("omlm_bias_silu_fwd", ptr(a), ptr(b), ptr(pre), ptr(z), R, C_, stream_ptr())


def silu_bwd(dz, pre, ds, total):
    call("omlm_silu_bwd", ptr(dz), ptr(pre), ptr(ds), total, stream_ptr())


def bias_add(a, b, out, R, C_, ld):
    call("omlm_bias_add", ptr(a), ptr(b), ptr(out), R, C_, ld, stream_ptr())


def relpos_mlp_fwd(w0, b0, W1, b1, W2, b2, W3, b3, saves, table, n, Hd, H, ldb, x0=0):
    sv = saves if saves is not None else [None] * 6
    if x0:
        call("omlm_relpos_mlp_fwd_from", ptr(w0), ptr(b0), ptr(W1), ptr(b1), ptr(W2), ptr(b2), ptr(W3), ptr(b3), *[ptr(t) for t in sv],
             ptr(table), int(n), int(Hd), int(H), int(ldb), int(x0), stream_ptr())
        return
    call("omlm_relpos_mlp_fwd", ptr(w0), ptr(b0), ptr(W1), ptr(b1), ptr(W2), ptr(b2), ptr(W3), ptr(b3), *[ptr(t) for t in sv], ptr(table),
         int(n), int(Hd), int(H), int(ldb), stream_ptr())


def relpos_mlp_bwd(dtable, W1, W2, W3, saves, scratch, grads, n, Hd, H, ldb, x0=0):
    if x0:
        call("omlm_relpos_mlp_bwd_from", ptr(dtable), ptr(W1), ptr(W2), ptr(W3), *[ptr(t) for t in saves], ptr(scratch),
             *[ptr(g) for g in grads], int(n), int(Hd), int(H), int(ldb), int(x0), stream_ptr())
        return
    call("omlm_relpos_mlp_bwd", ptr(dtable), ptr(W1), ptr(W2), ptr(W3), *[ptr(t) for t in saves], ptr(scratch), *[ptr(g) for g in grads],
         int(n), int(Hd), int(H), int(ldb), stream_ptr())


def rvq_encode(x, codebooks_T, indices, residual_out, n, D, C_, nstage, idx_stride=None):
    if idx_stride is None or idx_stride == nstage:
        call("omlm_rvq_encode", ptr(x), ptr(codebooks_T), ptr(indices), ptr(residual_out), n, D, C_, nstage, stream_ptr())
    else:
        assert nstage == 1
        call("omlm_rvq_encode_strided", ptr(x), ptr(codebooks_T), ptr(indices), int(idx_stride), ptr(residual_out), n, D, C_,
             stream_ptr())


def nearest_centroid(x, centroids_T, indices, n, D, C_):
    call("omlm_nearest_centroid", ptr(x), ptr(centroids_T), ptr(indices), n, D, C_, stream_ptr())


def vq_accumulate(x, indices, idx_stride, counts, sums, n, D, K):
    call("omlm_vq_accumulate", ptr(x), ptr(indices), int(idx_stride), ptr(counts), ptr(sums), n, D, K, stream_ptr())


def vq_kmeans_update(means, means_T, counts, sums, K, D):
    call("omlm_vq_kmeans_update", ptr(means), ptr(means_T), ptr(counts), ptr(sums), K, D, stream_ptr())


def vq_ema_update(cluster_size, embed_avg, embed, embed_T, counts, sums, total_scratch, K, D, decay, eps):
    call("omlm_vq_ema_update", ptr(cluster_size), ptr(embed_avg), ptr(embed), ptr(embed_T), ptr(counts), ptr(sums),
         ptr(total_scratch), K, D, float(decay), float(eps), stream_ptr())


def sample_topk_gumbel(logits, uniform, out, V, k, temperature, forbid_last):
    B, ld = logits.shape
    call("omlm_sample_topk_gumbel", ptr(logits), ptr(uniform), ptr(out), B, V, ld, int(k), float(temperature),
         int(forbid_last), stream_ptr())


def probe_tr16(out):
    call("omlm_probe_tr16", ptr(out), stream_ptr())
```

Baseline: 1172.

## Pair Q and KV projection GEMMs into a single persistent kernel launch

Adds a paired persistent GEMM walker that iterates over the tile spaces of two independent GEMMs in one launch. It is used for the forward Q/KV projections (with the qk-norm epilogue) and for the backward dq/dkv input-gradient GEMMs when fp16 activations are used. The aim is to cut launch overhead and fill the GPU better, since the narrow KV GEMM alone underuses it. The cost is extra per-tile selection logic and register pressure in the persistent kernel. A fallback to two separate calls remains when the shapes do not qualify.

```diff
diff --git a/include/omlm.h b/include/omlm.h
--- a/include/omlm.h
+++ b/include/omlm.h
@@ -37,6 +37,14 @@
 int omlm_gemm_qknorm(const void* A, const void* B, void* C, void* C2, int c2_col0, int ldc2, const float* scale, float* norm_out,
                      int ldnorm, int groups, long long a_rows, long long b_rows, int M, int N, int K, int lda, int ldb, int ldc,
                      int dtype, void* stream);
+int omlm_gemm_qknorm_pair(const void* A0, const void* B0, void* C0, void* C2_0, int c2_col0_0, int ldc2_0, const float* scale0, float* norm0,
+                          int ldnorm0, int groups0, long long a_rows0, long long b_rows0, int N0, int lda0, int ldb0, int ldc0,
+                          const void* A1, const void* B1, void* C1, void* C2_1, int c2_col0_1, int ldc2_1, const float* scale1, float* norm1,
+                          int ldnorm1, int groups1, long long a_rows1, long long b_rows1, int N1, int lda1, int ldb1, int ldc1,
+                          int M, int K, int dtype, void* stream);
+int omlm_gemm_pair(const void* A0, const void* B0, void* C0, long long a_rows0, long long b_rows0, int N0, int K0, int lda0, int ldb0, int ldc0,
+                   const void* A1, const void* B1, void* C1, long long a_rows1, long long b_rows1, int N1, int K1, int lda1, int ldb1, int ldc1,
+                   int M, int b_kmajor, int in_dtype, int out_dtype, void* workspace, long long workspace_bytes, void* stream);
 int omlm_qk_norm_bwd2(const float* dq, const float* dk, const float* dv, const void* q, const void* k, const float* qn, const float* kn,
                       const float* q_scale, const float* k_scale, void* dq_raw, void* dkv_raw, float* dq_scale, float* dk_scale,
                       int M, int H, int dtype, void* stream);
diff --git a/open_musiclm_amd/csrc/gemm.hip b/open_musiclm_amd/csrc/gemm.hip
--- a/open_musiclm_amd/csrc/gemm.hip
+++ b/open_musiclm_amd/csrc/gemm.hip
@@ -142,9 +142,17 @@
 }
 
 
-template <int BM_, int BN_, int WM_, int WN_, bool A_KMAJ, bool B_KMAJ, typename TOUT, bool CIN, int EPI = 0>
-__global__ __launch_bounds__((BM_ / WM_) * (BN_ / WN_) * 64) void gemm_bf16_tile_persist_kernel(GemmArgs g) {
-    extern __shared__ __attribute__((aligned(16))) char smem[];
+template <int MI, int NJ, int WN_, typename TOUT, bool CIN, int EPI>
+__device__ __forceinline__ void persist_epilogue(const GemmArgs& g, f32x16 (&acc)[MI][NJ], char* smem, int m0, int n0, int wm, int wn, int wave, int lane,
+                                                 float* patch) {
+    GemmArgs ge = g;
+    ge.c_map = nullptr;
+    if constexpr (!CIN) ge.Cin = nullptr;
+    tile_epilogue<MI, NJ, WN_, TOUT, EPI, false>(ge, acc, smem, m0, n0, wm, wn, wave, lane, false, patch);
+}
+
+template <int BM_, int BN_, int WM_, int WN_, bool A_KMAJ, bool B_KMAJ, typename TOUT, bool CIN, int EPI, bool PAIR>
+__device__ __forceinline__ void gemm_persist_walk(const GemmArgs& g0, const GemmArgs& g1, char* smem) {
     constexpr int NWN = BN_ / WN_, NWAVES = (BM_ / WM_) * NWN;
     constexpr int MI = WM_ / 32, NJ = WN_ / 32;
     constexpr int A_BYTES = BM_ * BK * 2, B_BYTES = BN_ * BK * 2, STAGE = A_BYTES + B_BYTES;
@@ -154,47 +162,61 @@
     constexpr int GROUP = OMLM_SUPER_ROWS / BM_;
     constexpr int VEC = sizeof(TOUT) == 2 ? 8 : 4, NSTORE = MI * (32 / (64 / (WN_ / VEC)));
 
-    const int tiles_m = (g.M + BM_ - 1) / BM_, tiles_n = (g.N + BN_ - 1) / BN_;
-    const int total = tiles_m * tiles_n;
-    const int nk = g.K / BK;
+    const int tm0 = (g0.M + BM_ - 1) / BM_, tn0 = (g0.N + BN_ - 1) / BN_;
+    const int tm1 = PAIR ? (g1.M + BM_ - 1) / BM_ : 0, tn1 = PAIR ? (g1.N + BN_ - 1) / BN_ : 0;
+    const int total0 = tm0 * tn0, total1 = tm1 * tn1;
+    const int total = total0 + total1;
     const int lane = threadIdx.x & 63;
     const int wave = __builtin_amdgcn_readfirstlane(threadIdx.x >> 6);
     const int wm = (wave / NWN) * WM_, wn = (wave % NWN) * WN_;
-    const dma_rsrc rsA = make_dma_rsrc(g.A, (unsigned long long)g.a_rows * g.lda * 2);
-    const dma_rsrc rsB = make_dma_rsrc(g.B, (unsigned long long)g.b_rows * g.ldb * 2);
+    const dma_rsrc rsA0 = make_dma_rsrc(g0.A, (unsigned long long)g0.a_rows * g0.lda * 2);
+    const dma_rsrc rsB0 = make_dma_rsrc(g0.B, (unsigned long long)g0.b_rows * g0.ldb * 2);
+    const dma_rsrc rsA1 = PAIR ? make_dma_rsrc(g1.A, (unsigned long long)g1.a_rows * g1.lda * 2) : rsA0;
+    const dma_rsrc rsB1 = PAIR ? make_dma_rsrc(g1.B, (unsigned long long)g1.b_rows * g1.ldb * 2) : rsB0;
     const unsigned smem_lds = (unsigned)(size_t)LDS_PTR(char, smem);
 
-    auto origin = [&](int lin, int& m0, int& n0) {
-        const int bid = xcd_logical_id(lin, total);
+    auto origin = [&](int lin, int& pr, int& m0, int& n0) {
+        const bool second = PAIR && lin >= total0;
+        pr = second ? 1 : 0;
+        const int tiles_m = second ? tm1 : tm0, tiles_n = second ? tn1 : tn0;
+        const int bid = second ? xcd_logical_id(lin - total0, total1) : xcd_logical_id(lin, total0);
         const int gsz = GROUP * tiles_n;
         const int grp = bid / gsz, first_m = grp * GROUP;
         const int rows_in = min(GROUP, tiles_m - first_m);
         m0 = (first_m + (bid - grp * gsz) % rows_in) * BM_;
         n0 = ((bid - grp * gsz) / rows_in) * BN_;
     };
-    auto piece = [&](int l, const unsigned (&va)[UA], const unsigned (&vb)[UB], int k0, unsigned stage_lds, bool live) {
+    auto piece = [&](int l, const unsigned (&va)[UA], const unsigned (&vb)[UB], int k0, unsigned stage_lds, bool live,
+                     const dma_rsrc rsA, const dma_rsrc rsB, int lda, int ldb) {
         if (l < UA) {
             const int b = wave + NWAVES * l;
             dma_issue_s(rsA, stage_lds + (unsigned)(b * 1024), live ? va[l] : OOB_OFF,
-                        A_KMAJ ? (unsigned)k0 * (unsigned)(g.lda * 2) : (unsigned)(k0 * 2));
+                        A_KMAJ ? (unsigned)k0 * (unsigned)(lda * 2) : (unsigned)(k0 * 2));
         } else {
             const int b = wave + NWAVES * (l - UA);
             dma_issue_s(rsB, stage_lds + (unsigned)A_BYTES + (unsigned)(b * 1024), live ? vb[l - UA] : OOB_OFF,
-                        B_KMAJ ? (unsigned)k0 * (unsigned)(g.ldb * 2) : (unsigned)(k0 * 2));
+                        B_KMAJ ? (unsigned)k0 * (unsigned)(ldb * 2) : (unsigned)(k0 * 2));
         }
     };
 
     int lin = blockIdx.x;
     const int G = gridDim.x;
     if (lin >= total) return;
-    int m0, n0;
-    origin(lin, m0, n0);
+    int pr, m0, n0;
+    origin(lin, pr, m0, n0);
     unsigned va[UA], vb[UB];
+    auto rsel = [](bool second, const dma_rsrc& x1, const dma_rsrc& x0) {
+        dma_rsrc r;
+#pragma unroll
+        for (int i = 0; i < 4; ++i) r[i] = second ? x1[i] : x0[i];
+        return r;
+    };
     {
+        const bool second = PAIR && pr;
         DmaStagerT<A_KMAJ, BM_, NWAVES> sa;
         DmaStagerT<B_KMAJ, BN_, NWAVES> sb;
-        sa.init(nullptr, g.lda, g.M, m0, wave, lane);
-        sb.init(nullptr, g.ldb, g.N, n0, wave, lane);
+        sa.init(nullptr, second ? g1.lda : g0.lda, second ? g1.M : g0.M, m0, wave, lane);
+        sb.init(nullptr, second ? g1.ldb : g0.ldb, second ? g1.N : g0.N, n0, wave, lane);
 #pragma unroll
         for (int i = 0; i < UA; ++i) va[i] = sa.vfast[i];
 #pragma unroll
@@ -202,20 +224,26 @@
     }
     int par = 0;
 #pragma unroll
-    for (int l = 0; l < UA + UB; ++l) piece(l, va, vb, 0, smem_lds, true);
+    for (int l = 0; l < UA + UB; ++l) piece(l, va, vb, 0, smem_lds, true, rsel(PAIR && pr, rsA1, rsA0), rsel(PAIR && pr, rsB1, rsB0), 0, 0);
     bool counted = false;
 
     for (;;) {
+        const bool second = PAIR && pr;
+        const dma_rsrc rsA = rsel(second, rsA1, rsA0), rsB = rsel(second, rsB1, rsB0);
+        const int nk = (second ? g1.K : g0.K) / BK;
+        const int lda = second ? g1.lda : g0.lda, ldb = second ? g1.ldb : g0.ldb;
         const int lin_n = lin + G;
         const bool has_next = lin_n < total;
-        int m0n = m0, n0n = n0;
-        if (has_next) origin(lin_n, m0n, n0n);
+        int prn = pr, m0n = m0, n0n = n0;
+        if (has_next) origin(lin_n, prn, m0n, n0n);
+        const bool second_n = PAIR && prn;
+        const dma_rsrc rsAn = rsel(second_n, rsA1, rsA0), rsBn = rsel(second_n, rsB1, rsB0);
         unsigned van[UA], vbn[UB];
         {
             DmaStagerT<A_KMAJ, BM_, NWAVES> sa;
             DmaStagerT<B_KMAJ, BN_, NWAVES> sb;
-            sa.init(nullptr, g.lda, g.M, m0n, wave, lane);
-            sb.init(nullptr, g.ldb, g.N, n0n, wave, lane);
+            sa.init(nullptr, second_n ? g1.lda : g0.lda, second_n ? g1.M : g0.M, m0n, wave, lane);
+            sb.init(nullptr, second_n ? g1.ldb : g0.ldb, second_n ? g1.N : g0.N, n0n, wave, lane);
 #pragma unroll
             for (int i = 0; i < UA; ++i) van[i] = sa.vfast[i];
 #pragma unroll
@@ -263,7 +291,7 @@
                                     for (int x = 0; x < UA; ++x) one_a[x] = v;
 #pragma unroll
                                     for (int x = 0; x < UB; ++x) one_b[x] = v;
-                                    piece(l, one_a, one_b, knext, nxt, live);
+                                    piece(l, one_a, one_b, knext, nxt, live, rsel(last, rsAn, rsA), rsel(last, rsBn, rsB), lda, ldb);
                                 }
                                 __builtin_amdgcn_sched_barrier(0);
                             }
@@ -299,19 +327,29 @@
         if (!has_next) asm volatile("s_waitcnt vmcnt(0)" ::: "memory");
         __syncthreads();
         float* patch = wave < NWAVES - 1 ? (float*)(smem + cur_last * STAGE + wave * PATCH) : (float*)(smem + 2 * STAGE);
-        GemmArgs ge = g;
-        ge.c_map = nullptr;
-        if constexpr (!CIN) ge.Cin = nullptr;
-        tile_epilogue<MI, NJ, WN_, TOUT, EPI, false>(ge, acc, smem, m0, n0, wm, wn, wave, lane, false, patch);
+        if (second) persist_epilogue<MI, NJ, WN_, TOUT, CIN, EPI>(g1, acc, smem, m0, n0, wm, wn, wave, lane, patch);
+        else        persist_epilogue<MI, NJ, WN_, TOUT, CIN, EPI>(g0, acc, smem, m0, n0, wm, wn, wave, lane, patch);
         if (!has_next) break;
-        counted = m0 + BM_ <= g.M && n0 + BN_ <= g.N;
+        counted = m0 + BM_ <= (second ? g1.M : g0.M) && n0 + BN_ <= (second ? g1.N : g0.N);
         par = (par + nk) & 1;
-        lin = lin_n; m0 = m0n; n0 = n0n;
+        lin = lin_n; pr = prn; m0 = m0n; n0 = n0n;
 #pragma unroll
         for (int i = 0; i < UA; ++i) va[i] = van[i];
 #pragma unroll
         for (int i = 0; i < UB; ++i) vb[i] = vbn[i];
     }
+}
+
+template <int BM_, int BN_, int WM_, int WN_, bool A_KMAJ, bool B_KMAJ, typename TOUT, bool CIN, int EPI = 0>
+__global__ __launch_bounds__((BM_ / WM_) * (BN_ / WN_) * 64) void gemm_bf16_tile_persist_kernel(GemmArgs g) {
+    extern __shared__ __attribute__((aligned(16))) char smem[];
+    gemm_persist_walk<BM_, BN_, WM_, WN_, A_KMAJ, B_KMAJ, TOUT, CIN, EPI, false>(g, g, smem);
+}
+
+template <int BM_, int BN_, int WM_, int WN_, bool A_KMAJ, bool B_KMAJ, typename TOUT, int EPI = 0>
+__global__ __launch_bounds__((BM_ / WM_) * (BN_ / WN_) * 64) void gemm_bf16_tile_persist_pair_kernel(GemmArgs g0, GemmArgs g1) {
+    extern __shared__ __attribute__((aligned(16))) char smem[];
+    gemm_persist_walk<BM_, BN_, WM_, WN_, A_KMAJ, B_KMAJ, TOUT, false, EPI, true>(g0, g1, smem);
 }
 
 
@@ -495,6 +533,8 @@
 template __global__ void gemm_bf16_tile_persist_kernel<128, 128, 64, 64, false, false, h16_t, false>(GemmArgs);
 template __global__ void gemm_bf16_tile_persist_kernel<128, 128, 64, 64, false, false, float, true>(GemmArgs);
 template __global__ void gemm_bf16_tile_persist_kernel<128, 128, 64, 64, false, false, h16_t, false, 1>(GemmArgs);
+template __global__ void gemm_bf16_tile_persist_pair_kernel<128, 128, 64, 64, false, false, h16_t, 1>(GemmArgs, GemmArgs);
+template __global__ void gemm_bf16_tile_persist_pair_kernel<128, 128, 64, 64, false, true, h16_t>(GemmArgs, GemmArgs);
 template __global__ void gemm_tile8_kernel<false, false, h16_t>(GemmArgs);
 template __global__ void gemm_tile8_kernel<false, true, h16_t>(GemmArgs);
 template __global__ void gemm_tile8_kernel<false, false, float>(GemmArgs);
@@ -838,31 +878,37 @@
                      in_dtype, out_dtype, alpha, stream, 0, nullptr, nullptr, nullptr, false, (float*)workspace, workspace_bytes);
 }
 
-#if !OMLM_FP16
-extern "C" int omlm_gemm_qknorm_h(const void* A, const void* B, void* C, void* C2, int c2_col0, int ldc2, const float* scale, float* norm_out,
-                                  int ldnorm, int groups, long long a_rows, long long b_rows, int M, int N, int K, int lda, int ldb, int ldc,
-                                  int dtype, void* stream);
-#endif
-extern "C" int OMLM_API(omlm_gemm_qknorm)(const void* A, const void* B, void* C, void* C2, int c2_col0, int ldc2, const float* scale,
-                                          float* norm_out, int ldnorm, int groups, long long a_rows, long long b_rows, int M, int N, int K,
-                                          int lda, int ldb, int ldc, int dtype, void* stream) {
-#if !OMLM_FP16
-    if (dtype == OMLM_DT_F16) return omlm_gemm_qknorm_h(A, B, C, C2, c2_col0, ldc2, scale, norm_out, ldnorm, groups, a_rows, b_rows, M, N, K, lda, ldb, ldc, 1, stream);
-#endif
-    if (M <= 0 || N <= 0) return OMLM_OK;
-    OMLM_CHECK_ARG(dtype == 1, "gemm_qknorm: operand dtype 1 (bf16) or 2 (fp16)");
+static int qknorm_args(GemmArgs& g, const void* A, const void* B, void* C, void* C2, int c2_col0, int ldc2, const float* scale, float* norm_out,
+                       int ldnorm, int groups, long long a_rows, long long b_rows, int M, int N, int K, int lda, int ldb, int ldc) {
     OMLM_CHECK_ARG(A && B && C && scale && norm_out && K > 0 && (K % 8) == 0, "gemm_qknorm: null operand / K");
     OMLM_CHECK_ARG((N % 64) == 0 && groups >= 0 && groups * 64 <= N && ldnorm >= groups, "gemm_qknorm: N must be whole 64-wide heads");
     OMLM_CHECK_ARG((lda % 8) == 0 && (ldb % 8) == 0 && (ldc % 8) == 0 && ((uintptr_t)A % 16) == 0 && ((uintptr_t)B % 16) == 0 && ((uintptr_t)C % 16) == 0,
                    "gemm_qknorm: 16-byte aligned operands, pitches multiples of 8");
     OMLM_CHECK_ARG(!C2 || ((c2_col0 % 64) == 0 && (ldc2 % 8) == 0 && ((uintptr_t)C2 % 16) == 0), "gemm_qknorm: second output");
     OMLM_CHECK_ARG((unsigned long long)a_rows * lda * 2 < 0xFFFFFFF0ull && (unsigned long long)b_rows * ldb * 2 < 0xFFFFFFF0ull, "operand exceeds the 4 GiB window");
-    GemmArgs g;
     memset(&g, 0, sizeof(g));
     g.A = A; g.B = B; g.C = C; g.a_rows = a_rows; g.b_rows = b_rows; g.M = M; g.N = N; g.K = K; g.lda = lda; g.ldb = ldb; g.ldc = ldc;
     g.alpha = 1.f; g.epi_scale = scale; g.epi_norm = norm_out; g.epi_groups = groups; g.epi_ldnorm = ldnorm; g.C2 = C2; g.c2_col0 = c2_col0; g.ldc2 = ldc2;
-    const int nk = (K + BK - 1) / BK;
-    g.kt_per_split = nk;
+    g.kt_per_split = (K + BK - 1) / BK;
+    return OMLM_OK;
+}
+
+#if !OMLM_FP16
+extern "C" int omlm_gemm_qknorm_h(const void* A, const void* B, void* C, void* C2, int c2_col0, int ldc2, const float* scale, float* norm_out,
+                                  int ldnorm, int groups, long long a_rows, long long b_rows, int M, int N, int K, int lda, int ldb, int ldc,
+                                  int dtype, void* stream);
+#endif
+extern "C" int OMLM_API(omlm_gemm_qknorm)(const void* A, const void* B, void* C, void* C2, int c2_col0, int ldc2, const float* scale,
+                                          float* norm_out, int ldnorm, int groups, long long a_rows, long long b_rows, int M, int N, int K,
+                                          int lda, int ldb, int ldc, int dtype, void* stream) {
+#if !OMLM_FP16
+    if (dtype == OMLM_DT_F16) return omlm_gemm_qknorm_h(A, B, C, C2, c2_col0, ldc2, scale, norm_out, ldnorm, groups, a_rows, b_rows, M, N, K, lda, ldb, ldc, 1, stream);
+#endif
+    if (M <= 0 || N <= 0) return OMLM_OK;
+    OMLM_CHECK_ARG(dtype == 1, "gemm_qknorm: operand dtype 1 (bf16) or 2 (fp16)");
+    GemmArgs g;
+    const int rc = qknorm_args(g, A, B, C, C2, c2_col0, ldc2, scale, norm_out, ldnorm, groups, a_rows, b_rows, M, N, K, lda, ldb, ldc);
+    if (rc != OMLM_OK) return rc;
     constexpr size_t LDS = 2 * (size_t)(128 + 128) * BK * 2;
     const int tiles = ((M + 127) / 128) * ((N + 127) / 128);
     auto kfast = gemm_bf16_tile_kernel<128, 128, 64, 64, false, false, h16_t, false, false, true, 1>;
@@ -884,6 +930,104 @@
     else if (K % BK == 0) hipLaunchKernelGGL(kfast, dim3(tiles, 1), dim3(256), LDS, as_stream(stream), g);
     else                                        hipLaunchKernelGGL(kgen, dim3(tiles, 1), dim3(256), LDS, as_stream(stream), g);
     return omlm_post_launch("omlm_gemm_qknorm");
+}
+
+#if OMLM_FP16
+#define OMLM_SELF(name) name##_h
+#else
+#define OMLM_SELF(name) name
+#endif
+
+#if !OMLM_FP16
+extern "C" int omlm_gemm_qknorm_pair_h(const void* A0, const void* B0, void* C0, void* C2_0, int c2_col0_0, int ldc2_0, const float* scale0,
+                                       float* norm0, int ldnorm0, int groups0, long long a_rows0, long long b_rows0, int N0, int lda0, int ldb0, int ldc0,
+                                       const void* A1, const void* B1, void* C1, void* C2_1, int c2_col0_1, int ldc2_1, const float* scale1,
+                                       float* norm1, int ldnorm1, int groups1, long long a_rows1, long long b_rows1, int N1, int lda1, int ldb1, int ldc1,
+                                       int M, int K, int dtype, void* stream);
+#endif
+extern "C" int OMLM_API(omlm_gemm_qknorm_pair)(const void* A0, const void* B0, void* C0, void* C2_0, int c2_col0_0, int ldc2_0, const float* scale0,
+                                               float* norm0, int ldnorm0, int groups0, long long a_rows0, long long b_rows0, int N0, int lda0, int ldb0, int ldc0,
+                                               const void* A1, const void* B1, void* C1, void* C2_1, int c2_col0_1, int ldc2_1, const float* scale1,
+                                               float* norm1, int ldnorm1, int groups1, long long a_rows1, long long b_rows1, int N1, int lda1, int ldb1, int ldc1,
+                                               int M, int K, int dtype, void* stream) {
+#if !OMLM_FP16
+    if (dtype == OMLM_DT_F16)
+        return omlm_gemm_qknorm_pair_h(A0, B0, C0, C2_0, c2_col0_0, ldc2_0, scale0, norm0, ldnorm0, groups0, a_rows0, b_rows0, N0, lda0, ldb0, ldc0,
+                                       A1, B1, C1, C2_1, c2_col0_1, ldc2_1, scale1, norm1, ldnorm1, groups1, a_rows1, b_rows1, N1, lda1, ldb1, ldc1,
+                                       M, K, 1, stream);
+#endif
+    OMLM_CHECK_ARG(dtype == 1, "gemm_qknorm_pair: operand dtype 1 (bf16) or 2 (fp16)");
+    const int slots = 2 * gemm_persist_slots();
+    if (M <= 0 || N0 <= 0 || N1 <= 0 || slots == 0 || K % BK != 0) {
+        int rc = OMLM_SELF(omlm_gemm_qknorm)(A0, B0, C0, C2_0, c2_col0_0, ldc2_0, scale0, norm0, ldnorm0, groups0, a_rows0, b_rows0, M, N0, K,
+                                            lda0, ldb0, ldc0, dtype, stream);
+        if (rc != OMLM_OK) return rc;
+        return OMLM_SELF(omlm_gemm_qknorm)(A1, B1, C1, C2_1, c2_col0_1, ldc2_1, scale1, norm1, ldnorm1, groups1, a_rows1, b_rows1, M, N1, K,
+                                          lda1, ldb1, ldc1, dtype, stream);
+    }
+    GemmArgs g0, g1;
+    int rc = qknorm_args(g0, A0, B0, C0, C2_0, c2_col0_0, ldc2_0, scale0, norm0, ldnorm0, groups0, a_rows0, b_rows0, M, N0, K, lda0, ldb0, ldc0);
+    if (rc != OMLM_OK) return rc;
+    rc = qknorm_args(g1, A1, B1, C1, C2_1, c2_col0_1, ldc2_1, scale1, norm1, ldnorm1, groups1, a_rows1, b_rows1, M, N1, K, lda1, ldb1, ldc1);
+    if (rc != OMLM_OK) return rc;
+    constexpr size_t LDSP = 2 * (size_t)(128 + 128) * BK * 2 + 32 * (64 + 4) * 4;
+    auto kp = gemm_bf16_tile_persist_pair_kernel<128, 128, 64, 64, false, false, h16_t, 1>;
+    static bool pattr = false;
+    if (!pattr) { (void)hipFuncSetAttribute((const void*)kp, hipFuncAttributeMaxDynamicSharedMemorySize, (int)LDSP); pattr = true; }
+    const int tiles = ((M + 127) / 128) * ((N0 + 127) / 128 + (N1 + 127) / 128);
+    hipLaunchKernelGGL(kp, dim3(tiles < slots ? tiles : slots), dim3(256), LDSP, as_stream(stream), g0, g1);
+    return omlm_post_launch("omlm_gemm_qknorm_pair");
+}
+
+#if !OMLM_FP16
+extern "C" int omlm_gemm_pair_h(const void* A0, const void* B0, void* C0, long long a_rows0, long long b_rows0, int N0, int K0, int lda0, int ldb0, int ldc0,
+                                const void* A1, const void* B1, void* C1, long long a_rows1, long long b_rows1, int N1, int K1, int lda1, int ldb1, int ldc1,
+                                int M, int b_kmajor, int in_dtype, int out_dtype, void* workspace, long long workspace_bytes, void* stream);
+#endif
+extern "C" int OMLM_API(omlm_gemm_pair)(const void* A0, const void* B0, void* C0, long long a_rows0, long long b_rows0, int N0, int K0, int lda0, int ldb0, int ldc0,
+                                        const void* A1, const void* B1, void* C1, long long a_rows1, long long b_rows1, int N1, int K1, int lda1, int ldb1, int ldc1,
+                                        int M, int b_kmajor, int in_dtype, int out_dtype, void* workspace, long long workspace_bytes, void* stream) {
+#if !OMLM_FP16
+    if (in_dtype == OMLM_DT_F16) {
+        OMLM_CHECK_ARG(out_dtype == OMLM_DT_F32 || out_dtype == OMLM_DT_F16, "fp16 operands produce fp32 or fp16 output");
+        return omlm_gemm_pair_h(A0, B0, C0, a_rows0, b_rows0, N0, K0, lda0, ldb0, ldc0, A1, B1, C1, a_rows1, b_rows1, N1, K1, lda1, ldb1, ldc1,
+                                M, b_kmajor, 1, OMLM_H_CODE(out_dtype), workspace, workspace_bytes, stream);
+    }
+#endif
+    const int slots = 2 * gemm_persist_slots();
+    const char* force = getenv("OMLM_GEMM_TILE");
+    auto narrow = [&](int N, int K, int lda, int ldb, const void* A, const void* B, const void* C, long long a_rows, long long b_rows) {
+        return N > 0 && N <= 1024 && K > 0 && K <= 512 && K % BK == 0 && lda % 8 == 0 && ldb % 8 == 0 && ((uintptr_t)A % 16) == 0 && ((uintptr_t)B % 16) == 0 &&
+               A && B && C && (!b_kmajor || ldb >= ((N + 7) / 8) * 8) && (unsigned long long)a_rows * lda * 2 < 0xFFFFFFF0ull &&
+               (unsigned long long)b_rows * ldb * 2 < 0xFFFFFFF0ull;
+    };
+    const long long tiles = (long long)((M + 127) / 128) * ((N0 + 127) / 128 + (N1 + 127) / 128);
+    if (!(in_dtype == 1 && out_dtype == 1 && M > 0 && slots > 0 && tiles > slots && !(force && force[0]) &&
+          narrow(N0, K0, lda0, ldb0, A0, B0, C0, a_rows0, b_rows0) && narrow(N1, K1, lda1, ldb1, A1, B1, C1, a_rows1, b_rows1))) {
+        int rc = OMLM_SELF(omlm_gemm)(A0, B0, C0, nullptr, nullptr, nullptr, nullptr, a_rows0, b_rows0, M, N0, K0, lda0, ldb0, ldc0, 0, 0, b_kmajor,
+                                     in_dtype, out_dtype, 1.0f, workspace, workspace_bytes, stream);
+        if (rc != OMLM_OK) return rc;
+        return OMLM_SELF(omlm_gemm)(A1, B1, C1, nullptr, nullptr, nullptr, nullptr, a_rows1, b_rows1, M, N1, K1, lda1, ldb1, ldc1, 0, 0, b_kmajor,
+                                   in_dtype, out_dtype, 1.0f, workspace, workspace_bytes, stream);
+    }
+    GemmArgs g0, g1;
+    memset(&g0, 0, sizeof(g0));
+    g0.A = A0; g0.B = B0; g0.C = C0; g0.a_rows = a_rows0; g0.b_rows = b_rows0; g0.M = M; g0.N = N0; g0.K = K0;
+    g0.lda = lda0; g0.ldb = ldb0; g0.ldc = ldc0; g0.alpha = 1.f; g0.kt_per_split = K0 / BK;
+    g1 = g0;
+    g1.A = A1; g1.B = B1; g1.C = C1; g1.a_rows = a_rows1; g1.b_rows = b_rows1; g1.N = N1; g1.K = K1;
+    g1.lda = lda1; g1.ldb = ldb1; g1.ldc = ldc1; g1.kt_per_split = K1 / BK;
+    constexpr size_t LDSP = 2 * (size_t)(128 + 128) * BK * 2 + 32 * (64 + 4) * 4;
+    auto k0 = gemm_bf16_tile_persist_pair_kernel<128, 128, 64, 64, false, false, h16_t>;
+    auto k1 = gemm_bf16_tile_persist_pair_kernel<128, 128, 64, 64, false, true, h16_t>;
+    static bool pattr = false;
+    if (!pattr) {
+        (void)hipFuncSetAttribute((const void*)k0, hipFuncAttributeMaxDynamicSharedMemorySize, (int)LDSP);
+        (void)hipFuncSetAttribute((const void*)k1, hipFuncAttributeMaxDynamicSharedMemorySize, (int)LDSP);
+        pattr = true;
+    }
+    hipLaunchKernelGGL(b_kmajor ? k1 : k0, dim3(slots), dim3(256), LDSP, as_stream(stream), g0, g1);
+    return omlm_post_launch("omlm_gemm_pair");
 }
 
 #if !OMLM_FP16
diff --git a/open_musiclm_amd/engine.py b/open_musiclm_amd/engine.py
--- a/open_musiclm_amd/engine.py
+++ b/open_musiclm_amd/engine.py
@@ -472,8 +472,8 @@
             qn = torch.empty(M, H, device=dev)
             kn = torch.empty(M, device=dev)
             q_raw, kv_raw = qn, kn
-            ops.gemm_qknorm(xn, w["Wq"], q, attn.q_scale.detach(), qn, H, M=M, N=H * DIM_HEAD, K=D)
-            ops.gemm_qknorm(xc, w["Wkv"], k, attn.k_scale.detach(), kn, 1, M=M, N=2 * DIM_HEAD, K=D, C2=v, c2_col0=DIM_HEAD)
+            ops.gemm_qknorm_pair(xn, w["Wq"], q, attn.q_scale.detach(), qn, H, xc, w["Wkv"], k, attn.k_scale.detach(), kn, 1,
+                                 M=M, N0=H * DIM_HEAD, N1=2 * DIM_HEAD, K=D, C2_1=v, c2_col0_1=DIM_HEAD)
         else:
             q_raw = torch.empty(M, H * DIM_HEAD, device=dev)
             kv_raw = torch.empty(M, 2 * DIM_HEAD, device=dev)
@@ -656,8 +656,11 @@
         dxn = torch.empty(M, D, dtype=T, device=dev)
         kv16 = T in _H16
         tmp = torch.empty(M, D, dtype=T if kv16 else torch.float32, device=dev)
-        ops.gemm(dq_raw, w["Wq"], dxn, M=M, N=D, K=H * DIM_HEAD, b_kmajor=True)
-        ops.gemm(dkv_raw, w["Wkv"], tmp, M=M, N=D, K=2 * DIM_HEAD, b_kmajor=True, Cin=None if kv16 else dx1)
+        if kv16:
+            ops.gemm_pair(dq_raw, w["Wq"], dxn, dkv_raw, w["Wkv"], tmp, M=M, N0=D, K0=H * DIM_HEAD, N1=D, K1=2 * DIM_HEAD, b_kmajor=True)
+        else:
+            ops.gemm(dq_raw, w["Wq"], dxn, M=M, N=D, K=H * DIM_HEAD, b_kmajor=True)
+            ops.gemm(dkv_raw, w["Wkv"], tmp, M=M, N=D, K=2 * DIM_HEAD, b_kmajor=True, Cin=dx1)
         gWq = grad_of(attn.to_q.weight)
         wgrad(dq_raw, sv.xn, gWq, H * DIM_HEAD, D)
         gWkv = grad_of(attn.to_kv.weight)
diff --git a/open_musiclm_amd/hip.py b/open_musiclm_amd/hip.py
--- a/open_musiclm_amd/hip.py
+++ b/open_musiclm_amd/hip.py
@@ -37,6 +37,8 @@
     "omlm_qk_norm_fwd": [vp, vp, vp, vp, vp, vp, vp, i32, i32, i32, vp],
     "omlm_qk_norm_bwd": [vp, vp, vp, vp, vp, vp, vp, vp, vp, vp, vp, i32, i32, i32, vp],
     "omlm_gemm_qknorm": [vp, vp, vp, vp, i32, i32, vp, vp, i32, i32, i64, i64, i32, i32, i32, i32, i32, i32, i32, vp],
+    "omlm_gemm_qknorm_pair": [vp, vp, vp, vp, i32, i32, vp, vp, i32, i32, i64, i64, i32, i32, i32, i32] * 2 + [i32, i32, i32, vp],
+    "omlm_gemm_pair": [vp, vp, vp, i64, i64, i32, i32, i32, i32, i32] * 2 + [i32, i32, i32, i32, vp, i64, vp],
     "omlm_qk_norm_bwd2": [vp, vp, vp, vp, vp, vp, vp, vp, vp, vp, vp, vp, vp, i32, i32, i32, vp],
     "omlm_attn_bias_table_floats": [i32, i32],
     "omlm_attn_bias_prepare": [vp, vp, i32, i32, i32, vp, vp, f32, f32, i32, vp],
diff --git a/open_musiclm_amd/ops.py b/open_musiclm_amd/ops.py
--- a/open_musiclm_amd/ops.py
+++ b/open_musiclm_amd/ops.py
@@ -335,6 +335,31 @@
          A.shape[-1], B.shape[-1], C_.shape[-1], dcode(A.dtype), stream_ptr())
 
 
+def gemm_qknorm_pair(A0, B0, C0, scale0, norm0, groups0, A1, B1, C1, scale1, norm1, groups1, *, M, N0, N1, K, C2_1=None, c2_col0_1=0):
+    hip.require_gpu(A0, "A0")
+    for A, B, C_, nrm, sc in ((A0, B0, C0, norm0, scale0), (A1, B1, C1, norm1, scale1)):
+        assert A.dtype in H16 and B.dtype == A.dtype and C_.dtype == A.dtype and nrm.dtype == torch.float32 and sc.dtype == torch.float32
+    assert A1.dtype == A0.dtype and (C2_1 is None or C2_1.dtype == A0.dtype)
+
+    def args(A, B, C_, C2, c2_col0, scale, nrm, groups, N):
+        return (ptr(A), ptr(B), ptr(C_), ptr(C2), int(c2_col0), C2.shape[-1] if C2 is not None else 0, ptr(scale), ptr(nrm),
+                nrm.shape[-1] if nrm.dim() > 1 else 1, int(groups), A.numel() // A.shape[-1], B.numel() // B.shape[-1], N,
+                A.shape[-1], B.shape[-1], C_.shape[-1])
+    call("omlm_gemm_qknorm_pair", *args(A0, B0, C0, None, 0, scale0, norm0, groups0, N0), *args(A1, B1, C1, C2_1, c2_col0_1, scale1, norm1, groups1, N1),
+         M, K, dcode(A0.dtype), stream_ptr())
+
+
+def gemm_pair(A0, B0, C0, A1, B1, C1, *, M, N0, K0, N1, K1, b_kmajor=False):
+    hip.require_gpu(A0, "A0")
+    assert A0.dtype in H16 and B0.dtype == A0.dtype and A1.dtype == A0.dtype and B1.dtype == A0.dtype and C1.dtype == C0.dtype
+    ws, wsb = tail_workspace(A0.device)
+
+    def args(A, B, C_, N, K):
+        return (ptr(A), ptr(B), ptr(C_), A.numel() // A.shape[-1], B.numel() // B.shape[-1], N, K, A.shape[-1], B.shape[-1], C_.shape[-1])
+    call("omlm_gemm_pair", *args(A0, B0, C0, N0, K0), *args(A1, B1, C1, N1, K1), M, int(b_kmajor), dcode(A0.dtype), dcode(C0.dtype),
+         ws, wsb, stream_ptr())
+
+
 def qk_norm_bwd2(dq, dk, dv, q, k, qn, kn, q_scale, k_scale, dq_raw, dkv_raw, dq_scale, dk_scale, H):
     call("omlm_qk_norm_bwd2", ptr(dq), ptr(dk), ptr(dv), ptr(q), ptr(k), ptr(qn), ptr(kn), ptr(q_scale), ptr(k_scale),
          ptr(dq_raw), ptr(dkv_raw), ptr(dq_scale), ptr(dk_scale), q.shape[0], H, dcode(dq_raw.dtype), stream_ptr())
```

Result: no change. 1178 (median of 6 runs) (+0.5%).
